# mattm458/tacotron2

Measured on AMD Instinct MI355X. Metric: mel-frames/sec (node), LJSpeech-shaped teacher-forced train step, b=32/GPU, fp32, higher is better.
Workload: dtype f32

## Files before the change

include/tacotron2_amd.h:

```cpp
#ifndef TACOTRON2_AMD_H
#define TACOTRON2_AMD_H
#include <stdint.h>
#ifdef __cplusplus
extern "C" {
#endif

#define T2_OK 0
#define T2_ERR_ARG 1
#define T2_ERR_LAUNCH 2
#define T2_ERR_RESIDENCY 3

const char* t2_last_error(void);
int t2_version(void);
int t2_sizeof(const char* struct_name);
int t2_debug_clock(int enable, uint64_t* out8);

typedef struct {
    const float* A; const float* B; float* C;
    int M, N, K;
    int64_t lda, ldb, ldc;
    int a_kmajor, b_kmajor;
    float alpha;
    const float* bias; const float* bias2;
    const float* mulmask; int64_t ldmask;
    int relu;
    int accumulate;
    int splitk;
    int batch; int64_t sA, sB, sC;
    int share_cu;
    int native_fp32;
    int a_tap_len; int64_t a_tap_stride;
    int precision;
    float* stat_out; int stat_Lp, stat_L;
} T2Gemm;
int t2_gemm(const T2Gemm* g, void* stream);

typedef struct { const float* x; int64_t ldx; const float* w; int64_t ldw; int K; } T2Seg;
typedef struct {
    int B, H;
    int nseg; T2Seg seg[3];
    const float* wpacked;
    const float* pre; int64_t ldpre;
    const float* bias1; const float* bias2;
    const float* c_prev; int64_t ldc_prev;
    const float* drop; int64_t lddrop;
    float* h_out; int64_t ldh;
    float* h_out2; int64_t ldh2;
    float* c_out; int64_t ldc_out;
    float* gates_out; int64_t ldg;
    const int32_t* len; int t;
    const float* xt;
    float* ht_out; int ht_col0;
    const float* zone_h; int64_t ldzone_h;
    const float* zone_c; int64_t ldzone_c;
    const float* h_prev; int64_t ldh_prev;
} T2LstmStep;
int t2_lstm_step_fwd(const T2LstmStep* steps, int n, void* stream);
int t2_lstm_pack_fwd(const T2Seg* segs, int nseg, int H, float* out, void* stream);
int t2_lstm_pack_bwd(const float* W, int64_t ldw, int N4, const float* W2, int64_t ldw2, int N2, int ncols, float* out,
                     void* stream);

typedef struct {
    int64_t seg_x[3]; int64_t pre, c_prev, drop, h_out, h_out2, c_out, gates_out; int dt;
    int64_t xt, ht_out;
    int64_t zone_h, zone_c, h_prev;
} T2LstmStride;
int t2_lstm_seq_fwd(const T2LstmStep* base, const T2LstmStride* inc, int n, int S, void* stream);
int t2_lstm_seq_fwd_persist(const T2LstmStep* base, const T2LstmStride* inc, int S, uint32_t* sync, void* stream);
int t2_lstm_seq_fwd_persist_n(const T2LstmStep* base, const T2LstmStride* inc, int n, int S, uint32_t* sync, void* stream);
int t2_lstm_seq_fwd_persist_pz(const T2LstmStep* base, const T2LstmStride* inc, int n, int S, uint32_t* counters, uint32_t* flag,
                               void* stream);
int t2_lstm_persist_resident(int H, int K, int B);
int t2_lstm_persist_resident_n(int H, int K, int B, int n);
typedef struct {
    void* p[64];
    int64_t row_bytes[64];
    int64_t nrows[64];
    int64_t stride_bytes[64];
    int n;
} T2ZeroRegions;
int t2_zero_regions(const T2ZeroRegions* r, void* stream);
int t2_stream_probe_chain(uint32_t* word, int n, void* stream);
int t2_stream_probe_spin(uint32_t* word, int microseconds, void* stream);
int t2_debug_persist_spin_limit(int polls);
int t2_guard_poison(const uint32_t* flag, float* x, int64_t n, void* stream);
typedef struct {
    int B, H, N4;
    const float* dg_next; int64_t lddg;
    const float* W; int64_t ldw;
    const float* dg2; int64_t lddg2; const float* W2; int64_t ldw2; int N2;
    const float* wtpacked;
    int ncols; int epi;
    const float* ext1; int64_t ldx1; const float* ext2; int64_t ldx2;
    float* dx_out; int64_t lddx;
    const float* drop; int64_t lddrop;
    const float* gates; int64_t ldgs;
    const float* c_prev; int64_t ldcp; const float* c_cur; int64_t ldcc;
    float* dc; int64_t lddc;
    float* dg_out; int64_t ldgo;
    float* dg_out2; int64_t ldgo2;
    const int32_t* len; int t;
    const float* dgt_next;
    float* dgt_out;
    int off_chain;
    const float* zone_h; int64_t ldzone_h;
    const float* zone_c; int64_t ldzone_c;
    float* dhz; int64_t lddhz;
} T2LstmBwdStep;
int t2_lstm_step_bwd(const T2LstmBwdStep* steps, int n, void* stream);
typedef struct { int64_t dg, dg2, ext1, ext2, drop, gates, c_prev, c_cur; int dt; int64_t dgt; int64_t zone_h, zone_c; } T2LstmBwdStride;
int t2_lstm_seq_bwd(const T2LstmBwdStep* base, const T2LstmBwdStride* inc, int n, int S, void* stream);

typedef struct {
    int B, L, A, Ad, Ef, Kl;
    const float* att_h; int64_t ldh;
    const float* Wq; const float* U; const float* v;
    const float* w_prev; int64_t ldw;
    const float* cum_prev; int64_t ldcum;
    const float* pmT; const float* memory; const int32_t* len;
    float* e_part; float* th_out;
    float* w_out; int64_t ldwo; float* cum_out; int64_t ldco;
    float* ctx_out; int64_t ldctx; float* ctx_out2; int64_t ldctx2;
    float* ctxt_out; int ctxt_col0;
    uint64_t* clk;
    int win_back, win_fwd;
    int32_t* win_peak;
    int forward;
} T2AttnStep;
int t2_attn_fold_location(const float* Wd, const float* Wc, float* U, int Ad, int F, int Kl, void* stream);
int t2_attn_step_fwd(const T2AttnStep* s, void* stream);

typedef struct {
    int B, L, T, A, Ad, Ef, Kl;
    const float* W_ih_ctx; int64_t ld_wih;
    const float* W_hh; const float* Wq; const float* U; const float* v;
    const float* wpacked;
    const float* pre; const float* pmT; const float* memory; const int32_t* len;
    const float* att_drop;
    float* xdec; float* att_c; float* gates; float* align; float* cum; float* th;
    float* xproj_ctx; int64_t ld_xproj;
    float* e_part;
    int t_begin, t_end;
    float* xdec_t;
    uint64_t* clk;
    int forward;
} T2AttnSeq;
int t2_attn_seq_fwd(const T2AttnSeq* a, void* stream);

typedef struct {
    int B, L, T, A, Ad, Ef, Kl;
    const float* W_ih_ctx; int64_t ld_wih;
    const float* W_hh; const float* Wq; const float* U; const float* v;
    const float* wtp_ctx;
    const float* wtp_h;
    const float* wtp_q;
    const float* memory; const float* xdec; const float* att_c; const float* gates; const float* align;
    const float* cum; const float* th; const float* att_drop;
    const float* dh_ext; int64_t ld_dh;
    const float* dctx_ext1; int64_t ld_dc1;
    const float* dctx_ext2; int64_t ld_dc2;
    float* dgates; float* dctx_tot; float* dq; float* dpmT; float* dv_part; float* dU_part;
    float* dc; float* G; float* de; float* din_part;
    float* dh_rec;
    int t_hi, t_lo;
    float* dgates_t;
    uint64_t* clk;
    float* ws_bd;
    const float* dalign;
} T2AttnSeqBwd;
int t2_attn_seq_bwd(const T2AttnSeqBwd* a, void* stream);

int t2_attn_seq_bwd_stash(const T2AttnSeqBwd* a, float* de_stash, int64_t ld_stash, void* stream);
int t2_attn_seq_bwd_forward(const T2AttnSeqBwd* a, float* de_stash, int64_t ld_stash, float* dprior, void* stream);
int t2_attn_acc_bwd(const T2AttnSeqBwd* a, const float* de_stash, int64_t ld_stash, int t_begin, int t_end, void* stream);
typedef struct { const float* zone_h; const float* zone_c; int64_t stride; float* dhz; } T2AttnZone;
int t2_attn_seq_fwd_zone(const T2AttnSeq* a, const T2AttnZone* z, void* stream);
int t2_attn_seq_bwd_zone(const T2AttnSeqBwd* a, float* de_stash, int64_t ld_stash, float* dprior, const T2AttnZone* z, void* stream);

int t2_embedding_fwd(const int64_t* idx, const float* table, float* out, int B, int L, int E, int pad, void* stream);
int t2_embedding_bwd(const int64_t* idx, const float* dout, float* dtable, int B, int L, int E, int Lp, int pad, void* stream);
int t2_pack_conv_weight(const float* w, float* wp, int Co, int Ci, int K, int flip, void* stream);
int t2_unpack_conv_wgrad(const float* gp, float* g, int Co, int Ci, int K, void* stream);

typedef struct {
    int B, L, C;
    const float* x; int Lp_x;
    const float* gamma; const float* beta;
    float* running_mean; float* running_var;
    int training; float momentum, eps;
    double* sums;
    float* mean; float* invstd;
    int act;
    const float* drop;
    const float* res; int Lp_res, pad_res;
    const int32_t* len; float fill;
    float* y; int Lp_y, pad_y;
    const float* dy; int Lp_dy, pad_dy;
    float* dx; int Lp_dx, pad_dx;
    float* dgamma; float* dbeta;
    int phase; const float* shift; float grad_share;
    int sums_prezeroed;
    const float* tile_stats; int tile_M;
} T2Bn;
int t2_bn_fwd(const T2Bn* s, void* stream);
int t2_bn_bwd(const T2Bn* s, void* stream);

int t2_colsum(const float* x, int64_t ld, int64_t R, int C, float* out, void* stream);
int t2_mel_to_tm(const float* mel, float* out, int B, int T, int M, void* stream);
int t2_swap01(const float* in, float* out, int D0, int D1, int C, int accumulate, void* stream);
int t2_finalize_fwd(const float* proj, int64_t ld_proj, const int32_t* len, float* mels, float* gates, float* post_in, int B,
                    int T, int M, void* stream);
int t2_finalize_bwd(const float* dpost_in, float* dproj, int B, int T, int M, void* stream);
int t2_outgrad_pack(const float* d_mels, const float* d_post, const float* d_gates, const int32_t* len, float* d_post_out,
                    float* dproj, int B, int T, int M, void* stream);
int t2_loss_fwd_bwd(const float* mels, const float* post, const float* gates, const float* mel_tgt, const float* gate_tgt,
                    const int32_t* len, int B, int T, int M, double* loss3 , float* d_post, float* dproj,
                    float grad_scale, void* stream);
int t2_loss_terms(const float* mels, const float* post, const float* gates, const float* mel_tgt, const float* gate_tgt,
                  const int32_t* len, int B, int T, int M, double* loss3, float* d_mels, float* d_post, float* d_gates,
                  float grad_scale, void* stream);
int t2_guided_attn(const float* align, const int32_t* chars_len, const int32_t* mel_len, int B, int T, int L, float sigma,
                   float alpha, double* loss, float* dalign, float grad_scale, void* stream);
int t2_mel_to_tm_r(const float* mel, float* out, int B, int T, int M, int r, void* stream);
int t2_finalize_fwd_r(const float* proj, int64_t ld_proj, const int32_t* len, float* mels, float* gates, float* post_in, int B,
                      int T, int M, int r, void* stream);
int t2_finalize_bwd_r(const float* dpost_in, float* dproj, int B, int T, int M, int r, void* stream);
int t2_outgrad_pack_r(const float* d_mels, const float* d_post, const float* d_gates, const int32_t* len, float* d_post_out,
                      float* dproj, int B, int T, int M, int r, void* stream);
int t2_loss_fwd_bwd_r(const float* mels, const float* post, const float* gates, const float* mel_tgt, const float* gate_tgt,
                      const int32_t* len, int B, int T, int M, int r, double* loss3, float* d_post, float* dproj,
                      float grad_scale, void* stream);
typedef struct { int mel_loss; int masked; float stop_weight; } T2LossOpts;
int t2_loss_fwd_bwd_opt(const float* mels, const float* post, const float* gates, const float* mel_tgt, const float* gate_tgt,
                        const int32_t* len, int B, int T, int M, int r, double* loss3, float* d_post, float* dproj,
                        float grad_scale, const T2LossOpts* opts, void* stream);
int t2_loss_terms_opt(const float* mels, const float* post, const float* gates, const float* mel_tgt, const float* gate_tgt,
                      const int32_t* len, int B, int T, int M, double* loss3, float* d_mels, float* d_post, float* d_gates,
                      float grad_scale, const T2LossOpts* opts, void* stream);
int t2_relu_mask_bwd(const float* g, const float* y, const float* mask, float* out, int64_t n, void* stream);
int t2_condition_fwd(const float* enc, const float* spk_table, const int32_t* spk, const float* desc, float* memory, int B,
                     int L, int E, int Ef, void* stream);
int t2_condition_bwd(const float* dmem, const float* memory, const int32_t* spk, float* denc, float* dspk_table, float* ddesc,
                     int B, int L, int E, int Ef, void* stream);
int t2_tanh_bias(float* x, const float* bias, int64_t rows, int C, void* stream);
int t2_leaky_relu(const float* x, float* y, int64_t n, float scale, float slope, void* stream);
int t2_axpy(const float* x, float* y, int64_t n, float alpha, void* stream);
int t2_tanh_bwd(const float* g, const float* y, float* out, int64_t n, void* stream);

int t2_linear_rows(const float* x, int64_t ldx, const float* w, int64_t ldw, const float* bias, const float* mask,
                   int64_t ldmask, int relu, float* out, int64_t ldo, int B, int N, int K, void* stream);
typedef struct {
    int B, L, A, D, Ef, Ad, P, M, Kl, Tcap;
    const float* W_comb; const float* b_comb; const float* row_comb;
    const float* W_pre2;
    const float* W_comb_t; const float* W_pre2_t; float* p1_t;
    const float* wp_att; const float* b_att_ih; const float* b_att_hh;
    const float* wp_dec; const float* b_dec_ih; const float* b_dec_hh;
    const float* Wq; const float* U; const float* v;
    const float* pmT; const float* memory; const int32_t* len;
    const float* prenet_mask;
    float* xs; float* att_h; float* att_c; float* dec_c; float* cum; float* xproj; float* p1; float* e_part;
    float* proj; int64_t ld_proj; float* align;
    int32_t* done; int32_t* state;
    const float* dec_pre;
    int win_back, win_fwd;
    int32_t* win_peak;
    int forward;
    float zone_p;
    const float* zone_att; const float* zone_dec;
    float stop_logit;
} T2Infer;
int t2_decoder_infer(const T2Infer* a, int t0, int t1, void* stream);
typedef struct { const float* proj[64]; int Bg[64]; int ngroups; int64_t ld_proj; int M, nframes; } T2StopScan;
int t2_stop_scan(const T2StopScan* s, int64_t* lengths, int32_t* out2, void* stream);
int t2_stop_scan_r(const T2StopScan* s, int r, int max_len, int64_t* lengths, int32_t* out2, void* stream);
int t2_stop_scan_thr(const T2StopScan* s, int r, int max_len, float stop_logit, int64_t* lengths, int32_t* out2, void* stream);

#define T2_ALIGN_MAX_L 4096
typedef struct {
    const float* align; int64_t ld_b, ld_s;
    int B, S, L, r, mode;
    const int32_t* chars_len;
    const int32_t* frames_len;
    int32_t* dur; int64_t ld_dur;
    float* stats;
    uint8_t* back;
} T2AlignDur;
int t2_align_durations(const T2AlignDur* a, void* stream);

#define T2_DTW_MAX_T 4096
#define T2_DTW_MAX_K 32
#define T2_CEPS_MAX_M 1024
typedef struct {
    const float* mel; int64_t ld_b, ld_t;
    int B, T, M, K;
    const int32_t* len;
    const float* basis;
    float* out; int64_t ld_ob, ld_ot;
} T2MelCeps;
int t2_mel_cepstra(const T2MelCeps* a, void* stream);
typedef struct {
    const float* a; int64_t ld_ab, ld_at;
    const float* b; int64_t ld_bb, ld_bt;
    int B, Ta, Tb, K;
    const int32_t* len_a; const int32_t* len_b;
    float scale;
    double* cost;
    int32_t* path_len;
    uint8_t* back;
    int32_t* path;
} T2Dtw;
int t2_dtw(const T2Dtw* a, void* stream);

#define T2_YIN_MAX_SPAN 4096
#define T2_PROSODY_NSTAT 8
#define T2_PROSODY_MAX_T 4096
typedef struct {
    const float* wav; int64_t ld_wav;
    const int64_t* n;
    int B; int64_t n_max;
    int sr, hop, W, tau_min, tau_max;
    float thr, vthr, power_floor;
    float* f0; float* aper; float* power;
    float* cmnd;
} T2Yin;
int t2_yin(const T2Yin* a, void* stream);
typedef struct {
    const float* f0; const float* aper; const float* power;
    const int64_t* n;
    int B, T, hop, S;
    float* out;
} T2ProsodyStats;
int t2_prosody_stats(const T2ProsodyStats* a, void* stream);

int t2_logmel_frames(int64_t n_samples, int hop);
int t2_logmel_fwd(const float* wav, int64_t n, const float* basis, const float* fb, float* padded, float* spec, float* mag,
                  float* out, int n_fft, int hop, int n_mels, void* stream);

int t2_logmel_batch_workspace(int B, int64_t n_max, int n_fft, int hop, int n_mels, int64_t* out5);
int t2_logmel_batch_fwd(const float* wavs, int64_t ld_wav, const int64_t* n_dev, int B, int64_t n_max, const float* basis,
                        const float* fb, float* padded, float* spec, float* mag, float* tmp, float* mel, int64_t T_out,
                        float* gate, int32_t* mel_len, int n_fft, int hop, int n_mels, void* stream);

int t2_philox_mask(float* out, int64_t n, float p, uint64_t seed, uint64_t stream_id, void* stream);
int t2_philox_bernoulli(float* out, int64_t n, float p, uint64_t seed, uint64_t stream_id, void* stream);
int t2_sumsq(const float* g, int64_t n, double* out, void* stream);
int t2_adam_step(float* p, const float* g, float* m, float* v, int64_t n, const double* sumsq, float max_norm, float lr,
                 float beta1, float beta2, float eps, float weight_decay, int step, float grad_scale, void* stream);

#ifdef __cplusplus
}
#endif
#endif
```

tacotron2_amd/csrc/t2_common.hpp:

```cpp
#pragma once
#include <hip/hip_runtime.h>
#include <mutex>
#include <unordered_map>
#include <stdint.h>
#include <stdio.h>
#include <string.h>
#include <stdlib.h>

#include "../../include/tacotron2_amd.h"

typedef float f32x4 __attribute__((ext_vector_type(4)));
typedef float f32x2 __attribute__((ext_vector_type(2)));
typedef float f32x16 __attribute__((ext_vector_type(16)));

#define T2_WAVE 64

#define T2_CHECK_LAUNCH()                                                     \
    do {                                                                      \
        hipError_t e__ = hipGetLastError();                                   \
        if (e__ != hipSuccess) {                                              \
            t2_set_error(hipGetErrorString(e__), __FILE__, __LINE__);         \
            return T2_ERR_LAUNCH;                                             \
        }                                                                     \
    } while (0)

#define T2_REQUIRE(cond, msg)                                                 \
    do {                                                                      \
        if (!(cond)) {                                                        \
            t2_set_error(msg, __FILE__, __LINE__);                            \
            return T2_ERR_ARG;                                                \
        }                                                                     \
    } while (0)

#define T2_TRY(expr)                                                          \
    do {                                                                      \
        int rc__ = (expr);                                                    \
        if (rc__ != 0) return rc__;                                           \
    } while (0)

void t2_set_error(const char* msg, const char* file, int line);

int t2_lstm_step_fwd_launch(const T2LstmStep* steps, int n, hipStream_t st);
int t2_lstm_step_bwd_launch(const T2LstmBwdStep* steps, int n, hipStream_t st, unsigned long long* clk = nullptr);
void t2_lstm_fwd_advance(T2LstmStep& c, const T2LstmStride& inc);
void t2_lstm_bwd_advance(T2LstmBwdStep& c, const T2LstmBwdStride& inc);

#define T2_CHAIN_PRIO() __builtin_amdgcn_s_setprio(3)

#ifdef T2_STAMPS
#define T2_RING_BEGIN(clk, cond, kind)                                                                              \
    unsigned long long* ring__ = nullptr;                                                                           \
    if ((clk) && (cond)) {                                                                                          \
        const unsigned long long seq__ = atomicAdd(&(clk)[32], 1ull);                                               \
        ring__ = (clk) + 40 + 8 * (seq__ % 11);                                                                     \
        ring__[0] = (kind); ring__[4] = 0; ring__[5] = 0; ring__[6] = 0;                                            \
        ring__[1] = __builtin_amdgcn_s_memrealtime(); ring__[3] = __builtin_amdgcn_s_memtime();                     \
    }
#define T2_RING(i) do { if (ring__) ring__[i] = __builtin_amdgcn_s_memtime(); } while (0)
#define T2_RING_END() do { if (ring__) { ring__[7] = __builtin_amdgcn_s_memtime(); ring__[2] = __builtin_amdgcn_s_memrealtime(); } } while (0)
#else
#define T2_RING_BEGIN(clk, cond, kind) do { } while (0)
#define T2_RING(i) do { } while (0)
#define T2_RING_END() do { } while (0)
#endif

#ifdef T2_AB_KNOBS
#define T2_KNOB(env, dflt) (getenv(env) ? atoi(getenv(env)) : (dflt))
#else
#define T2_KNOB(env, dflt) (dflt)
#endif

static inline int t2_cdiv(long a, long b) { return (int)((a + b - 1) / b); }
static inline bool t2_aligned16(const void* p) { return (((uintptr_t)p) & 15) == 0; }

__device__ __forceinline__ float t2_sigmoid(float x) { return __builtin_amdgcn_rcpf(1.0f + __expf(-x)); }
__device__ __forceinline__ float t2_tanh(float x) { return 1.0f - 2.0f * __builtin_amdgcn_rcpf(__expf(2.0f * x) + 1.0f); }

template <int CTRL, int ROW_MASK>
__device__ __forceinline__ float t2_dpp(float ident, float v) {
    return __builtin_bit_cast(float, __builtin_amdgcn_update_dpp(__builtin_bit_cast(int, ident), __builtin_bit_cast(int, v), CTRL,
                                                                 ROW_MASK, 0xf, false));
}
__device__ __forceinline__ float t2_wave_sum(float v) {
    v += t2_dpp<0xB1, 0xf>(0.f, v);
    v += t2_dpp<0x4E, 0xf>(0.f, v);
    v += t2_dpp<0x124, 0xf>(0.f, v);
    v += t2_dpp<0x128, 0xf>(0.f, v);
    v += t2_dpp<0x142, 0xa>(0.f, v);
    v += t2_dpp<0x143, 0xc>(0.f, v);
    return __builtin_bit_cast(float, __builtin_amdgcn_readlane(__builtin_bit_cast(int, v), 63));
}
__device__ __forceinline__ float t2_wave_max(float v) {
    const float ni = -__builtin_inff();
    v = fmaxf(v, t2_dpp<0xB1, 0xf>(ni, v));
    v = fmaxf(v, t2_dpp<0x4E, 0xf>(ni, v));
    v = fmaxf(v, t2_dpp<0x124, 0xf>(ni, v));
    v = fmaxf(v, t2_dpp<0x128, 0xf>(ni, v));
    v = fmaxf(v, t2_dpp<0x142, 0xa>(ni, v));
    v = fmaxf(v, t2_dpp<0x143, 0xc>(ni, v));
    return __builtin_bit_cast(float, __builtin_amdgcn_readlane(__builtin_bit_cast(int, v), 63));
}
__device__ __forceinline__ float t2_quad_sum(float v) {
    v += t2_dpp<0xB1, 0xf>(0.f, v);
    v += t2_dpp<0x4E, 0xf>(0.f, v);
    return v;
}
__device__ __forceinline__ float t2_oct_sum(float v) {
    v = t2_quad_sum(v);
    v += t2_dpp<0x141, 0xf>(0.f, v);
    return v;
}
__device__ __forceinline__ float t2_row_sum(float v) {
    v = t2_quad_sum(v);
    v += t2_dpp<0x124, 0xf>(0.f, v);
    v += t2_dpp<0x128, 0xf>(0.f, v);
    return v;
}
__device__ __forceinline__ float t2_half_sum_hi(float v) {
    v = t2_row_sum(v);
    v += t2_dpp<0x142, 0xa>(0.f, v);
    return v;
}
__device__ __forceinline__ double t2_wave_sum_d(double v) {
#pragma unroll
    for (int o = 32; o > 0; o >>= 1) v += __shfl_xor(v, o, 64);
    return v;
}

__device__ __forceinline__ float t2_block_sum(float v, float* red) {
    const int lane = threadIdx.x & 63, w = threadIdx.x >> 6, nw = (blockDim.x + 63) >> 6;
    v = t2_wave_sum(v);
    __syncthreads();
    if (lane == 0) red[w] = v;
    __syncthreads();
    float s = 0.f;
    for (int i = 0; i < nw; ++i) s += red[i];
    return s;
}
__device__ __forceinline__ float t2_block_max(float v, float* red) {
    const int lane = threadIdx.x & 63, w = threadIdx.x >> 6, nw = (blockDim.x + 63) >> 6;
    v = t2_wave_max(v);
    __syncthreads();
    if (lane == 0) red[w] = v;
    __syncthreads();
    float s = red[0];
    for (int i = 1; i < nw; ++i) s = fmaxf(s, red[i]);
    return s;
}

template <typename K>
inline bool t2_allow_lds(K kernel, size_t bytes) {
    if (bytes <= 64 * 1024) return true;
    if (bytes > 160 * 1024) return false;
    static std::unordered_map<const void*, size_t> granted;
    static std::mutex mu;
    const void* f = reinterpret_cast<const void*>(kernel);
    std::lock_guard<std::mutex> lock(mu);
    size_t& g = granted[f];
    if (bytes > g) {
        if (hipFuncSetAttribute(f, hipFuncAttributeMaxDynamicSharedMemorySize, (int)bytes) != hipSuccess) return false;
        g = bytes;
    }
    return true;
}

__device__ __forceinline__ void t2_philox4(uint32_t c0, uint32_t c1, uint32_t c2, uint32_t c3, uint32_t k0,
                                           uint32_t k1, uint32_t out[4]) {
#pragma unroll
    for (int r = 0; r < 10; ++r) {
        const uint64_t p0 = (uint64_t)0xD2511F53u * c0;
        const uint64_t p1 = (uint64_t)0xCD9E8D57u * c2;
        const uint32_t n0 = (uint32_t)(p1 >> 32) ^ c1 ^ k0;
        const uint32_t n1 = (uint32_t)p1;
        const uint32_t n2 = (uint32_t)(p0 >> 32) ^ c3 ^ k1;
        const uint32_t n3 = (uint32_t)p0;
        c0 = n0; c1 = n1; c2 = n2; c3 = n3;
        k0 += 0x9E3779B9u; k1 += 0xBB67AE85u;
    }
    out[0] = c0; out[1] = c1; out[2] = c2; out[3] = c3;
}
```

tacotron2_amd/csrc/t2_elementwise.hip:

```cpp
#include "t2_common.hpp"
#include <cmath>

namespace {

__global__ void embedding_fwd_kernel(const int64_t* idx, const float* table, float* out, int B, int L, int E, int pad) {
    const int Lp = L + 2 * pad;
    const long n = (long)B * Lp * E;
    for (long i = (long)blockIdx.x * blockDim.x + threadIdx.x; i < n; i += (long)gridDim.x * blockDim.x) {
        const int e = (int)(i % E);
        const long row = i / E;
        const int lp = (int)(row % Lp), b = (int)(row / Lp);
        const int l = lp - pad;
        float v = 0.f;
        if (l >= 0 && l < L) v = table[idx[(long)b * L + l] * E + e];
        out[i] = v;
    }
}

__global__ void embedding_bwd_kernel(const int64_t* idx, const float* dout, float* dtable, int B, int L, int E, int Lp,
                                     int pad) {
    const long n = (long)B * L * E;
    for (long i = (long)blockIdx.x * blockDim.x + threadIdx.x; i < n; i += (long)gridDim.x * blockDim.x) {
        const int e = (int)(i % E);
        const long row = i / E;
        const int l = (int)(row % L), b = (int)(row / L);
        const int64_t id = idx[row];
        if (id != 0) atomicAdd(&dtable[id * E + e], dout[((long)b * Lp + pad + l) * E + e]);
    }
}

__global__ void pack_conv_w_kernel(const float* w, float* wp, int Co, int Ci, int K, int flip) {
    const long n = (long)Co * Ci * K;
    for (long i = (long)blockIdx.x * blockDim.x + threadIdx.x; i < n; i += (long)gridDim.x * blockDim.x) {
        const int k = (int)(i % K);
        const int ci = (int)((i / K) % Ci);
        const int co = (int)(i / ((long)K * Ci));
        if (!flip) wp[(long)co * K * Ci + (long)k * Ci + ci] = w[i];
        else wp[(long)ci * K * Co + (long)(K - 1 - k) * Co + co] = w[i];
    }
}

__global__ void unpack_conv_wgrad_kernel(const float* gp, float* g, int Co, int Ci, int K) {
    const long n = (long)Co * Ci * K;
    for (long i = (long)blockIdx.x * blockDim.x + threadIdx.x; i < n; i += (long)gridDim.x * blockDim.x) {
        const int k = (int)(i % K);
        const int ci = (int)((i / K) % Ci);
        const int co = (int)(i / ((long)K * Ci));
        g[i] += gp[(long)co * K * Ci + (long)k * Ci + ci];
    }
}

struct BnK {
    int B, L, C;
    const float* x; int Lp_x;
    const float* gamma; const float* beta;
    float* rmean; float* rvar;
    int training; float momentum, eps;
    double* sums;
    const float* shift;
    float* mean; float* invstd;
    int act;
    const float* drop;
    const float* res; int Lp_res, pad_res;
    const int32_t* len; float fill;
    float* y; int Lp_y, pad_y;
    const float* dy; int Lp_dy, pad_dy;
    float* dx; int Lp_dx, pad_dx;
    float* dgamma; float* dbeta;
    double grad_share;
};

__global__ __launch_bounds__(256) void bn_stats_kernel(BnK p, int rows_per_block) {
    __shared__ float s1[4][64], s2[4][64];
    const int cl = threadIdx.x & 63, rl = threadIdx.x >> 6;
    const int c = blockIdx.x * 64 + cl;
    const long R = (long)p.B * p.L;
    const long r0 = (long)blockIdx.y * rows_per_block;
    long r1 = r0 + rows_per_block; if (r1 > R) r1 = R;
    float a = 0.f, q = 0.f;
    if (blockIdx.x == 0 && blockIdx.y == 0 && threadIdx.x == 0) atomicAdd(&p.sums[2 * p.C], (double)R);
    if (c < p.C) {
        const float sh = p.shift ? p.shift[c] : p.x[c];
        for (long r = r0 + rl; r < r1; r += 4) {
            const int b = (int)(r / p.L), l = (int)(r % p.L);
            const float v = p.x[((long)b * p.Lp_x + l) * p.C + c] - sh;
            a += v; q = fmaf(v, v, q);
        }
    }
    s1[rl][cl] = a; s2[rl][cl] = q;
    __syncthreads();
    if (rl == 0 && c < p.C) {
        const double sa = (double)s1[0][cl] + s1[1][cl] + s1[2][cl] + s1[3][cl];
        const double sq = (double)s2[0][cl] + s2[1][cl] + s2[2][cl] + s2[3][cl];
        atomicAdd(&p.sums[c], sa);
        atomicAdd(&p.sums[p.C + c], sq);
    }
}

__global__ __launch_bounds__(1024) void bn_merge_tiles_kernel(BnK p, const float* ts, int tile_M) {
    __shared__ double sn[16][64], sm[16][64], sq[16][64];
    const int cl = threadIdx.x & 63, tl = threadIdx.x >> 6;
    const int c = blockIdx.x * 64 + cl;
    const int ntile = (tile_M + 127) / 128;
    const int Lp = p.Lp_x, L = p.L;
    auto upto = [&](int x) { const int r = x % Lp; return (x / Lp) * L + (r < L ? r : L); };
    auto merge = [](double& n, double& mean, double& M2, double nt, double mt, double m2t) {
        if (nt <= 0) return;
        const double tot = n + nt, delta = mt - mean;
        mean += delta * nt / tot;
        M2 += m2t + delta * delta * n * nt / tot;
        n = tot;
    };
    double n = 0, mean = 0, M2 = 0;
    if (c < p.C) {
        for (int t0 = tl; t0 < ntile; t0 += 64) {
            float sh[4], s1[4], s2[4];
#pragma unroll
            for (int u = 0; u < 4; ++u) {
                const int t = t0 + 16 * u;
                const float* o = ts + (long)(t < ntile ? t : 0) * 3 * p.C + c;
                sh[u] = o[0]; s1[u] = o[p.C]; s2[u] = o[2 * (long)p.C];
            }
#pragma unroll
            for (int u = 0; u < 4; ++u) {
                const int t = t0 + 16 * u;
                if (t >= ntile) continue;
                const int r0 = t * 128, r1 = r0 + 128 < tile_M ? r0 + 128 : tile_M;
                const double nt = (double)(upto(r1) - upto(r0));
                if (nt <= 0) continue;
                merge(n, mean, M2, nt, (double)sh[u] + (double)s1[u] / nt, (double)s2[u] - (double)s1[u] * s1[u] / nt);
            }
        }
    }
    sn[tl][cl] = n; sm[tl][cl] = mean; sq[tl][cl] = M2;
    __syncthreads();
    for (int s_ = 8; s_ >= 1; s_ >>= 1) {
        if (tl < s_) {
            double a = sn[tl][cl], b = sm[tl][cl], d = sq[tl][cl];
            merge(a, b, d, sn[tl + s_][cl], sm[tl + s_][cl], sq[tl + s_][cl]);
            sn[tl][cl] = a; sm[tl][cl] = b; sq[tl][cl] = d;
        }
        __syncthreads();
    }
    if (tl == 0 && c < p.C) {
        n = sn[0][cl]; mean = sm[0][cl]; M2 = sq[0][cl];
        const double s = (double)(p.shift ? p.shift[c] : p.x[c]);
        const double dm = mean - s;
        p.sums[c] = n * dm;
        p.sums[p.C + c] = (M2 > 0 ? M2 : 0) + n * dm * dm;
        if (c == 0) p.sums[2 * p.C] = n;
    }
}

__global__ void bn_finalize_kernel(BnK p) {
    const int c = blockIdx.x * blockDim.x + threadIdx.x;
    if (c >= p.C) return;
    if (p.training) {
        const double n = p.sums[2 * p.C];
        const double md = p.sums[c] / n;
        double var = p.sums[p.C + c] / n - md * md;
        if (var < 0) var = 0;
        const double m = md + (double)(p.shift ? p.shift[c] : p.x[c]);
        p.mean[c] = (float)m;
        p.invstd[c] = (float)(1.0 / sqrt(var + (double)p.eps));
        if (p.rmean) {
            const double unb = n > 1 ? var * n / (n - 1) : var;
            p.rmean[c] = (1.f - p.momentum) * p.rmean[c] + p.momentum * (float)m;
            p.rvar[c] = (1.f - p.momentum) * p.rvar[c] + p.momentum * (float)unb;
        }
    } else {
        p.mean[c] = p.rmean[c];
        p.invstd[c] = 1.f / sqrtf(p.rvar[c] + p.eps);
    }
}

__global__ void bn_apply_kernel(BnK p) {
    const long n = (long)p.B * p.Lp_y * p.C;
    for (long i = (long)blockIdx.x * blockDim.x + threadIdx.x; i < n; i += (long)gridDim.x * blockDim.x) {
        const int c = (int)(i % p.C);
        const long row = i / p.C;
        const int lp = (int)(row % p.Lp_y), b = (int)(row / p.Lp_y);
        const int l = lp - p.pad_y;
        float v = 0.f;
        if (l >= 0 && l < p.L) {
            const float xv = p.x[((long)b * p.Lp_x + l) * p.C + c];
            v = (xv - p.mean[c]) * p.invstd[c] * p.gamma[c] + p.beta[c];
            if (p.act == 1) v = fmaxf(v, 0.f);
            else if (p.act == 2) v = t2_tanh(v);
            if (p.drop) v *= p.drop[((long)b * p.L + l) * p.C + c];
            if (p.res) v += p.res[((long)b * p.Lp_res + p.pad_res + l) * p.C + c];
            if (p.len && l >= p.len[b]) v = p.fill;
        }
        p.y[i] = v;
    }
}

__device__ __forceinline__ float bn_dz(const BnK& p, int b, int l, int c, float& xhat) {
    const float xv = p.x[((long)b * p.Lp_x + l) * p.C + c];
    xhat = (xv - p.mean[c]) * p.invstd[c];
    float g = p.dy[((long)b * p.Lp_dy + p.pad_dy + l) * p.C + c];
    if (p.drop) g *= p.drop[((long)b * p.L + l) * p.C + c];
    const float pre = xhat * p.gamma[c] + p.beta[c];
    if (p.act == 1) g = pre > 0.f ? g : 0.f;
    else if (p.act == 2) { const float t = t2_tanh(pre); g *= (1.f - t * t); }
    return g;
}

__global__ __launch_bounds__(256) void bn_bwd_reduce_kernel(BnK p, int rows_per_block) {
    __shared__ float s1[4][64], s2[4][64];
    const int cl = threadIdx.x & 63, rl = threadIdx.x >> 6;
    const int c = blockIdx.x * 64 + cl;
    const long R = (long)p.B * p.L;
    const long r0 = (long)blockIdx.y * rows_per_block;
    long r1 = r0 + rows_per_block; if (r1 > R) r1 = R;
    float a = 0.f, q = 0.f;
    if (blockIdx.x == 0 && blockIdx.y == 0 && threadIdx.x == 0) atomicAdd(&p.sums[2 * p.C], (double)R);
    if (c < p.C) {
        for (long r = r0 + rl; r < r1; r += 4) {
            const int b = (int)(r / p.L), l = (int)(r % p.L);
            float xh;
            const float dz = bn_dz(p, b, l, c, xh);
            a += dz; q = fmaf(dz, xh, q);
        }
    }
    s1[rl][cl] = a; s2[rl][cl] = q;
    __syncthreads();
    if (rl == 0 && c < p.C) {
        atomicAdd(&p.sums[c], (double)s1[0][cl] + s1[1][cl] + s1[2][cl] + s1[3][cl]);
        atomicAdd(&p.sums[p.C + c], (double)s2[0][cl] + s2[1][cl] + s2[2][cl] + s2[3][cl]);
    }
}

__global__ void bn_bwd_apply_kernel(BnK p) {
    const long n = (long)p.B * p.Lp_dx * p.C;
    const float invn = (float)(1.0 / p.sums[2 * p.C]);
    for (long i = (long)blockIdx.x * blockDim.x + threadIdx.x; i < n; i += (long)gridDim.x * blockDim.x) {
        const int c = (int)(i % p.C);
        const long row = i / p.C;
        const int lp = (int)(row % p.Lp_dx), b = (int)(row / p.Lp_dx);
        const int l = lp - p.pad_dx;
        float v = 0.f;
        if (l >= 0 && l < p.L) {
            float xh;
            const float dz = bn_dz(p, b, l, c, xh);
            const float gi = p.gamma[c] * p.invstd[c];
            if (p.training) v = gi * (dz - (float)p.sums[c] * invn - xh * (float)p.sums[p.C + c] * invn);
            else v = gi * dz;
        }
        p.dx[i] = v;
        if (lp == 0 && b == 0) {
            p.dbeta[c] += (float)(p.sums[c] * p.grad_share);
            p.dgamma[c] += (float)(p.sums[p.C + c] * p.grad_share);
        }
    }
}

void to_bnk(const T2Bn* s, BnK& k) {
    k.B = s->B; k.L = s->L; k.C = s->C; k.x = s->x; k.Lp_x = s->Lp_x; k.gamma = s->gamma; k.beta = s->beta;
    k.rmean = s->running_mean; k.rvar = s->running_var; k.training = s->training; k.momentum = s->momentum; k.eps = s->eps;
    k.sums = s->sums; k.mean = s->mean; k.invstd = s->invstd; k.act = s->act; k.drop = s->drop;
    k.res = s->res; k.Lp_res = s->Lp_res; k.pad_res = s->pad_res; k.len = s->len; k.fill = s->fill;
    k.y = s->y; k.Lp_y = s->Lp_y; k.pad_y = s->pad_y; k.dy = s->dy; k.Lp_dy = s->Lp_dy; k.pad_dy = s->pad_dy;
    k.dx = s->dx; k.Lp_dx = s->Lp_dx; k.pad_dx = s->pad_dx; k.dgamma = s->dgamma; k.dbeta = s->dbeta;
    k.shift = s->shift; k.grad_share = s->grad_share > 0.f ? (double)s->grad_share : 1.0;
}

inline int ew_grid(long n) { long g = (n + 255) / 256; return (int)(g > 4096 ? 4096 : (g < 1 ? 1 : g)); }

__global__ __launch_bounds__(256) void colsum_kernel(const float* x, long ld, long R, int C, float* out, int rows_per_block) {
    __shared__ float s1[4][64];
    const int cl = threadIdx.x & 63, rl = threadIdx.x >> 6;
    const int c = blockIdx.x * 64 + cl;
    const long r0 = (long)blockIdx.y * rows_per_block;
    long r1 = r0 + rows_per_block; if (r1 > R) r1 = R;
    float a = 0.f;
    if (c < C) for (long r = r0 + rl; r < r1; r += 4) a += x[r * ld + c];
    s1[rl][cl] = a;
    __syncthreads();
    if (rl == 0 && c < C) atomicAdd(&out[c], s1[0][cl] + s1[1][cl] + s1[2][cl] + s1[3][cl]);
}

__global__ __launch_bounds__(256) void colsum4_kernel(const float* x, long ld, long R, int C, float* out, int rows_per_block) {
    __shared__ f32x4 s1[4][64];
    const int cl = threadIdx.x & 63, rl = threadIdx.x >> 6;
    const int c = blockIdx.x * 256 + cl * 4;
    const int cc = c < C ? c : 0;
    const long r0 = (long)blockIdx.y * rows_per_block;
    long r1 = r0 + rows_per_block; if (r1 > R) r1 = R;
    f32x4 a = {0.f, 0.f, 0.f, 0.f};
    long r = r0 + rl;
    for (; r + 28 < r1; r += 32) {
        f32x4 v[8];
#pragma unroll
        for (int i = 0; i < 8; ++i) v[i] = *reinterpret_cast<const f32x4*>(x + (r + 4 * i) * ld + cc);
#pragma unroll
        for (int i = 0; i < 8; ++i) a += v[i];
    }
    for (; r < r1; r += 4) a += *reinterpret_cast<const f32x4*>(x + r * ld + cc);
    s1[rl][cl] = a;
    __syncthreads();
    if (rl == 0 && c < C) {
        const f32x4 t = s1[0][cl] + s1[1][cl] + s1[2][cl] + s1[3][cl];
        atomicAdd(&out[c], t[0]); atomicAdd(&out[c + 1], t[1]); atomicAdd(&out[c + 2], t[2]); atomicAdd(&out[c + 3], t[3]);
    }
}


template <bool GROUPED>
__global__ void mel_to_tm_kernel(const float* mel, float* out, int B, int T, int M, int r_, int S_) {
    const int r = GROUPED ? r_ : 1, S = GROUPED ? S_ : T;
    const long n = (long)(S + 1) * B * M;
    for (long i = (long)blockIdx.x * blockDim.x + threadIdx.x; i < n; i += (long)gridDim.x * blockDim.x) {
        const int m = (int)(i % M);
        const long row = i / M;
        const int b = (int)(row % B), s = (int)(row / B);
        const long t = (long)r * s - 1;
        out[i] = (s == 0 || (GROUPED && t >= T)) ? 0.f : mel[((long)b * T + t) * M + m];
    }
}

__global__ void swap01_kernel(const float* in, float* out, int D0, int D1, int C, int accumulate) {
    const long n = (long)D0 * D1 * C;
    for (long i = (long)blockIdx.x * blockDim.x + threadIdx.x; i < n; i += (long)gridDim.x * blockDim.x) {
        const int c = (int)(i % C);
        const long row = i / C;
        const int d1 = (int)(row % D1), d0 = (int)(row / D1);
        const long o = ((long)d1 * D0 + d0) * C + c;
        if (accumulate) out[o] += in[i]; else out[o] = in[i];
    }
}

template <bool GROUPED>
__global__ void finalize_fwd_kernel(const float* proj, long ldp, const int32_t* len, float* mels, float* gates, float* post_in,
                                    int B, int T, int M, int r_) {
    const int r = GROUPED ? r_ : 1;
    const int Tp = T + 4, M1 = M + 1;
    const long n = (long)B * Tp * M1;
    for (long i = (long)blockIdx.x * blockDim.x + threadIdx.x; i < n; i += (long)gridDim.x * blockDim.x) {
        const int m = (int)(i % M1);
        const long row = i / M1;
        const int tp = (int)(row % Tp), b = (int)(row / Tp);
        const int t = tp - 2;
        const bool in = t >= 0 && t < T;
        const int s = in ? t / r : 0, j = in ? t - s * r : 0;
        const float v = in ? proj[((long)s * B + b) * ldp + (m < M ? j * M + m : r * M)] : 0.f;
        if (m < M) {
            if (post_in) post_in[((long)b * Tp + tp) * M + m] = v;
            if (in) mels[((long)b * T + t) * M + m] = (t >= len[b]) ? 0.f : v;
        } else if (in) {
            gates[(long)b * T + t] = (t >= len[b]) ? -1000.f : v;
        }
    }
}

__device__ __forceinline__ float loss_stop_w() { return 1.f; }
__device__ __forceinline__ float loss_stop_w(float w) { return w; }
template <bool GROUPED, int MEL = 0, bool MASKED = false, bool WEIGHTED = false, typename... W>
__global__ __launch_bounds__(256) void loss_kernel(const float* mels, const float* post, const float* gates, const float* mel_tgt,
                                                   const float* gate_tgt, const int32_t* len, int B, int T, int M, int r_, int S_,
                                                   double* loss3, float* d_post, float* dproj, float gscale, float* d_mels,
                                                   float* d_gates, W... stop_weight) {
    static_assert(sizeof...(W) == (WEIGHTED ? 1 : 0), "the weight argument comes with WEIGHTED only");
    __shared__ double red[3][4];
    __shared__ unsigned long long nf_s;
    const float stop_w = loss_stop_w(stop_weight...);
    const int r = GROUPED ? r_ : 1, S = GROUPED ? S_ : T;
    const long nm = (long)B * T * M, ng = (long)B * T;
    const long nv = (long)B * S * r * M, ns = (long)B * S;
    const long ldq = (long)r * M + 1;
    float sm = 1.f / (float)nm, sg = 1.f / (float)ng;
    double dm = (double)nm, dg = (double)ng;
    if (MASKED) {
        if (threadIdx.x == 0) nf_s = 0ull;
        __syncthreads();
        unsigned long long c = 0ull;
        for (int b = threadIdx.x; b < B; b += blockDim.x) c += (unsigned long long)min(max(len[b], 0), T);
        if (c) atomicAdd(&nf_s, c);
        __syncthreads();
        const double nf = (double)nf_s;
        dg = nf; dm = nf * (double)M;
        sg = nf > 0.0 ? (float)(1.0 / dg) : 0.f;
        sm = nf > 0.0 ? (float)(1.0 / dm) : 0.f;
    }
    double a_g = 0, a_m = 0, a_p = 0;
    for (long i = (long)blockIdx.x * blockDim.x + threadIdx.x; i < nv + ns; i += (long)gridDim.x * blockDim.x) {
        if (i < nv) {
            const int m = (int)(i % M);
            const long row = i / M;
            const int tv = (int)(row % ((long)S * r)), b = (int)(row / ((long)S * r));
            const int s = tv / r, j = tv - s * r;
            float g = 0.f;
            if (tv < T) {
                const long k = ((long)b * T + tv) * M + m;
                const bool masked = tv >= len[b];
                float g1 = 0.f, g2 = 0.f;
                if (!MASKED || !masked) {
                    const float tg = mel_tgt[k];
                    const float e1 = mels[k] - tg, e2 = post[k] - tg;
                    if (MEL == 0) {
                        a_m += (double)e1 * e1; a_p += (double)e2 * e2;
                        g1 = masked ? 0.f : 2.f * e1 * sm * gscale;
                        g2 = masked ? 0.f : 2.f * e2 * sm * gscale;
                    } else {
                        const float s1 = (float)(e1 > 0.f) - (float)(e1 < 0.f), s2 = (float)(e2 > 0.f) - (float)(e2 < 0.f);
                        a_m += (double)fabsf(e1) + (MEL == 2 ? (double)e1 * e1 : 0.0);
                        a_p += (double)fabsf(e2) + (MEL == 2 ? (double)e2 * e2 : 0.0);
                        g1 = masked ? 0.f : (MEL == 2 ? 2.f * e1 + s1 : s1) * sm * gscale;
                        g2 = masked ? 0.f : (MEL == 2 ? 2.f * e2 + s2 : s2) * sm * gscale;
                    }
                }
                if (d_post) d_post[k] = g2;
                if (d_mels) d_mels[k] = g1;
                g = g1 + g2;
            }
            if (dproj) dproj[((long)s * B + b) * ldq + (long)j * M + m] = g;
        } else {
            const long q = i - nv;
            const int s = (int)(q % S), b = (int)(q / S);
            float gsum = 0.f;
            for (int j = 0; j < r; ++j) {
                const int t = s * r + j;
                if (t >= T) break;
                float g = 0.f;
                if (!MASKED || t < len[b]) {
                    const float x = gates[(long)b * T + t], y = gate_tgt[(long)b * T + t];
                    if (!WEIGHTED) {
                        a_g += (double)(fmaxf(x, 0.f) - x * y + log1pf(expf(-fabsf(x))));
                        g = t >= len[b] ? 0.f : (t2_sigmoid(x) - y) * sg * gscale;
                    } else {
                        const float l1p = log1pf(expf(-fabsf(x)));
                        a_g += (double)(y * (fmaxf(-x, 0.f) + l1p) + stop_w * (1.f - y) * (fmaxf(x, 0.f) + l1p));
                        g = t >= len[b] ? 0.f : (t2_sigmoid(x) * (y + stop_w * (1.f - y)) - y) * sg * gscale;
                    }
                }
                if (d_gates) d_gates[(long)b * T + t] = g;
                gsum = GROUPED ? gsum + g : g;
            }
            if (dproj) dproj[((long)s * B + b) * ldq + (long)r * M] = gsum;
        }
    }
    const int lane = threadIdx.x & 63, w = threadIdx.x >> 6;
    a_g = t2_wave_sum_d(a_g); a_m = t2_wave_sum_d(a_m); a_p = t2_wave_sum_d(a_p);
    if (lane == 0) { red[0][w] = a_g; red[1][w] = a_m; red[2][w] = a_p; }
    __syncthreads();
    if (threadIdx.x < 3) {
        const double s = red[threadIdx.x][0] + red[threadIdx.x][1] + red[threadIdx.x][2] + red[threadIdx.x][3];
        if (!MASKED) atomicAdd(&loss3[threadIdx.x], s / (threadIdx.x == 0 ? (double)ng : (double)nm));
        else if (dg > 0.0) atomicAdd(&loss3[threadIdx.x], s / (threadIdx.x == 0 ? dg : dm));
    }
}
__global__ __launch_bounds__(256) void guided_attn_kernel(const float* align, const int32_t* chars_len, const int32_t* mel_len,
                                                          int B, int T, int L, double inv2s2, float alpha, double* loss,
                                                          float* dalign, float gscale) {
    __shared__ double red[4];
    double acc = 0;
    const int lane = threadIdx.x & 63, w = __builtin_amdgcn_readfirstlane(threadIdx.x >> 6);
    for (long row = (long)blockIdx.x * 4 + w; row < (long)B * T; row += (long)gridDim.x * 4) {
        const int b = (int)(row / T), t = (int)(row - (long)b * T);
        const int Nb = min(max(chars_len[b], 0), L), Tb = min(max(mel_len[b], 0), T);
        const bool live = t < Tb && Nb > 0;
        const double invNT = live ? 1.0 / ((double)Nb * (double)Tb) : 0.0;
        const double coef = (double)alpha / (double)B * invNT;
        const float cg = (float)(coef * (double)gscale);
        float rowsum = 0.f;
        for (int l = lane; l < L; l += 64) {
            float g = 0.f;
            if (live && l < Nb) {
                const double x = (double)((long)l * Tb - (long)t * Nb) * invNT;
                g = -expm1f(-(float)(x * x * inv2s2));
                rowsum = fmaf(g, align[row * L + l], rowsum);
            }
            if (dalign) dalign[row * L + l] = cg * g;
        }
        acc += coef * (double)rowsum;
    }
    acc = t2_wave_sum_d(acc);
    if (lane == 0) red[w] = acc;
    __syncthreads();
    if (threadIdx.x == 0) atomicAdd(loss, red[0] + red[1] + red[2] + red[3]);
}

template <bool GROUPED>
__global__ void outgrad_pack_kernel(const float* d_mels, const float* d_post, const float* d_gates, const int32_t* len,
                                    float* d_post_out, float* dproj, int B, int T, int M, int r_, int S_) {
    const int r = GROUPED ? r_ : 1, S = GROUPED ? S_ : T;
    const long nv = (long)B * S * r * M, ns = (long)B * S;
    const long ldq = (long)r * M + 1;
    for (long i = (long)blockIdx.x * blockDim.x + threadIdx.x; i < nv + ns; i += (long)gridDim.x * blockDim.x) {
        if (i < nv) {
            const int m = (int)(i % M);
            const long row = i / M;
            const int tv = (int)(row % ((long)S * r)), b = (int)(row / ((long)S * r));
            const int s = tv / r, j = tv - s * r;
            float g = 0.f;
            if (tv < T) {
                const long k = ((long)b * T + tv) * M + m;
                const bool masked = tv >= len[b];
                const float g1 = (masked || !d_mels) ? 0.f : d_mels[k];
                const float g2 = (masked || !d_post) ? 0.f : d_post[k];
                d_post_out[k] = g2;
                g = g1 + g2;
            }
            dproj[((long)s * B + b) * ldq + (long)j * M + m] = g;
        } else {
            const long q = i - nv;
            const int s = (int)(q % S), b = (int)(q / S);
            float gsum = 0.f;
            if (d_gates)
                for (int j = 0; j < r; ++j) {
                    const int t = s * r + j;
                    if (t >= T || t >= len[b]) break;
                    gsum = GROUPED ? gsum + d_gates[(long)b * T + t] : d_gates[(long)b * T + t];
                }
            dproj[((long)s * B + b) * ldq + (long)r * M] = gsum;
        }
    }
}

template <bool GROUPED>
__global__ void finalize_bwd_kernel(const float* dpost_in, float* dproj, int B, int T, int M, int r_) {
    const int r = GROUPED ? r_ : 1;
    const int Tp = T + 4;
    const long n = (long)B * T * M;
    const long ldq = (long)r * M + 1;
    for (long i = (long)blockIdx.x * blockDim.x + threadIdx.x; i < n; i += (long)gridDim.x * blockDim.x) {
        const int m = (int)(i % M);
        const long row = i / M;
        const int t = (int)(row % T), b = (int)(row / T);
        const int s = t / r, j = t - s * r;
        dproj[((long)s * B + b) * ldq + (long)j * M + m] += dpost_in[((long)b * Tp + t) * M + m];
    }
}

__global__ void relu_mask_bwd_kernel(const float* g, const float* y, const float* mask, float* out, long n) {
    for (long i = (long)blockIdx.x * blockDim.x + threadIdx.x; i < n; i += (long)gridDim.x * blockDim.x)
        out[i] = y[i] > 0.f ? g[i] * (mask ? mask[i] : 1.f) : 0.f;
}

__global__ void condition_fwd_kernel(const float* enc, const float* spk_table, const int32_t* spk, const float* desc,
                                     float* memory, int B, int L, int E, int Ef) {
    const long n = (long)B * L * Ef;
    for (long i = (long)blockIdx.x * blockDim.x + threadIdx.x; i < n; i += (long)gridDim.x * blockDim.x) {
        const int e = (int)(i % Ef);
        const long row = i / Ef;
        const int b = (int)(row / L);
        float v;
        if (e < E) {
            v = enc[row * E + e];
            if (spk_table) v = t2_tanh(v + spk_table[(long)spk[b] * E + e]);
        } else {
            v = desc[(long)b * (Ef - E) + (e - E)];
        }
        memory[i] = v;
    }
}

__global__ void condition_bwd_kernel(const float* dmem, const float* memory, const int32_t* spk, int has_spk, float* denc,
                                     float* dspk_table, float* ddesc, int B, int L, int E, int Ef) {
    const int b = blockIdx.x, l0 = blockIdx.y * 16;
    for (int e = threadIdx.x; e < Ef; e += blockDim.x) {
        float g[16], m[16];
#pragma unroll
        for (int r = 0; r < 16; ++r) {
            const int l = l0 + r < L ? l0 + r : L - 1;
            const long i = ((long)b * L + l) * Ef + e;
            g[r] = dmem[i];
            m[r] = (e < E && has_spk) ? memory[i] : 0.f;
        }
        float acc = 0.f;
#pragma unroll
        for (int r = 0; r < 16; ++r) {
            if (l0 + r >= L) continue;
            float v = g[r];
            if (e < E) {
                if (has_spk) v *= (1.f - m[r] * m[r]);
                denc[((long)b * L + l0 + r) * E + e] = v;
            }
            acc += v;
        }
        if (e < E) { if (has_spk) atomicAdd(&dspk_table[(long)spk[b] * E + e], acc); }
        else if (ddesc) atomicAdd(&ddesc[(long)b * (Ef - E) + (e - E)], acc);
    }
}

__global__ void tanh_bias_kernel(float* x, const float* bias, long rows, int C) {
    const long n = rows * C;
    for (long i = (long)blockIdx.x * blockDim.x + threadIdx.x; i < n; i += (long)gridDim.x * blockDim.x)
        x[i] = t2_tanh(x[i] + (bias ? bias[i % C] : 0.f));
}
__global__ void tanh_bwd_kernel(const float* g, const float* y, float* out, long n) {
    for (long i = (long)blockIdx.x * blockDim.x + threadIdx.x; i < n; i += (long)gridDim.x * blockDim.x)
        out[i] = g[i] * (1.f - y[i] * y[i]);
}

__global__ void philox_mask_kernel(float* out, long n, float p, uint64_t seed, uint64_t stream_id) {
    const float keep_scale = 1.f / (1.f - p);
    const long n4 = (n + 3) / 4;
    for (long i = (long)blockIdx.x * blockDim.x + threadIdx.x; i < n4; i += (long)gridDim.x * blockDim.x) {
        uint32_t r[4];
        t2_philox4((uint32_t)i, (uint32_t)(i >> 32), (uint32_t)stream_id, (uint32_t)(stream_id >> 32), (uint32_t)seed,
                   (uint32_t)(seed >> 32), r);
#pragma unroll
        for (int j = 0; j < 4; ++j) {
            const long e = 4 * i + j;
            if (e < n) {
                const float u = (float)(r[j] >> 8) * (1.0f / 16777216.0f);
                out[e] = u < p ? 0.f : keep_scale;
            }
        }
    }
}

__global__ void philox_bernoulli_kernel(float* out, long n, float p, uint64_t seed, uint64_t stream_id) {
    const long n4 = (n + 3) / 4;
    for (long i = (long)blockIdx.x * blockDim.x + threadIdx.x; i < n4; i += (long)gridDim.x * blockDim.x) {
        uint32_t r[4];
        t2_philox4((uint32_t)i, (uint32_t)(i >> 32), (uint32_t)stream_id, (uint32_t)(stream_id >> 32), (uint32_t)seed,
                   (uint32_t)(seed >> 32), r);
#pragma unroll
        for (int j = 0; j < 4; ++j) {
            const long e = 4 * i + j;
            if (e < n) out[e] = (float)(r[j] >> 8) * (1.0f / 16777216.0f) < p ? 1.f : 0.f;
        }
    }
}

__global__ __launch_bounds__(256) void sumsq_kernel(const float* g, long n, double* out) {
    __shared__ double red[4];
    double a = 0;
    for (long i = (long)blockIdx.x * blockDim.x + threadIdx.x; i < n; i += (long)gridDim.x * blockDim.x) {
        const double v = g[i];
        a += v * v;
    }
    a = t2_wave_sum_d(a);
    if ((threadIdx.x & 63) == 0) red[threadIdx.x >> 6] = a;
    __syncthreads();
    if (threadIdx.x == 0) atomicAdd(out, red[0] + red[1] + red[2] + red[3]);
}

__global__ void adam_kernel(float* p, const float* g, float* m, float* v, long n, const double* sumsq, float max_norm,
                            float lr, float b1, float b2, float eps, float wd, float bc1, float bc2, float gscale) {
    float clip = 1.f;
    if (sumsq && !isfinite(*sumsq)) return;
    if (sumsq && max_norm > 0.f) {
        const float tot = (float)sqrt(*sumsq) * gscale;
        const float c = max_norm / (tot + 1e-6f);
        clip = c < 1.f ? c : 1.f;
    }
    clip *= gscale;
    for (long i = (long)blockIdx.x * blockDim.x + threadIdx.x; i < n; i += (long)gridDim.x * blockDim.x) {
        const float pv = p[i];
        const float gr = g[i] * clip + wd * pv;
        const float mv = b1 * m[i] + (1.f - b1) * gr;
        const float vv = b2 * v[i] + (1.f - b2) * gr * gr;
        m[i] = mv; v[i] = vv;
        p[i] = pv - lr * (mv / bc1) / (sqrtf(vv / bc2) + eps);
    }
}

__global__ void guard_poison_kernel(const uint32_t* flag, float* x, long n) {
    if (__hip_atomic_load(flag, __ATOMIC_RELAXED, __HIP_MEMORY_SCOPE_AGENT) == 0u) return;
    for (long i = (long)blockIdx.x * blockDim.x + threadIdx.x; i < n; i += (long)gridDim.x * blockDim.x) x[i] = __builtin_nanf("");
}

struct ZeroK { T2ZeroRegions r; };
__global__ __launch_bounds__(256) void zero_regions_kernel(ZeroK k) {
    const int y = blockIdx.y;
    char* base = (char*)k.r.p[y];
    const long rb = k.r.row_bytes[y], nr = k.r.nrows[y], sb = k.r.stride_bytes[y];
    const long tid = (long)blockIdx.x * blockDim.x + threadIdx.x, nth = (long)gridDim.x * blockDim.x;
    if (nr == 1 || sb == rb) {
        const long n = rb * nr;
        if ((((uintptr_t)base) & 15) == 0 && (n & 15) == 0) {
            f32x4* q = (f32x4*)base;
            const f32x4 z = {0.f, 0.f, 0.f, 0.f};
            for (long i = tid; i < (n >> 4); i += nth) q[i] = z;
        } else {
            uint32_t* q = (uint32_t*)base;
            for (long i = tid; i < (n >> 2); i += nth) q[i] = 0u;
        }
    } else {
        const long rw = rb >> 2;
        for (long i = tid; i < rw * nr; i += nth) {
            const long row = i / rw, c = i - row * rw;
            ((uint32_t*)(base + row * sb))[c] = 0u;
        }
    }
}

__global__ void probe_tick_kernel(uint32_t* word) { word[0] += 1u; }
__global__ void probe_spin_kernel(uint32_t* word, unsigned long long ticks) {
    const unsigned long long t0 = __builtin_amdgcn_s_memrealtime();
    unsigned polls = 0;
    while (__builtin_amdgcn_s_memrealtime() - t0 < ticks && polls < (1u << 24)) { __builtin_amdgcn_s_sleep(16); ++polls; }
    word[0] = polls;
}

}

#define ST ((hipStream_t)stream)

extern "C" int t2_zero_regions(const T2ZeroRegions* r, void* stream) {
    (void)hipGetLastError();
    T2_REQUIRE(r && r->n >= 0 && r->n <= 64, "t2_zero_regions: 0..64 regions");
    if (r->n == 0) return T2_OK;
    long most = 0;
    for (int i = 0; i < r->n; ++i) {
        T2_REQUIRE(r->p[i] && r->row_bytes[i] > 0 && r->nrows[i] > 0 && (r->row_bytes[i] & 3) == 0 && ((uintptr_t)r->p[i] & 3) == 0 &&
                   (r->nrows[i] == 1 || ((r->stride_bytes[i] & 3) == 0 && r->stride_bytes[i] >= r->row_bytes[i])),
                   "t2_zero_regions: regions are 4-byte aligned runs of whole words (rows: stride >= row, a multiple of 4)");
        const long n = r->row_bytes[i] * r->nrows[i];
        if (n > most) most = n;
    }
    long gx = (most + 16 * 256 * 8 - 1) / (16 * 256 * 8);
    gx = gx < 1 ? 1 : (gx > 1024 ? 1024 : gx);
    ZeroK k; k.r = *r;
    hipLaunchKernelGGL(zero_regions_kernel, dim3((unsigned)gx, r->n), dim3(256), 0, ST, k);
    T2_CHECK_LAUNCH(); return T2_OK;
}
extern "C" int t2_stream_probe_chain(uint32_t* word, int n, void* stream) {
    (void)hipGetLastError();
    T2_REQUIRE(word && n >= 0 && n <= 100000, "t2_stream_probe_chain: bad arguments");
    for (int i = 0; i < n; ++i) hipLaunchKernelGGL(probe_tick_kernel, dim3(1), dim3(1), 0, ST, word);
    T2_CHECK_LAUNCH(); return T2_OK;
}
extern "C" int t2_stream_probe_spin(uint32_t* word, int microseconds, void* stream) {
    (void)hipGetLastError();
    T2_REQUIRE(word && microseconds >= 0 && microseconds <= 50000, "t2_stream_probe_spin: 0..50000 us");
    hipLaunchKernelGGL(probe_spin_kernel, dim3(1), dim3(64), 0, ST, word, (unsigned long long)microseconds * 100ull);
    T2_CHECK_LAUNCH(); return T2_OK;
}

extern "C" int t2_guard_poison(const uint32_t* flag, float* x, int64_t n, void* stream) {
    (void)hipGetLastError();
    T2_REQUIRE(flag && x && n >= 0, "t2_guard_poison: bad arguments");
    if (n == 0) return T2_OK;
    hipLaunchKernelGGL(guard_poison_kernel, dim3(ew_grid(n) > 1024 ? 1024 : ew_grid(n)), dim3(256), 0, ST, flag, x, (long)n);
    T2_CHECK_LAUNCH(); return T2_OK;
}

extern "C" int t2_embedding_fwd(const int64_t* idx, const float* table, float* out, int B, int L, int E, int pad, void* stream) {
    (void)hipGetLastError();
    T2_REQUIRE(idx && table && out, "t2_embedding_fwd: null");
    hipLaunchKernelGGL(embedding_fwd_kernel, dim3(ew_grid((long)B * (L + 2 * pad) * E)), dim3(256), 0, ST, idx, table, out, B, L, E, pad);
    T2_CHECK_LAUNCH(); return T2_OK;
}
extern "C" int t2_embedding_bwd(const int64_t* idx, const float* dout, float* dtable, int B, int L, int E, int Lp, int pad, void* stream) {
    (void)hipGetLastError();
    T2_REQUIRE(idx && dout && dtable, "t2_embedding_bwd: null");
    hipLaunchKernelGGL(embedding_bwd_kernel, dim3(ew_grid((long)B * L * E)), dim3(256), 0, ST, idx, dout, dtable, B, L, E, Lp, pad);
    T2_CHECK_LAUNCH(); return T2_OK;
}
extern "C" int t2_pack_conv_weight(const float* w, float* wp, int Co, int Ci, int K, int flip, void* stream) {
    (void)hipGetLastError();
    T2_REQUIRE(w && wp, "t2_pack_conv_weight: null");
    hipLaunchKernelGGL(pack_conv_w_kernel, dim3(ew_grid((long)Co * Ci * K)), dim3(256), 0, ST, w, wp, Co, Ci, K, flip);
    T2_CHECK_LAUNCH(); return T2_OK;
}
extern "C" int t2_unpack_conv_wgrad(const float* gp, float* g, int Co, int Ci, int K, void* stream) {
    (void)hipGetLastError();
    T2_REQUIRE(gp && g, "t2_unpack_conv_wgrad: null");
    hipLaunchKernelGGL(unpack_conv_wgrad_kernel, dim3(ew_grid((long)Co * Ci * K)), dim3(256), 0, ST, gp, g, Co, Ci, K);
    T2_CHECK_LAUNCH(); return T2_OK;
}

extern "C" int t2_bn_fwd(const T2Bn* s, void* stream) {
    (void)hipGetLastError();
    T2_REQUIRE(s && s->x && s->gamma && s->beta && s->mean && s->invstd && s->y, "t2_bn_fwd: null operand");
    T2_REQUIRE(s->training ? (s->sums != nullptr) : (s->running_mean && s->running_var), "t2_bn_fwd: stats operands");
    T2_REQUIRE(s->phase >= 0 && s->phase <= 2 && (s->phase == 0 || (s->training && s->shift)),
               "t2_bn_fwd: phases 1/2 (sync-BN) need training statistics and a rank-independent shift");
    BnK k; to_bnk(s, k);
    if (s->training && s->phase != 2) {
        if (s->tile_stats) {
            T2_REQUIRE(s->tile_M > 0 && (long)s->tile_M <= (long)s->B * s->Lp_x, "t2_bn_fwd: tile_M is the producing GEMM's row count");
            hipLaunchKernelGGL(bn_merge_tiles_kernel, dim3(t2_cdiv(s->C, 64)), dim3(1024), 0, ST, k, s->tile_stats, s->tile_M);
        } else {
            if (!s->sums_prezeroed) (void)hipMemsetAsync(s->sums, 0, sizeof(double) * (2 * s->C + 2), ST);
            const long R = (long)s->B * s->L;
            const int rpb = 128;
            hipLaunchKernelGGL(bn_stats_kernel, dim3(t2_cdiv(s->C, 64), t2_cdiv(R, rpb)), dim3(256), 0, ST, k, rpb);
        }
    }
    if (s->phase != 1) {
        hipLaunchKernelGGL(bn_finalize_kernel, dim3(t2_cdiv(s->C, 256)), dim3(256), 0, ST, k);
        hipLaunchKernelGGL(bn_apply_kernel, dim3(ew_grid((long)s->B * s->Lp_y * s->C)), dim3(256), 0, ST, k);
    }
    T2_CHECK_LAUNCH(); return T2_OK;
}

extern "C" int t2_bn_bwd(const T2Bn* s, void* stream) {
    (void)hipGetLastError();
    T2_REQUIRE(s && s->x && s->gamma && s->beta && s->mean && s->invstd && s->dy && s->dx && s->sums && s->dgamma && s->dbeta,
               "t2_bn_bwd: null operand");
    T2_REQUIRE(s->phase >= 0 && s->phase <= 2, "t2_bn_bwd: bad phase");
    BnK k; to_bnk(s, k);
    if (s->phase != 2) {
        if (!s->sums_prezeroed) (void)hipMemsetAsync(s->sums, 0, sizeof(double) * (2 * s->C + 2), ST);
        const long R = (long)s->B * s->L;
        const int rpb = 128;
        hipLaunchKernelGGL(bn_bwd_reduce_kernel, dim3(t2_cdiv(s->C, 64), t2_cdiv(R, rpb)), dim3(256), 0, ST, k, rpb);
    }
    if (s->phase != 1) hipLaunchKernelGGL(bn_bwd_apply_kernel, dim3(ew_grid((long)s->B * s->Lp_dx * s->C)), dim3(256), 0, ST, k);
    T2_CHECK_LAUNCH(); return T2_OK;
}

extern "C" int t2_colsum(const float* x, int64_t ld, int64_t R, int C, float* out, void* stream) {
    (void)hipGetLastError();
    T2_REQUIRE(x && out && R > 0 && C > 0, "t2_colsum: bad arguments");
    if (C % 4 == 0 && ld % 4 == 0 && t2_aligned16(x) && C >= 256) {
        const int cb = t2_cdiv(C, 256);
        long rpb = t2_cdiv(R, t2_cdiv(1024, cb)); rpb = (rpb + 31) / 32 * 32; if (rpb < 32) rpb = 32;
        hipLaunchKernelGGL(colsum4_kernel, dim3(cb, t2_cdiv(R, rpb)), dim3(256), 0, ST, x, (long)ld, (long)R, C, out, (int)rpb);
    } else {
        const int rpb = 256;
        hipLaunchKernelGGL(colsum_kernel, dim3(t2_cdiv(C, 64), t2_cdiv(R, rpb)), dim3(256), 0, ST, x, (long)ld, (long)R, C, out, rpb);
    }
    T2_CHECK_LAUNCH(); return T2_OK;
}
extern "C" int t2_mel_to_tm(const float* mel, float* out, int B, int T, int M, void* stream) {
    (void)hipGetLastError();
    T2_REQUIRE(mel && out, "t2_mel_to_tm: null");
    hipLaunchKernelGGL(mel_to_tm_kernel<false>, dim3(ew_grid((long)(T + 1) * B * M)), dim3(256), 0, ST, mel, out, B, T, M, 1, T);
    T2_CHECK_LAUNCH(); return T2_OK;
}
extern "C" int t2_swap01(const float* in, float* out, int D0, int D1, int C, int accumulate, void* stream) {
    (void)hipGetLastError();
    T2_REQUIRE(in && out, "t2_swap01: null");
    hipLaunchKernelGGL(swap01_kernel, dim3(ew_grid((long)D0 * D1 * C)), dim3(256), 0, ST, in, out, D0, D1, C, accumulate);
    T2_CHECK_LAUNCH(); return T2_OK;
}
extern "C" int t2_finalize_fwd(const float* proj, int64_t ld_proj, const int32_t* len, float* mels, float* gates, float* post_in,
                               int B, int T, int M, void* stream) {
    (void)hipGetLastError();
    T2_REQUIRE(proj && len && mels && gates, "t2_finalize_fwd: null");
    hipLaunchKernelGGL(finalize_fwd_kernel<false>, dim3(ew_grid((long)B * (T + 4) * (M + 1))), dim3(256), 0, ST, proj, (long)ld_proj, len,
                       mels, gates, post_in, B, T, M, 1);
    T2_CHECK_LAUNCH(); return T2_OK;
}
extern "C" int t2_loss_fwd_bwd(const float* mels, const float* post, const float* gates, const float* mel_tgt,
                               const float* gate_tgt, const int32_t* len, int B, int T, int M, double* loss3, float* d_post,
                               float* dproj, float grad_scale, void* stream) {
    (void)hipGetLastError();
    T2_REQUIRE(mels && post && gates && mel_tgt && gate_tgt && len && loss3, "t2_loss_fwd_bwd: null");
    (void)hipMemsetAsync(loss3, 0, 3 * sizeof(double), ST);
    hipLaunchKernelGGL(loss_kernel<false>, dim3(ew_grid((long)B * T * (M + 1))), dim3(256), 0, ST, mels, post, gates, mel_tgt, gate_tgt,
                       len, B, T, M, 1, T, loss3, d_post, dproj, grad_scale, (float*)nullptr, (float*)nullptr);
    T2_CHECK_LAUNCH(); return T2_OK;
}
extern "C" int t2_loss_terms(const float* mels, const float* post, const float* gates, const float* mel_tgt, const float* gate_tgt,
                             const int32_t* len, int B, int T, int M, double* loss3, float* d_mels, float* d_post, float* d_gates,
                             float grad_scale, void* stream) {
    (void)hipGetLastError();
    T2_REQUIRE(mels && post && gates && mel_tgt && gate_tgt && len && loss3, "t2_loss_terms: null");
    (void)hipMemsetAsync(loss3, 0, 3 * sizeof(double), ST);
    hipLaunchKernelGGL(loss_kernel<false>, dim3(ew_grid((long)B * T * (M + 1))), dim3(256), 0, ST, mels, post, gates, mel_tgt, gate_tgt,
                       len, B, T, M, 1, T, loss3, d_post, (float*)nullptr, grad_scale, d_mels, d_gates);
    T2_CHECK_LAUNCH(); return T2_OK;
}
extern "C" int t2_guided_attn(const float* align, const int32_t* chars_len, const int32_t* mel_len, int B, int T, int L, float sigma,
                              float alpha, double* loss, float* dalign, float grad_scale, void* stream) {
    (void)hipGetLastError();
    T2_REQUIRE(align && chars_len && mel_len && loss, "t2_guided_attn: null");
    T2_REQUIRE(B >= 1 && T >= 1 && L >= 1, "t2_guided_attn: need B, T, L >= 1");
    T2_REQUIRE(sigma > 0.f && alpha >= 0.f, "t2_guided_attn: need sigma > 0 and alpha >= 0");
    (void)hipMemsetAsync(loss, 0, sizeof(double), ST);
    const long wgs = ((long)B * T + 3) / 4;
    hipLaunchKernelGGL(guided_attn_kernel, dim3((unsigned)(wgs > 4096 ? 4096 : wgs)), dim3(256), 0, ST, align, chars_len, mel_len,
                       B, T, L, 1.0 / (2.0 * (double)sigma * (double)sigma), alpha, loss, dalign, grad_scale);
    T2_CHECK_LAUNCH(); return T2_OK;
}
extern "C" int t2_outgrad_pack(const float* d_mels, const float* d_post, const float* d_gates, const int32_t* len,
                               float* d_post_out, float* dproj, int B, int T, int M, void* stream) {
    (void)hipGetLastError();
    T2_REQUIRE(len && d_post_out && dproj, "t2_outgrad_pack: null");
    hipLaunchKernelGGL(outgrad_pack_kernel<false>, dim3(ew_grid((long)B * T * (M + 1))), dim3(256), 0, ST, d_mels, d_post, d_gates, len,
                       d_post_out, dproj, B, T, M, 1, T);
    T2_CHECK_LAUNCH(); return T2_OK;
}
extern "C" int t2_finalize_bwd(const float* dpost_in, float* dproj, int B, int T, int M, void* stream) {
    (void)hipGetLastError();
    T2_REQUIRE(dpost_in && dproj, "t2_finalize_bwd: null");
    hipLaunchKernelGGL(finalize_bwd_kernel<false>, dim3(ew_grid((long)B * T * M)), dim3(256), 0, ST, dpost_in, dproj, B, T, M, 1);
    T2_CHECK_LAUNCH(); return T2_OK;
}
#define T2_REQUIRE_GROUPED(name) \
    T2_REQUIRE(B >= 1 && T >= 1 && M >= 1 && r >= 1 && (long)((T + r - 1) / r) * r < (1L << 31), name ": need B, T, M >= 1 and r >= 1")
extern "C" int t2_mel_to_tm_r(const float* mel, float* out, int B, int T, int M, int r, void* stream) {
    (void)hipGetLastError();
    T2_REQUIRE(mel && out, "t2_mel_to_tm_r: null");
    T2_REQUIRE_GROUPED("t2_mel_to_tm_r");
    if (r == 1) return t2_mel_to_tm(mel, out, B, T, M, stream);
    const int S = (T + r - 1) / r;
    hipLaunchKernelGGL(mel_to_tm_kernel<true>, dim3(ew_grid((long)(S + 1) * B * M)), dim3(256), 0, ST, mel, out, B, T, M, r, S);
    T2_CHECK_LAUNCH(); return T2_OK;
}
extern "C" int t2_finalize_fwd_r(const float* proj, int64_t ld_proj, const int32_t* len, float* mels, float* gates, float* post_in,
                                 int B, int T, int M, int r, void* stream) {
    (void)hipGetLastError();
    T2_REQUIRE(proj && len && mels && gates, "t2_finalize_fwd_r: null");
    T2_REQUIRE_GROUPED("t2_finalize_fwd_r");
    T2_REQUIRE(ld_proj >= (int64_t)r * M + 1, "t2_finalize_fwd_r: ld_proj < r * M + 1");
    if (r == 1) return t2_finalize_fwd(proj, ld_proj, len, mels, gates, post_in, B, T, M, stream);
    hipLaunchKernelGGL(finalize_fwd_kernel<true>, dim3(ew_grid((long)B * (T + 4) * (M + 1))), dim3(256), 0, ST, proj, (long)ld_proj, len, mels,
                       gates, post_in, B, T, M, r);
    T2_CHECK_LAUNCH(); return T2_OK;
}
extern "C" int t2_loss_fwd_bwd_r(const float* mels, const float* post, const float* gates, const float* mel_tgt,
                                 const float* gate_tgt, const int32_t* len, int B, int T, int M, int r, double* loss3, float* d_post,
                                 float* dproj, float grad_scale, void* stream) {
    (void)hipGetLastError();
    T2_REQUIRE(mels && post && gates && mel_tgt && gate_tgt && len && loss3 && d_post && dproj, "t2_loss_fwd_bwd_r: null");
    T2_REQUIRE_GROUPED("t2_loss_fwd_bwd_r");
    if (r == 1) return t2_loss_fwd_bwd(mels, post, gates, mel_tgt, gate_tgt, len, B, T, M, loss3, d_post, dproj, grad_scale, stream);
    const int S = (T + r - 1) / r;
    (void)hipMemsetAsync(loss3, 0, 3 * sizeof(double), ST);
    hipLaunchKernelGGL(loss_kernel<true>, dim3(ew_grid((long)B * S * ((long)r * M + 1))), dim3(256), 0, ST, mels, post, gates, mel_tgt,
                       gate_tgt, len, B, T, M, r, S, loss3, d_post, dproj, grad_scale, (float*)nullptr, (float*)nullptr);
    T2_CHECK_LAUNCH(); return T2_OK;
}
static int loss_opts_check(const T2LossOpts* o, const char* what) {
    T2_REQUIRE(o != nullptr, what);
    T2_REQUIRE(o->mel_loss >= 0 && o->mel_loss <= 2, what);
    T2_REQUIRE(std::isfinite(o->stop_weight) && o->stop_weight > 0.f, what);
    return T2_OK;
}
template <bool GROUPED>
static void loss_opt_launch(const T2LossOpts* o, unsigned grid, hipStream_t st, const float* mels, const float* post, const float* gates,
                            const float* mel_tgt, const float* gate_tgt, const int32_t* len, int B, int T, int M, int r, int S,
                            double* loss3, float* d_post, float* dproj, float gs, float* d_mels, float* d_gates) {
    const int key = o->mel_loss * 4 + (o->masked ? 2 : 0) + (o->stop_weight != 1.f ? 1 : 0);
#define T2_LOSS_CASE(MEL, MASKED)                               \
    case (MEL) * 4 + (MASKED) * 2:                                                                                                   \
        hipLaunchKernelGGL((loss_kernel<GROUPED, MEL, (MASKED) != 0, false>), dim3(grid), dim3(256), 0, st, mels, post, gates, mel_tgt, \
                           gate_tgt, len, B, T, M, r, S, loss3, d_post, dproj, gs, d_mels, d_gates);                                  \
        break;                                                                                                                       \
    case (MEL) * 4 + (MASKED) * 2 + 1:                                                                                               \
        hipLaunchKernelGGL((loss_kernel<GROUPED, MEL, (MASKED) != 0, true, float>), dim3(grid), dim3(256), 0, st, mels, post, gates,  \
                           mel_tgt, gate_tgt, len, B, T, M, r, S, loss3, d_post, dproj, gs, d_mels, d_gates, o->stop_weight);         \
        break;
    switch (key) {
        T2_LOSS_CASE(0, 0) T2_LOSS_CASE(0, 1) T2_LOSS_CASE(1, 0) T2_LOSS_CASE(1, 1) T2_LOSS_CASE(2, 0) T2_LOSS_CASE(2, 1)
    }
#undef T2_LOSS_CASE
}
static bool loss_opts_default(const T2LossOpts* o) { return o->mel_loss == 0 && !o->masked && o->stop_weight == 1.f; }
extern "C" int t2_loss_fwd_bwd_opt(const float* mels, const float* post, const float* gates, const float* mel_tgt,
                                   const float* gate_tgt, const int32_t* len, int B, int T, int M, int r, double* loss3, float* d_post,
                                   float* dproj, float grad_scale, const T2LossOpts* opts, void* stream) {
    (void)hipGetLastError();
    T2_REQUIRE(mels && post && gates && mel_tgt && gate_tgt && len && loss3 && d_post && dproj, "t2_loss_fwd_bwd_opt: null");
    T2_REQUIRE_GROUPED("t2_loss_fwd_bwd_opt");
    T2_TRY(loss_opts_check(opts, "t2_loss_fwd_bwd_opt: need options with mel_loss in {0, 1, 2} and a finite stop_weight > 0"));
    if (loss_opts_default(opts))
        return t2_loss_fwd_bwd_r(mels, post, gates, mel_tgt, gate_tgt, len, B, T, M, r, loss3, d_post, dproj, grad_scale, stream);
    const int S = (T + r - 1) / r;
    (void)hipMemsetAsync(loss3, 0, 3 * sizeof(double), ST);
    const unsigned grid = ew_grid((long)B * S * ((long)r * M + 1));
    if (r == 1) loss_opt_launch<false>(opts, grid, ST, mels, post, gates, mel_tgt, gate_tgt, len, B, T, M, 1, T, loss3, d_post, dproj,
                                       grad_scale, nullptr, nullptr);
    else loss_opt_launch<true>(opts, grid, ST, mels, post, gates, mel_tgt, gate_tgt, len, B, T, M, r, S, loss3, d_post, dproj, grad_scale,
                               nullptr, nullptr);
    T2_CHECK_LAUNCH(); return T2_OK;
}
extern "C" int t2_loss_terms_opt(const float* mels, const float* post, const float* gates, const float* mel_tgt, const float* gate_tgt,
                                 const int32_t* len, int B, int T, int M, double* loss3, float* d_mels, float* d_post, float* d_gates,
                                 float grad_scale, const T2LossOpts* opts, void* stream) {
    (void)hipGetLastError();
    T2_REQUIRE(mels && post && gates && mel_tgt && gate_tgt && len && loss3, "t2_loss_terms_opt: null");
    T2_REQUIRE(B >= 1 && T >= 1 && M >= 1, "t2_loss_terms_opt: need B, T, M >= 1");
    T2_TRY(loss_opts_check(opts, "t2_loss_terms_opt: need options with mel_loss in {0, 1, 2} and a finite stop_weight > 0"));
    if (loss_opts_default(opts))
        return t2_loss_terms(mels, post, gates, mel_tgt, gate_tgt, len, B, T, M, loss3, d_mels, d_post, d_gates, grad_scale, stream);
    (void)hipMemsetAsync(loss3, 0, 3 * sizeof(double), ST);
    loss_opt_launch<false>(opts, ew_grid((long)B * T * (M + 1)), ST, mels, post, gates, mel_tgt, gate_tgt, len, B, T, M, 1, T, loss3, d_post,
                           nullptr, grad_scale, d_mels, d_gates);
    T2_CHECK_LAUNCH(); return T2_OK;
}
extern "C" int t2_outgrad_pack_r(const float* d_mels, const float* d_post, const float* d_gates, const int32_t* len,
                                 float* d_post_out, float* dproj, int B, int T, int M, int r, void* stream) {
    (void)hipGetLastError();
    T2_REQUIRE(len && d_post_out && dproj, "t2_outgrad_pack_r: null");
    T2_REQUIRE_GROUPED("t2_outgrad_pack_r");
    if (r == 1) return t2_outgrad_pack(d_mels, d_post, d_gates, len, d_post_out, dproj, B, T, M, stream);
    const int S = (T + r - 1) / r;
    hipLaunchKernelGGL(outgrad_pack_kernel<true>, dim3(ew_grid((long)B * S * ((long)r * M + 1))), dim3(256), 0, ST, d_mels, d_post, d_gates,
                       len, d_post_out, dproj, B, T, M, r, S);
    T2_CHECK_LAUNCH(); return T2_OK;
}
extern "C" int t2_finalize_bwd_r(const float* dpost_in, float* dproj, int B, int T, int M, int r, void* stream) {
    (void)hipGetLastError();
    T2_REQUIRE(dpost_in && dproj, "t2_finalize_bwd_r: null");
    T2_REQUIRE_GROUPED("t2_finalize_bwd_r");
    if (r == 1) return t2_finalize_bwd(dpost_in, dproj, B, T, M, stream);
    hipLaunchKernelGGL(finalize_bwd_kernel<true>, dim3(ew_grid((long)B * T * M)), dim3(256), 0, ST, dpost_in, dproj, B, T, M, r);
    T2_CHECK_LAUNCH(); return T2_OK;
}
extern "C" int t2_relu_mask_bwd(const float* g, const float* y, const float* mask, float* out, int64_t n, void* stream) {
    (void)hipGetLastError();
    T2_REQUIRE(g && y && out, "t2_relu_mask_bwd: null");
    hipLaunchKernelGGL(relu_mask_bwd_kernel, dim3(ew_grid(n)), dim3(256), 0, ST, g, y, mask, out, (long)n);
    T2_CHECK_LAUNCH(); return T2_OK;
}
extern "C" int t2_condition_fwd(const float* enc, const float* spk_table, const int32_t* spk, const float* desc, float* memory,
                                int B, int L, int E, int Ef, void* stream) {
    (void)hipGetLastError();
    T2_REQUIRE(enc && memory && (Ef == E || desc), "t2_condition_fwd: bad arguments");
    hipLaunchKernelGGL(condition_fwd_kernel, dim3(ew_grid((long)B * L * Ef)), dim3(256), 0, ST, enc, spk_table, spk, desc, memory, B,
                       L, E, Ef);
    T2_CHECK_LAUNCH(); return T2_OK;
}
extern "C" int t2_condition_bwd(const float* dmem, const float* memory, const int32_t* spk, float* denc, float* dspk_table,
                                float* ddesc, int B, int L, int E, int Ef, void* stream) {
    (void)hipGetLastError();
    T2_REQUIRE(dmem && memory && denc, "t2_condition_bwd: null");
    hipLaunchKernelGGL(condition_bwd_kernel, dim3(B, t2_cdiv(L, 16)), dim3(256), 0, ST, dmem, memory, spk, dspk_table != nullptr, denc,
                       dspk_table, ddesc, B, L, E, Ef);
    T2_CHECK_LAUNCH(); return T2_OK;
}
__global__ void leaky_relu_kernel(const float* x, float* y, long n, float scale, float slope) {
    for (long i = (long)blockIdx.x * blockDim.x + threadIdx.x; i < n; i += (long)gridDim.x * blockDim.x) {
        const float v = scale * x[i];
        y[i] = v > 0.f ? v : slope * v;
    }
}
__global__ void axpy_kernel(const float* x, float* y, long n, float alpha) {
    for (long i = (long)blockIdx.x * blockDim.x + threadIdx.x; i < n; i += (long)gridDim.x * blockDim.x) y[i] = fmaf(alpha, x[i], y[i]);
}
extern "C" int t2_leaky_relu(const float* x, float* y, int64_t n, float scale, float slope, void* stream) {
    (void)hipGetLastError();
    T2_REQUIRE(x && y && n >= 0, "t2_leaky_relu: bad arguments");
    if (n == 0) return T2_OK;
    hipLaunchKernelGGL(leaky_relu_kernel, dim3(ew_grid(n)), dim3(256), 0, ST, x, y, (long)n, scale, slope);
    T2_CHECK_LAUNCH(); return T2_OK;
}
extern "C" int t2_axpy(const float* x, float* y, int64_t n, float alpha, void* stream) {
    (void)hipGetLastError();
    T2_REQUIRE(x && y && n >= 0, "t2_axpy: bad arguments");
    if (n == 0) return T2_OK;
    hipLaunchKernelGGL(axpy_kernel, dim3(ew_grid(n)), dim3(256), 0, ST, x, y, (long)n, alpha);
    T2_CHECK_LAUNCH(); return T2_OK;
}
extern "C" int t2_tanh_bias(float* x, const float* bias, int64_t rows, int C, void* stream) {
    (void)hipGetLastError();
    T2_REQUIRE(x, "t2_tanh_bias: null");
    hipLaunchKernelGGL(tanh_bias_kernel, dim3(ew_grid(rows * C)), dim3(256), 0, ST, x, bias, (long)rows, C);
    T2_CHECK_LAUNCH(); return T2_OK;
}
extern "C" int t2_tanh_bwd(const float* g, const float* y, float* out, int64_t n, void* stream) {
    (void)hipGetLastError();
    T2_REQUIRE(g && y && out, "t2_tanh_bwd: null");
    hipLaunchKernelGGL(tanh_bwd_kernel, dim3(ew_grid(n)), dim3(256), 0, ST, g, y, out, (long)n);
    T2_CHECK_LAUNCH(); return T2_OK;
}
extern "C" int t2_philox_mask(float* out, int64_t n, float p, uint64_t seed, uint64_t stream_id, void* stream) {
    (void)hipGetLastError();
    T2_REQUIRE(out && n >= 0 && p >= 0.f && p < 1.f, "t2_philox_mask: bad arguments");
    if (n == 0) return T2_OK;
    hipLaunchKernelGGL(philox_mask_kernel, dim3(ew_grid((n + 3) / 4)), dim3(256), 0, ST, out, (long)n, p, seed, stream_id);
    T2_CHECK_LAUNCH(); return T2_OK;
}
extern "C" int t2_philox_bernoulli(float* out, int64_t n, float p, uint64_t seed, uint64_t stream_id, void* stream) {
    (void)hipGetLastError();
    T2_REQUIRE(out && n >= 0 && p >= 0.f && p <= 1.f, "t2_philox_bernoulli: bad arguments");
    if (n == 0) return T2_OK;
    hipLaunchKernelGGL(philox_bernoulli_kernel, dim3(ew_grid((n + 3) / 4)), dim3(256), 0, ST, out, (long)n, p, seed, stream_id);
    T2_CHECK_LAUNCH(); return T2_OK;
}
extern "C" int t2_sumsq(const float* g, int64_t n, double* out, void* stream) {
    (void)hipGetLastError();
    T2_REQUIRE(g && out, "t2_sumsq: null");
    (void)hipMemsetAsync(out, 0, sizeof(double), ST);
    hipLaunchKernelGGL(sumsq_kernel, dim3(ew_grid(n) > 1024 ? 1024 : ew_grid(n)), dim3(256), 0, ST, g, (long)n, out);
    T2_CHECK_LAUNCH(); return T2_OK;
}
extern "C" int t2_adam_step(float* p, const float* g, float* m, float* v, int64_t n, const double* sumsq, float max_norm, float lr,
                            float beta1, float beta2, float eps, float weight_decay, int step, float grad_scale, void* stream) {
    (void)hipGetLastError();
    T2_REQUIRE(p && g && m && v && step >= 1, "t2_adam_step: bad arguments");
    const float bc1 = 1.f - powf(beta1, (float)step), bc2 = 1.f - powf(beta2, (float)step);
    hipLaunchKernelGGL(adam_kernel, dim3(ew_grid(n)), dim3(256), 0, ST, p, g, m, v, (long)n, sumsq, max_norm, lr, beta1, beta2, eps,
                       weight_decay, bc1, bc2, grad_scale);
    T2_CHECK_LAUNCH(); return T2_OK;
}
```

tacotron2_amd/csrc/t2_error.cpp:

```cpp
#include <stdio.h>
#include "../../include/tacotron2_amd.h"
static thread_local char g_err[512] = "";
void t2_set_error(const char* msg, const char* file, int line) {
    snprintf(g_err, sizeof(g_err), "%s (%s:%d)", msg ? msg : "?", file ? file : "?", line);
}
extern "C" const char* t2_last_error(void) { return g_err; }
extern "C" int t2_version(void) { return 100; }

#include <string.h>
extern "C" int t2_sizeof(const char* name) {
#define T2_SZ(T) if (strcmp(name, #T) == 0) return (int)sizeof(T)
    T2_SZ(T2Gemm); T2_SZ(T2Seg); T2_SZ(T2LstmStep); T2_SZ(T2LstmStride); T2_SZ(T2LstmBwdStep); T2_SZ(T2LstmBwdStride);
    T2_SZ(T2AttnStep); T2_SZ(T2AttnSeq); T2_SZ(T2AttnSeqBwd); T2_SZ(T2Bn); T2_SZ(T2Infer); T2_SZ(T2StopScan); T2_SZ(T2ZeroRegions);
    T2_SZ(T2AlignDur); T2_SZ(T2AttnZone); T2_SZ(T2LossOpts); T2_SZ(T2MelCeps); T2_SZ(T2Dtw);
    T2_SZ(T2Yin); T2_SZ(T2ProsodyStats);
#undef T2_SZ
    return -1;
}
```

tacotron2_amd/engine.py:

```python
from __future__ import annotations

import contextlib
import ctypes
import math
import numbers
import threading as _threading
from typing import Dict, NamedTuple, Optional

import torch

from . import _lib
from . import guard as _guard
from ._lib import call, make
from .params import ParamStore, reduction_factor

KL, KPAD = 31, 15


def _stream():
    return torch.cuda.current_stream().cuda_stream


_TLS = _threading.local()

# ... 42 lines not shown
        raise ValueError(f"yin: need 0 < fmin < fmax, got fmin = {fmin!r}, fmax = {fmax!r}")
    return int(sr // fmax), int(sr // fmin)


def _check_lengths(fn: str, n, B: int, dev):
    if not torch.is_tensor(n) or n.device != dev:
        raise ValueError(f"{fn}: n must be a tensor on the device of the signals, {dev}")
    if n.dim() != 1 or n.shape[0] != B or n.is_floating_point() or n.dtype == torch.bool:
        raise ValueError(f"{fn}: n must be {B} integers")
    return n.to(torch.int64).contiguous()


def yin(wav, n, sr=22050, hop=256, W=1024, fmin=60.0, fmax=500.0, thr=0.1, vthr=0.3, power_floor=1e-10, n_max=None,
        return_cmnd=False):
    if not torch.is_tensor(wav) or wav.dim() != 2 or wav.dtype != torch.float32:
        raise ValueError("yin: wav must be a float32 (B, samples) tensor")
    if wav.device.type != "cuda":
        raise ValueError(f"yin: wav must be on the GPU, got {wav.device}")
    B, ld = wav.shape
    if B < 1 or B > 65535:
        raise ValueError(f"yin: batch of {B}, outside 1 .. 65535")
    if ld > 1 and wav.stride(1) != 1:
        raise ValueError("yin: the last dimension of wav must be contiguous")
    n_max = ld if n_max is None else int(n_max)
    ld_wav = wav.stride(0) if B > 1 else max(ld, 1)
    if not 0 <= n_max <= ld or (B > 1 and ld_wav < n_max):
        raise ValueError(f"yin: n_max = {n_max} outside 0 .. {ld}, the row length of wav (row stride {ld_wav})")
    n64 = _check_lengths("yin", n, B, wav.device)
    for name, val in (("hop", hop), ("W", W)):
        if isinstance(val, bool) or not isinstance(val, int):
            raise ValueError(f"yin: {name} must be an integer, got {val!r}")
    tau_min, tau_max = yin_lags(sr, fmin, fmax)
    if hop < 1 or W < 16:
        raise ValueError(f"yin: need hop >= 1 and W >= 16, got hop = {hop}, W = {W}")
    if tau_min < 2 or tau_max <= tau_min + 1:
        raise ValueError(f"yin: lags {tau_min} .. {tau_max} of {fmin} .. {fmax} Hz at {sr} Hz: need tau_min >= 2 and "
                         "tau_max > tau_min + 1")
    if W + tau_max > YIN_MAX_SPAN:
        raise ValueError(f"yin: W + tau_max = {W + tau_max} samples per frame, above the limit of {YIN_MAX_SPAN} (T2_YIN_MAX_SPAN)")
    for name, val in (("thr", thr), ("vthr", vthr), ("power_floor", power_floor)):
        if not isinstance(val, numbers.Real) or not math.isfinite(val):
            raise ValueError(f"yin: {name} must be a finite number, got {val!r}")
    T = 1 + n_max // hop
    with torch.cuda.device(wav.device):
        f0, aper, power = (torch.empty(B, T, dtype=torch.float32, device=wav.device) for _ in range(3))
        cmnd = torch.empty(B, T, tau_max + 1, dtype=torch.float32, device=wav.device) if return_cmnd else None
        a = make("T2Yin", wav=wav, ld_wav=ld_wav, n=n64, B=B, n_max=n_max, sr=sr, hop=hop, W=W, tau_min=tau_min, tau_max=tau_max,
                 thr=float(thr), vthr=float(vthr), power_floor=float(power_floor), f0=f0, aper=aper, power=power, cmnd=cmnd)
        call("t2_yin", a, _stream())
    return (f0, aper, power, cmnd) if return_cmnd else (f0, aper, power)


def prosody_stats(f0, aper, power, n, hop=256, span=1024 + 367):
    for name, x in (("f0", f0), ("aper", aper), ("power", power)):
        if not torch.is_tensor(x) or x.dim() != 2 or x.dtype != torch.float32:
            raise ValueError(f"prosody_stats: {name} must be a float32 (B, T) tensor")
        if x.device.type != "cuda" or x.device != f0.device:
            raise ValueError(f"prosody_stats: {name} must be on the GPU, all three on one device")
        if x.shape != f0.shape or not x.is_contiguous():
            raise ValueError(f"prosody_stats: {name} must be contiguous and of the shape of f0 {tuple(f0.shape)}")
    B, T = f0.shape
    if B < 1 or B > 65535:
        raise ValueError(f"prosody_stats: batch of {B}, outside 1 .. 65535")
    if T < 1 or T > PROSODY_MAX_T:
        raise ValueError(f"prosody_stats: {T} frames, outside 1 .. {PROSODY_MAX_T} (T2_PROSODY_MAX_T)")
    for name, val in (("hop", hop), ("span", span)):
        if isinstance(val, bool) or not isinstance(val, int) or val < 1:
            raise ValueError(f"prosody_stats: {name} must be an integer >= 1, got {val!r}")
    n64 = _check_lengths("prosody_stats", n, B, f0.device)
    with torch.cuda.device(f0.device):
        out = torch.empty(B, PROSODY_NSTAT, dtype=torch.float32, device=f0.device)
        a = make("T2ProsodyStats", f0=f0, aper=aper, power=power, n=n64, B=B, T=T, hop=hop, S=span, out=out)
        call("t2_prosody_stats", a, _stream())
    return out


def fill_splits(M: int, N: int, K: int) -> bool:
    return ((M + 127) // 128) * ((N + 127) // 128) < 256 and K >= 1024


def chunk_splits(frames: int, B: int, D: int) -> int:
    tiles = ((frames * B + 127) // 128) * ((4 * D + 127) // 128)
    return max(1, min(4, 256 // max(tiles, 1)))


def check_attention_window(window):
    if window is None:
        return None
    try:
        back, fwd = window
    except (TypeError, ValueError):
        raise ValueError(f"attention_window must be (back, fwd), got {window!r}") from None
    for v in (back, fwd):
        if isinstance(v, bool) or not isinstance(v, numbers.Integral) or v < 0:
            raise ValueError(f"attention_window must be two integers >= 0, got {window!r}")
    return int(back), int(fwd)


def check_forward_attention(forward, window=None):
    if not isinstance(forward, bool):
        raise ValueError(f"forward_attention must be True or False, got {forward!r}")
    if forward and window is not None:
        raise ValueError("forward_attention does not compose with attention_window: use one of the two")
    return forward


def check_rate(p, name: str, closed: bool = False) -> float:
    if isinstance(p, bool) or not isinstance(p, (int, float)) or not (0.0 <= float(p) < 1.0 or (closed and float(p) == 1.0)):
        raise ValueError(f"{name} must be a number in [0, 1{']' if closed else ')'}, got {p!r}")
    return float(p)


def zone_stride(z, n: int) -> int:
    return 0 if z is None or z.shape[0] == 1 else n


def check_guided_attention(guided):
    if guided is None:
        return None
    try:
        sigma, alpha = guided
    except (TypeError, ValueError):
        raise ValueError(f"guided_attention must be (sigma, alpha), got {guided!r}") from None
    for v in (sigma, alpha):
        if isinstance(v, bool) or not isinstance(v, numbers.Real) or v != v or abs(v) == float("inf"):
            raise ValueError(f"guided_attention must be two finite numbers (sigma, alpha), got {guided!r}")
    if sigma <= 0 or alpha < 0:
        raise ValueError(f"guided_attention needs sigma > 0 and alpha >= 0, got {guided!r}")
    return float(sigma), float(alpha)


MEL_LOSSES = ("l2", "l1", "l1+l2")
LOSS_DEFAULTS = ("l2", False, 1.0)


def check_loss_options(loss):
    if loss is None:
        return LOSS_DEFAULTS
    if isinstance(loss, dict):
        unknown = sorted(set(loss) - {"mel", "masked", "stop_weight"})
        if unknown:
            raise ValueError(f"loss options: unknown key {unknown[0]!r} (known: mel, masked, stop_weight)")
        mel, masked, w = (loss.get(k, dflt) for k, dflt in zip(("mel", "masked", "stop_weight"), LOSS_DEFAULTS))
    else:
        try:
            mel, masked, w = loss
        except (TypeError, ValueError):
            raise ValueError(f"loss options must be a dict or (mel, masked, stop_weight), got {loss!r}") from None
    if not isinstance(mel, str) or mel not in MEL_LOSSES:
        raise ValueError(f"loss options: mel must be one of {', '.join(MEL_LOSSES)}, got {mel!r}")
    if not isinstance(masked, bool):
        raise ValueError(f"loss options: masked must be True or False, got {masked!r}")
    if isinstance(w, bool) or not isinstance(w, numbers.Real) or w != w or abs(w) == float("inf") or w <= 0:
        raise ValueError(f"loss options: stop_weight must be a finite number > 0, got {w!r}")
    if not 0.0 < float(ctypes.c_float(float(w)).value) < float("inf"):
        raise ValueError(f"loss options: stop_weight must be a finite float32 > 0, got {w!r}")
    return mel, masked, float(w)


def loss_opts_struct(loss):
    mel, masked, w = loss
    return make("T2LossOpts", mel_loss=MEL_LOSSES.index(mel), masked=int(masked), stop_weight=w)


def check_stop_threshold(tau) -> float:
    if isinstance(tau, bool) or not isinstance(tau, numbers.Real) or not 0.0 < float(tau) < 1.0:
        raise ValueError(f"stop_threshold must be a number with 0 < threshold < 1, got {tau!r}")
    return float(tau)


def stop_logit(tau: float) -> float:
    v = float(ctypes.c_float(math.log(tau / (1.0 - tau))).value)
    if v != v or abs(v) == float("inf"):
        raise ValueError(f"stop_threshold {tau!r} has no finite float32 logit")
    return v


def _ptr(t: torch.Tensor, elem_off: int = 0) -> int:
    return t.data_ptr() + 4 * elem_off


def _pending() -> Dict[int, list]:
    d = getattr(_TLS, "pending", None)
    if d is None:
        d = _TLS.pending = {}
    return d


def zero_later(t: torch.Tensor) -> torch.Tensor:
    if t.numel() == 0:
        return t
    es = t.element_size()
    if t.is_contiguous():
        reg = (t.data_ptr(), t.numel() * es, 1, t.numel() * es)
    else:
        assert t.dim() == 2 and t.stride(1) == 1, "zero_later: contiguous tensors or rows with unit inner stride"
        reg = (t.data_ptr(), t.shape[1] * es, t.shape[0], t.stride(0) * es)
    assert reg[0] % 4 == 0 and reg[1] % 4 == 0 and reg[3] % 4 == 0, "zero_later: regions are runs of whole 4-byte words"
    st = torch.cuda.current_stream(t.device)
    _pending().setdefault(st.cuda_stream, []).append((reg, t))
    return t


def flush_zeros() -> None:
    mine = _pending()
    if not mine:
        return
    pending = list(mine.items())
    mine.clear()
    for stream, regs in pending:
        for i0 in range(0, len(regs), 64):
            part = regs[i0:i0 + 64]
            z = _lib.S["T2ZeroRegions"]()
            for i, ((ptr, rb, nr, sb), _) in enumerate(part):
                z.p[i] = ptr; z.row_bytes[i] = rb; z.nrows[i] = nr; z.stride_bytes[i] = sb
            z.n = len(part)
            call("t2_zero_regions", z, stream)


_lib.PRE_CALL.append(flush_zeros)


def splitk_for(M: int, N: int, K: int) -> int:
    tiles = ((M + 127) // 128) * ((N + 127) // 128)
    kt = (K + 31) // 32
    best, best_cost = 1, None
    for sk in range(1, max(1, min(kt // 4, 64)) + 1):
        w = tiles * sk
        cost = ((w + 255) // 256) / sk * (1.15 if w < 384 else 1.0) * (1.0 + 0.01 * sk)
        if best_cost is None or cost < best_cost - 1e-12:
            best, best_cost = sk, cost
    return best


def _chunk_sizes(T: int, CH: int, ramp_at_end: bool = True):
    if not ramp_at_end or CH < 16 or T <= CH:
        return [min(CH, T - c0) for c0 in range(0, T, CH)]
    tail = [CH // 2, CH // 4, CH // 8, CH - CH // 2 - CH // 4 - CH // 8]
    body = T - CH
    sizes = [min(CH, body - c0) for c0 in range(0, body, CH)]
    return sizes + tail


def chunk_ranges(T: int, CH: int, ramp: bool = True, descending: bool = False):
    edges = [0]
    for n in _chunk_sizes(T, CH, ramp_at_end=ramp):
        edges.append(edges[-1] + n)
    asc = list(zip(edges[:-1], edges[1:]))
    return [(c1, c0) for c0, c1 in reversed(asc)] if descending else asc


def forward_schedule(T: int, CH: int, B: int, D: int, ramp: bool = True, splitk_small: bool = True, controls: bool = False):
    out = []
    for c0, c1 in chunk_ranges(T, CH, ramp):
        sk = chunk_splits(c1 - c0, B, D) if splitk_small else 1
        out.append((c0, c1, sk, sk > 1 and not controls))
    return out


class SideOp(NamedTuple):
    kind: str
    share: bool
    hi: int = 0
    lo: int = 0
    k: int = -1


class BackwardSchedule(NamedTuple):
    chunks: tuple
    tail: tuple


def backward_schedule(T: int, CH: int, WG: int, n_deferred: int, stash: bool, ramp: bool = True) -> BackwardSchedule:
    ranges = chunk_ranges(T, CH, ramp, descending=True)
    n, left = len(ranges), n_deferred
    dec_hi = att_hi = T

    def att(kind, k, hi=None):
        return SideOp(kind, kind == "att_wgrads", ranges[k][0] if hi is None else hi, ranges[k][1], k)
    chunks = []
    for ci, (hi, lo) in enumerate(ranges):
        ops = []
        if (ci + 1) % WG == 0:
            ops.append(SideOp("dec_wgrads", True, dec_hi, lo)); dec_hi = lo
        if left and ci >= 4:
            ops.append(SideOp("deferred", True)); left -= 1
        k = ci - 2
        if k >= 0:
            if stash:
                ops.append(att("att_acc", k))
            if (k + 1) % WG == 0:
                ops.append(att("att_wgrads", k, hi=att_hi)); att_hi = ranges[k][1]
        chunks.append((hi, lo, tuple(ops)))
    tail = [att("att_acc", n - 2)] if stash and n >= 2 else []
    tail += [SideOp("deferred", False)] * left
    if dec_hi > 0:
        tail.append(SideOp("dec_wgrads", True, dec_hi, 0))
    if stash:
        tail.append(att("att_acc", n - 1))
    tail += [SideOp("acc_done", False), att("att_wgrads", n - 1, hi=att_hi)]
    return BackwardSchedule(tuple(chunks), tuple(tail))


class Engine:

    def __init__(self, ps: ParamStore):
        self.ps = ps
        self.d = ps.dims
        self.r = reduction_factor(ps.dims)
        self.dev = ps.device
        self.zoneout = check_rate(ps.dims.get("zoneout", 0.0), "zoneout", closed=True)
        self.cell_dropout = check_rate(ps.dims.get("cell_dropout", 0.1), "cell_dropout")
        self._ws: Dict[str, torch.Tensor] = {}
        self._ceps_bases: Dict[tuple, torch.Tensor] = {}
        self._cleared: Dict[tuple, tuple] = {}
        self._bn_clean: set = set()
        self._persist_next = 0
        self._side = None
        self.chunk = 64
        self.chunk_bwd = 64
        self.dec_chain = "persistent"
        self._persist_sync = None
        self._persist_ok = {}
        self.wgrad_group = 4
        self.ramp_chunks = True
        self.share_cu = 1
        self.splitk_small_chunks = True
        self.enc_chain = "persistent"
        self.enc_persist_max_rows = 32
        self.bn_epilogue_stats = False
        self.bptt_off_chain = True
        self.sync_bn_group = None
        self.guided_loss = None
        self.grad_tail_hook = None
        self.generation = 0
        self.profile = False
        self.marks = []; self.spans = []
        self.guard_bytes = _guard.DEFAULT_BYTES
        self._guards: Dict[str, tuple] = {}
        self._guard_short: Dict[str, int] = {}

    def persist_resident(self, D: int, B: int, n: int = 1) -> bool:
        key = (D, min(B, 32) <= 16, n)
        if key not in self._persist_ok:
            rc = _lib.call_value("t2_lstm_persist_resident_n", D, D, min(B, 32), n)
            if rc not in (0, 3):
                raise _lib.T2Error(f"t2_lstm_persist_resident failed (rc={rc}): {_lib.lib().t2_last_error().decode()}")
            self._persist_ok[key] = rc == 0
        return self._persist_ok[key]

    def persist_sync(self):
        if self._persist_sync is None:
            self._persist_sync = torch.zeros(self.PERSIST_RING0 + 256 * self.PERSIST_RING, dtype=torch.int32, device=self.dev)
        return self._persist_sync

    def check_persistent_kernels(self):
        if self._persist_sync is not None and int(self._persist_sync[256].item()) != 0:
            self._persist_sync[256:272].zero_()
            raise _lib.T2Error("t2_lstm_seq_fwd_persist: an inter-workgroup wait timed out (outputs of that forward are invalid)")
        if self.guard_bytes > 0 or self.ps.guard_bytes > 0:
            hits = self.guard_check()
            if hits:
                raise _lib.T2Error("guard bands overwritten: " + _guard.describe(hits))

    def guard_check(self) -> list:
        if self.dev.type == "cuda":
            torch.cuda.synchronize(self.dev)
        hits = []
        for name, (backing, g, n, short) in self._guards.items():
            hits += _guard.scan(name, backing, g, n, short)
        return hits + self.ps.guard_check()

    def side_stream(self):
        if self._side is None:
            self._side = torch.cuda.Stream(device=self.dev)
        return self._side

    def stream_concurrency_check(self, n: int = 200, spin_us: int = 3000) -> dict:
        import os
        main, side = torch.cuda.current_stream(), self.side_stream()
        w = torch.zeros(8, dtype=torch.int32, device=self.dev)

        def pattern(spin):
            e0, e1 = torch.cuda.Event(enable_timing=True), torch.cuda.Event(enable_timing=True)
            e0.record(main)
            if spin:
                self._wait(side, e0)
                call("t2_stream_probe_spin", _ptr(w, 4), spin, side.cuda_stream)
            call("t2_stream_probe_chain", w, n, main.cuda_stream)
            e1.record(main)
            torch.cuda.synchronize(self.dev)
            return e0.elapsed_time(e1) * 1e3

        pattern(10)
        alone_us = pattern(0)
        beside_us = pattern(spin_us)
        ok = beside_us < alone_us + 0.5 * spin_us
        return dict(ok=bool(ok), launches=n, chain_alone_us=round(alone_us, 1), chain_beside_spin_us=round(beside_us, 1),
                    spin_us=spin_us, us_per_dependent_launch=round(alone_us / n, 2),
                    GPU_MAX_HW_QUEUES=os.environ.get("GPU_MAX_HW_QUEUES"))

    def ensure_concurrent_streams(self, max_tries: int = 8) -> dict:
        qc = self.stream_concurrency_check()
        tries = 1
        while not qc["ok"] and tries < max_tries:
            self._spare_streams = getattr(self, "_spare_streams", []) + [self._side]
            self._side = torch.cuda.Stream(device=self.dev)
            qc = self.stream_concurrency_check()
            tries += 1
        qc["tries"] = tries
        return qc

    def mark(self, name: str):
        if self.profile:
            ev = torch.cuda.Event(enable_timing=True)
            ev.record(torch.cuda.current_stream())
            self.marks.append((name, ev))

    def segment_times_ms(self):
        out: Dict[str, float] = {}
        for (n0, e0), (n1, e1) in zip(self.marks[:-1], self.marks[1:]):
            out[n1] = out.get(n1, 0.0) + e0.elapsed_time(e1)
        for name, e0, e1 in self.spans:
            out[name] = out.get(name, 0.0) + e0.elapsed_time(e1)
        return out

    def span_begin(self):
        if not self.profile:
            return None
        ev = torch.cuda.Event(enable_timing=True)
        ev.record(torch.cuda.current_stream())
        return ev

    def span_end(self, name: str, e0):
        if e0 is not None:
            ev = torch.cuda.Event(enable_timing=True)
            ev.record(torch.cuda.current_stream())
            self.spans.append((name, e0, ev))

    def make_masks(self, B: int, L: int, T: int, training: bool, seed: int, step: int) -> dict:
        d = self.d
        p = float(d["dropout"])
        E, Pd, A, D, M, Pn = d["encoded_dim"], d["prenet_dim"], d["att_rnn_dim"], d["rnn_hidden_dim"], d["num_mels"], d["postnet_dim"]
        st = _stream()
        sid = [step * 64]
        Tf, T = T, (T + self.r - 1) // self.r

        def gen(name, n, rate):
            m = self.buf("mask." + name, n)
            call("t2_philox_mask", m, n, rate, seed, sid[0], st)
            sid[0] += 1
            return m

        masks = {}
        if p > 0.0:
            masks["prenet_drop"] = [gen(f"pre{i}", (T + 1) * B * Pd, p).view(T + 1, B, Pd) for i in range(2)]
        if training:
            if p > 0.0:
                masks["enc_drop"] = [gen(f"enc{i}", B * L * E, p).view(B, L, E) for i in range(3)]
                chans = [Pn, Pn, Pn, Pn, M]
                masks["post_drop"] = [gen(f"post{i}", B * Tf * c, p).view(B, Tf, c) for i, c in enumerate(chans)]
            if self.cell_dropout > 0.0:
                masks["att_drop"] = gen("att", T * B * A, self.cell_dropout).view(T, B, A)
                masks["dec_drop"] = gen("dec", T * B * D, self.cell_dropout).view(T, B, D)
        if self.zoneout > 0.0 and training:
            for i, (key, H) in enumerate((("att_zone_h", A), ("att_zone_c", A), ("dec_zone_h", D), ("dec_zone_c", D))):
                masks[key] = self.buf("mask." + key, T, B, H)
                call("t2_philox_bernoulli", masks[key], T * B * H, self.zoneout, seed, step * 64 + 48 + i, st)
        elif self.zoneout > 0.0:
            for cell, H in (("att", A), ("dec", D)):
                block = self.buf(f"mask.{cell}_zone_p", 1, B, H).fill_(self.zoneout)
                masks[cell + "_zone_h"] = masks[cell + "_zone_c"] = block
        return masks

    def buf(self, name: str, *shape, dtype=torch.float32, zero: bool = False) -> torch.Tensor:
        n = 1
        for s in shape:
            n *= s
        t = self._ws.get(name)
        if self.guard_bytes > 0:
            if t is None or t.numel() != n or t.dtype != dtype:
                assert all(nm != name for nm, _ in self._cleared.values()), \
                    f"workspace {name}: prezero() and the buf(zero=True) that follows it ask for different sizes"
                t = self._ws[name] = self._guarded(name, n, dtype)
        elif t is None or t.numel() < n or t.dtype != dtype:
            t = torch.empty(max(n, 1), dtype=dtype, device=self.dev)
            self._ws[name] = t
        v = t[:n].view(*shape)
        return self.need_zero(v) if zero else v

    def clear_ahead(self, v: torch.Tensor, name: str = "") -> torch.Tensor:
        assert v.is_contiguous()
        self._cleared[(v.data_ptr(), v.numel() * v.element_size())] = (name, zero_later(v))
        return v

    def need_zero(self, v: torch.Tensor) -> torch.Tensor:
        if not (v.is_contiguous() and self._cleared.pop((v.data_ptr(), v.numel() * v.element_size()), None)):
            zero_later(v)
        return v

    def prezero(self, name: str, *shape, dtype=torch.float32) -> torch.Tensor:
        return self.clear_ahead(self.buf(name, *shape, dtype=dtype), name)

    def gemm_fill(self, A, B, C, M, N, K, lda, ldb, ldc, a_k=1, b_k=1, bias=None):
        if fill_splits(M, N, K) and torch.is_tensor(C):
            self.need_zero(C.view(-1)[:M * ldc])
            gemm(A, B, C, M, N, K, lda, ldb, ldc, a_k=a_k, b_k=b_k, bias=bias, accumulate=2, splitk=2)
        else:
            gemm(A, B, C, M, N, K, lda, ldb, ldc, a_k=a_k, b_k=b_k, bias=bias)

    def fill_ahead(self, C, M, N, K, ldc) -> None:
        if fill_splits(M, N, K):
            self.clear_ahead(C.view(-1)[:M * ldc])

    @staticmethod
    def _record(stream):
        flush_zeros()
        return stream.record_event()

    @staticmethod
    def _wait(stream, other):
        flush_zeros()
        (stream.wait_event if isinstance(other, torch.cuda.Event) else stream.wait_stream)(other)

    def _guarded(self, name: str, n: int, dtype) -> torch.Tensor:
        short = self._guard_short.get(name, 0)
        backing, v, g = _guard.alloc(n, dtype, self.dev, self.guard_bytes, short)
        self._guards[name] = (backing, g, n, short)
        return v

    def out(self, name: str, *shape, zero: bool = False) -> torch.Tensor:
        if self.guard_bytes <= 0:
            return (torch.zeros if zero else torch.empty)(*shape, dtype=torch.float32, device=self.dev)
        n = 1
        for s in shape:
            n *= s
        v = self._guarded("out." + name, n, torch.float32)
        return (v.zero_() if zero else v).view(*shape)

    def workspace_report(self, top: int = 8) -> dict:
        sizes = sorted(((t.numel() * t.element_size(), n) for n, t in self._ws.items()), reverse=True)
        return dict(total_bytes=sum(b for b, _ in sizes), buffers=len(sizes), largest={n: b for b, n in sizes[:top]})

    BN_SLOTS = {"enc.conv0": 0, "enc.conv1": 1, "enc.conv2": 2, "post.conv0": 3, "post.conv1": 4, "post.conv2": 5, "post.conv3": 6,
                "post.conv4": 7}

    def bn_sums(self, tag: str, backward: bool) -> torch.Tensor:
        C = max(self.d["encoded_dim"], self.d["postnet_dim"], self.d["num_mels"])
        arena = self.buf("bn.sums", 16, 2 * C + 2, dtype=torch.float64)
        if tag not in self.BN_SLOTS:
            return zero_later(self.buf(f"{tag}.sums", 2 * C + 2, dtype=torch.float64))
        slot = self.BN_SLOTS[tag] + (8 if backward else 0)
        if slot in self._bn_clean:
            self._bn_clean.discard(slot)
        else:
            zero_later(arena[slot])
        return arena[slot]

    def begin_phase(self, backward: bool):
        self._cleared.clear()
        C = max(self.d["encoded_dim"], self.d["postnet_dim"], self.d["num_mels"])
        arena = self.buf("bn.sums", 16, 2 * C + 2, dtype=torch.float64)
        zero_later(arena[8:] if backward else arena[:8])
        self._bn_clean = (self._bn_clean - set(range(0, 16))) | set(range(8, 16) if backward else range(0, 8))
        if not backward:
            if self._persist_sync is not None:
                zero_later(self._persist_sync[self.PERSIST_RING0:])
            self._persist_next = 0

    PERSIST_RING0 = 320
    PERSIST_RING = 96

    def persist_flag(self) -> int:
        return self.persist_sync().data_ptr() + 4 * 256

    def persist_counters(self, nblocks: int) -> int:
        ring = self.persist_sync()
        if self._persist_next + nblocks > self.PERSIST_RING:
            zero_later(ring[self.PERSIST_RING0:])
            self._persist_next = 0
        a = ring.data_ptr() + 4 * (self.PERSIST_RING0 + 256 * self._persist_next)
        self._persist_next += nblocks
        return a

    def pack_fwd(self, name, segs, H):
        arr = (_lib.S["T2Seg"] * len(segs))()
        ktot = 0
        for i, (w, ld, K) in enumerate(segs):
            arr[i].w = w if isinstance(w, int) else w.data_ptr()
            arr[i].ldw = ld; arr[i].K = K
            ktot += K
        ntpad = (ktot // 16 + 15) // 16 * 16
        out = self.buf("pack." + name, H // 4 * ntpad * 256)
        call("t2_lstm_pack_fwd", arr, len(segs), H, out, _stream())
        return out

    def pack_bwd(self, name, W, ldw, N4, ncols, W2=None, ldw2=0, N2=0):
        tiles = (ncols + 15) // 16
        nchpad = ((N4 + N2) // 16 + 31) // 32 * 32
        out = self.buf("pack." + name, tiles * nchpad * 256)
        call("t2_lstm_pack_bwd", W, ldw, N4, W2, ldw2, N2, ncols, out, _stream())
        return out

    def conv_bn_fwd(self, tag, x_pad, w, bias, bn_prefix, B, L, Ci, Co, act, drop, training, ctx,
                    y=None, Lp_y=None, pad_y=2, res=None, Lp_res=0, pad_res=0, length=None, fill=0.0):
        P, Bf = self.ps.P, self.ps.Bf
        Lp = L + 4
        wp = self.buf(f"{tag}.wp", Co, 5 * Ci)
        call("t2_pack_conv_weight", w, wp, Co, Ci, 5, 0, _stream())
        raw = self.buf(f"{tag}.raw", B * Lp, Co)
        Mg = B * Lp - 4
        tstats = None
        if training and self.bn_epilogue_stats and not fill_splits(Mg, Co, 5 * Ci) and not GEMM_NATIVE_FP32[0]:
            tstats = self.buf(f"{tag}.tstats", (Mg + 127) // 128, 3, Co)
            gemm(x_pad, wp, raw, Mg, Co, 5 * Ci, Ci, 5 * Ci, Co, bias=bias, stat_out=tstats, stat_Lp=Lp, stat_L=L)
        else:
            self.gemm_fill(x_pad, wp, raw, Mg, Co, 5 * Ci, Ci, 5 * Ci, Co, bias=bias)
        mean = self.buf(f"{tag}.mean", Co)
        invstd = self.buf(f"{tag}.invstd", Co)
        sums = self.bn_sums(tag, backward=False)
        if y is None:
            y = self.buf(f"{tag}.y", B, Lp, Co)
            Lp_y = Lp
        sync = training and self.sync_bn_group is not None
        bn = make("T2Bn", B=B, L=L, C=Co, x=raw, Lp_x=Lp, gamma=P[bn_prefix + ".weight"], beta=P[bn_prefix + ".bias"],
                  running_mean=Bf[bn_prefix + ".running_mean"], running_var=Bf[bn_prefix + ".running_var"],
                  training=1 if training else 0, momentum=0.1, eps=1e-5, sums=sums, mean=mean, invstd=invstd, act=act,
                  drop=drop, res=res, Lp_res=Lp_res, pad_res=pad_res, len=length, fill=fill, y=y, Lp_y=Lp_y, pad_y=pad_y,
                  sums_prezeroed=1, tile_stats=tstats, tile_M=Mg if tstats is not None else 0)
        if sync:
            shift = self.buf(f"{tag}.shift", Co)
            shift.copy_(Bf[bn_prefix + ".running_mean"])
            bn.shift = shift.data_ptr(); bn.phase = 1
            call("t2_bn_fwd", bn, _stream())
            import torch.distributed as dist
            dist.all_reduce(sums, group=self.sync_bn_group)
            bn.phase = 2
        call("t2_bn_fwd", bn, _stream())
        if training:
            self.ps.num_batches_tracked[bn_prefix + ".num_batches_tracked"] += 1
        ctx[tag] = dict(x_pad=x_pad, raw=raw, mean=mean, invstd=invstd, drop=drop, wp=wp)
        return y

    def encoder_fwd(self, chars_idx, chars_len32, training, masks, ctx):
        d, P = self.d, self.ps.P
        B, L = chars_idx.shape
        E, H = d["encoded_dim"], d["encoded_dim"] // 2
        Lp = L + 4
        x = self.buf("enc.x0", B, Lp, E)
        for li in range(3):
            self.fill_ahead(self.buf(f"enc.conv{li}.raw", B * Lp, E), B * Lp - 4, E, 5 * E, E)
        call("t2_embedding_fwd", chars_idx, P["encoder.embedding.weight"], x, B, L, E, 2, _stream())
        enc_drop = masks.get("enc_drop") if masks else None
        for li, i in enumerate((0, 4, 8)):
            x = self.conv_bn_fwd(f"enc.conv{li}", x, P[f"encoder.convolutions.{i}.weight"],
                                 P[f"encoder.convolutions.{i}.bias"], f"encoder.convolutions.{i + 1}", B, L, E, E, 1,
                                 enc_drop[li] if enc_drop is not None else None, training, ctx)
        pre = self.buf("enc.pre", B * Lp, 8 * H)
        w_ih = self.ps.cat_view("encoder.lstm.weight_ih_l0", 8 * H, E)
        b_ih = self.ps.cat_view("encoder.lstm.bias_ih_l0", 8 * H, 0)
        b_hh = self.ps.cat_view("encoder.lstm.bias_hh_l0", 8 * H, 0)
        gemm(_ptr(x, 2 * E), w_ih, pre, B * Lp - 4, 8 * H, E, E, E, 8 * H, bias=b_ih, bias2=b_hh)
        S = L
        hs = self.buf("enc.h", 2, S + 1, B, H)
        cs = self.buf("enc.c", 2, S + 1, B, H)
        gs = self.buf("enc.gates", 2, S, B, 4 * H)
        for z in (hs[0, 0], cs[0, 0], hs[1, S], cs[1, S]):
            zero_later(z)
        enc = self.buf("enc.out", B, L, E)
        steps = (_lib.S["T2LstmStep"] * 2)()
        incs = (_lib.S["T2LstmStride"] * 2)()
        persist = B <= self.enc_persist_max_rows and self.enc_chain == "persistent" and H % 16 == 0 and self.persist_resident(H, B, 2)
        ctx["enc_persist"] = persist
        if persist:
            Bp = (B + 15) // 16 * 16
            ht = self.buf("enc.ht", 2, S + 1, H // 16, Bp, 16, zero=(B != Bp))
            zero_later(ht[0, 0]); zero_later(ht[1, S])
        for dr in range(2):
            t0 = 0 if dr == 0 else S - 1
            sg = 1 if dr == 0 else -1
            whh = P["encoder.lstm.weight_hh_l0" + ("" if dr == 0 else "_reverse")]
            slot_in = 0 if dr == 0 else S
            slot_out = 1 if dr == 0 else S - 1
            st = steps[dr]
            st.B, st.H, st.nseg = B, H, 1
            st.wpacked = self.pack_fwd(f"enc.whh{dr}", [(whh, H, H)], H).data_ptr()
            st.seg[0].x = _ptr(hs[dr, slot_in]); st.seg[0].ldx = H
            st.seg[0].w = whh.data_ptr(); st.seg[0].ldw = H; st.seg[0].K = H
            st.pre = _ptr(pre, t0 * 8 * H + dr * 4 * H); st.ldpre = Lp * 8 * H
            st.c_prev = _ptr(cs[dr, slot_in]); st.ldc_prev = H
            st.h_out = _ptr(hs[dr, slot_out]); st.ldh = H
            st.h_out2 = _ptr(enc, t0 * E + dr * H); st.ldh2 = L * E
            st.c_out = _ptr(cs[dr, slot_out]); st.ldc_out = H
            st.gates_out = _ptr(gs[dr, t0]); st.ldg = 4 * H
            st.len = chars_len32.data_ptr(); st.t = t0
            ic = incs[dr]
            ic.seg_x[0] = sg * B * H
            ic.pre = sg * 8 * H; ic.c_prev = sg * B * H; ic.h_out = sg * B * H; ic.h_out2 = sg * E
            ic.c_out = sg * B * H; ic.gates_out = sg * B * 4 * H; ic.dt = sg
            if persist:
                st.xt = _ptr(ht[dr, slot_in]); st.ht_out = _ptr(ht[dr, slot_out]); st.ht_col0 = 0
                ic.xt = sg * H * Bp; ic.ht_out = sg * H * Bp
        self.mark("fwd.enc.convs")
        if persist:
            call("t2_lstm_seq_fwd_persist_pz", steps, incs, 2, S, self.persist_counters((B + 31) // 32), self.persist_flag(), _stream())
            call("t2_guard_poison", self._persist_sync.data_ptr() + 4 * 256, enc, B * L * E, _stream())
        else:
            call("t2_lstm_seq_fwd", steps, incs, 2, S, _stream())
        ctx["enc_stash"] = dict(x3=x, pre=pre, hs=hs, cs=cs, gs=gs, B=B, L=L)
        return enc

    def controls_terms(self, controls, B):
        d, P = self.d, self.ps.P
        C = d.get("controls_dim", 0) if d.get("controls") else 0
        assert (controls is not None) == bool(C), \
            "Controls are enabled, but no control vector was passed to the model!" if C else \
            "Controls are disabled, but a control vector was passed to the model!"
        if not C:
            return None, None, None
        M, D = self.r * d["num_mels"], d["rnn_hidden_dim"]
        ctl = controls.to(self.dev, torch.float32).contiguous()
        assert tuple(ctl.shape) == (B, C), f"controls must be (B, {C})"
        cterm = self.buf("ctl.dec", B, 4 * D)
        gemm(ctl, P["decoder.lstm.weight_ih#controls"], cterm, B, 4 * D, C, C, C, 4 * D)
        cmel1 = self.buf("ctl.mel", B, M + 1, zero=True)
        gemm(ctl, P["decoder.mel_out.weight#controls"], cmel1, B, M, C, C, C, M + 1)
        return ctl, cterm, cmel1

    def condition(self, pf, enc, speaker_id, description_embeddings):
        d, P = self.d, self.ps.P
        B, L, E = enc.shape
        Ef = E + (128 if d.get("description_embeddings") else 0)
        Ad = d["att_dim"]
        st = _stream()
        memory = self.buf(pf + "memory", B, L, Ef)
        desc = None
        if d.get("description_embeddings"):
            desc = self.buf(pf + "desc", B, 128)
            Dd = d["description_embeddings_dim"]
            gemm(description_embeddings, P["description_embeddings_linear.0.weight"], desc, B, 128, Dd, Dd, Dd, 128)
            call("t2_tanh_bias", desc, P["description_embeddings_linear.0.bias"], B, 128, st)
        spk32 = speaker_id.to(torch.int32) if d.get("speaker_tokens") else None
        call("t2_condition_fwd", enc, P["speaker_embedding.weight"] if d.get("speaker_tokens") else None, spk32, desc,
             memory, B, L, E, Ef, st)
        pmT = self.buf(pf + "pmT", B, Ad, L)
        gemm(P["att_encoder.weight"], memory, pmT, Ad, L, Ef, Ef, Ef, L, batch=B, sA=0, sB=L * Ef, sC=Ad * L)
        return memory, desc, spk32, pmT

    def postnet_fwd(self, post_in, post, mlen32, B, T, post_drop, training, ctx):
        d, P = self.d, self.ps.P
        M, Pn = d["num_mels"], d["postnet_dim"]
        chans = [M, Pn, Pn, Pn, Pn, M]
        x = post_in
        for li in range(5):
            last = li == 4
            x = self.conv_bn_fwd(f"post.conv{li}", x, P[f"postnet.postnet.{4 * li}.weight"], None,
                                 f"postnet.postnet.{4 * li + 1}", B, T, chans[li], chans[li + 1], 0 if last else 2,
                                 post_drop[li] if post_drop is not None else None, training, ctx,
                                 y=post if last else None, Lp_y=T if last else None, pad_y=0 if last else 2,
                                 res=post_in if last else None, Lp_res=T + 4, pad_res=2,
                                 length=mlen32 if last else None, fill=0.0)

    def forward_tf(self, chars_idx, chars_len, mel, mel_len, speaker_id=None, description_embeddings=None,
                   training=True, masks: Optional[dict] = None, save_for_backward=True, controls=None, forward_attention=False):
        forward_attention = check_forward_attention(forward_attention)
        d, P, ps = self.d, self.ps.P, self.ps
        masks = masks or {}
        B, L = chars_idx.shape
        Tf, M = mel.shape[1], d["num_mels"]
        r = self.r
        T, Mr = (Tf + r - 1) // r, r * M
        E, Pd, A, D, Ad = d["encoded_dim"], d["prenet_dim"], d["att_rnn_dim"], d["rnn_hidden_dim"], d["att_dim"]
        Ef = E + (128 if d.get("description_embeddings") else 0)
        F = d.get("loc_filters", 32)
        ctx: dict = dict(B=B, L=L, T=Tf, S=T, r=r, forward_attention=forward_attention)
        self.generation += 1
        ctx["generation"] = self.generation
        st = _stream()
        len32 = chars_len.to(torch.int32)
        mlen32 = mel_len.to(torch.int32)
        ctx["len32"], ctx["mlen32"], ctx["chars_idx"] = len32, mlen32, chars_idx

        self.begin_phase(backward=False)
        self.mark("start")
        main0, side0 = torch.cuda.current_stream(), self.side_stream()
        self._wait(side0, main0)
        with torch.cuda.stream(side0):
            mel_tm = self.buf("mel_tm", T + 1, B, M)
            call("t2_mel_to_tm_r", mel, mel_tm, B, Tf, M, r, _stream())
            pd = masks.get("prenet_drop")
            p1 = self.buf("p1", T + 1, B, Pd)
            p2 = self.buf("p2", T + 1, B, Pd)
            R1 = (T + 1) * B
            gemm(mel_tm, P["prenet.0.weight"], p1, R1, Pd, M, M, M, Pd, relu=1, mulmask=pd[0] if pd else None, ldmask=Pd)
            gemm(p1, P["prenet.3.weight"], p2, R1, Pd, Pd, Pd, Pd, Pd, relu=1, mulmask=pd[1] if pd else None, ldmask=Pd)
            R = T * B
            pre_att = self.buf("pre_att", T, B, 4 * A)
            sp0 = self.span_begin()
            gemm(p2, P["decoder.att_rnn.weight_ih"], pre_att, R, 4 * A, Pd, Pd, Pd + Ef, 4 * A,
                 bias=P["decoder.att_rnn.bias_ih"], bias2=P["decoder.att_rnn.bias_hh"])
            self.span_end("fwd.dec.pre_att_gemm.side_stream", sp0)
        enc = self.encoder_fwd(chars_idx, len32, training, masks, ctx)
        self.mark("fwd.enc.bilstm")

        memory, desc, spk32, pmT = self.condition("", enc, speaker_id, description_embeddings)
        ctx.update(enc=enc, memory=memory, desc=desc, spk32=spk32, desc_in=description_embeddings)

        self.mark("fwd.condition")
        self._wait(main0, side0)
        self.mark("fwd.dec.pre_att_gemm")
        U = self.buf("U", Ad, 2, KL)
        call("t2_attn_fold_location", P["decoder.attention.location_dense.weight"],
             P["decoder.attention.location_conv.weight"], U, Ad, F, KL, st)
        xdec = self.buf("xdec", T + 1, B, A + Ef)
        zero_later(xdec[0])
        att_c = self.buf("att_c", T + 1, B, A)
        zero_later(att_c[0])
        cum = self.buf("cum", T + 1, B, L)
        zero_later(cum[0])
        xproj = self.buf("xproj", T + 1, B, D + Ef)
        zero_later(xproj[0])
        Bp = (B + 15) // 16 * 16
        xdec_t = self.buf("xdec_t", T + 1, (A + Ef) // 16, Bp, 16, zero=(B != Bp))
        zero_later(xdec_t[0])
        dech_t = self.buf("dech_t", T + 1, D // 16, Bp, 16, zero=(B != Bp))
        zero_later(dech_t[0])
        gates_att = self.buf("gates_att", T, B, 4 * A) if save_for_backward else None
        th = self.buf("th", T, B, Ad, (L + 3) // 4 * 4) if save_for_backward else None
        align = self.out("align", B, T, L)
        e_part = self.buf("e_part", B, Ad // 16, L)
        wp_att = self.pack_fwd("att", [(P["decoder.att_rnn.weight_hh"], A, A),
                                       (_ptr(P["decoder.att_rnn.weight_ih"], Pd), Pd + Ef, Ef)], A)
        seq = make("T2AttnSeq", B=B, L=L, T=T, A=A, Ad=Ad, Ef=Ef, Kl=KL, wpacked=wp_att,
                   W_ih_ctx=_ptr(P["decoder.att_rnn.weight_ih"], Pd), ld_wih=Pd + Ef,
                   W_hh=P["decoder.att_rnn.weight_hh"], Wq=P["decoder.attention.query_layer.weight"], U=U,
                   v=P["decoder.attention.v.weight"], pre=pre_att, pmT=pmT, memory=memory, len=len32,
                   att_drop=masks.get("att_drop"), xdec=xdec, att_c=att_c, gates=gates_att, align=align, cum=cum, th=th,
                   xproj_ctx=_ptr(xproj, B * (D + Ef) + D), ld_xproj=D + Ef, e_part=e_part, xdec_t=xdec_t,
                   forward=int(forward_attention))
        azh, azc = masks.get("att_zone_h"), masks.get("att_zone_c")
        zatt = make("T2AttnZone", zone_h=azh, zone_c=azc, stride=zone_stride(azh if azh is not None else azc, B * A)) \
            if azh is not None or azc is not None else None
        pre_dec = self.buf("pre_dec", T, B, 4 * D)
        dec_c = self.buf("dec_c", T + 1, B, D)
        zero_later(dec_c[0])
        gates_dec = self.buf("gates_dec", T, B, 4 * D) if save_for_backward else None
        dd = masks.get("dec_drop")
        dzh, dzc = masks.get("dec_zone_h"), masks.get("dec_zone_c")
        dzs = zone_stride(dzh if dzh is not None else dzc, B * D)
        ldp = D + Ef
        wp_dec = self.pack_fwd("dec", [(P["decoder.lstm.weight_hh"], D, D)], D)

        def dec_chunk(c0, c1):
            stp = make("T2LstmStep", B=B, H=D, nseg=1, wpacked=wp_dec, pre=_ptr(pre_dec, c0 * B * 4 * D), ldpre=4 * D,
                       c_prev=_ptr(dec_c, c0 * B * D), ldc_prev=D,
                       drop=_ptr(dd, c0 * B * D) if dd is not None else None, lddrop=D,
                       h_out=_ptr(xproj, (c0 + 1) * B * ldp), ldh=ldp, c_out=_ptr(dec_c, (c0 + 1) * B * D), ldc_out=D,
                       gates_out=_ptr(gates_dec, c0 * B * 4 * D) if gates_dec is not None else None, ldg=4 * D,
                       xt=_ptr(dech_t, c0 * D * Bp), ht_out=_ptr(dech_t, (c0 + 1) * D * Bp), ht_col0=0,
                       zone_h=_ptr(dzh, c0 * dzs) if dzh is not None else None, ldzone_h=D,
                       zone_c=_ptr(dzc, c0 * dzs) if dzc is not None else None, ldzone_c=D,
                       h_prev=_ptr(xproj, c0 * B * ldp) if dzh is not None or dzc is not None else None, ldh_prev=ldp)
            stp.seg[0].x = _ptr(xproj, c0 * B * ldp); stp.seg[0].ldx = ldp
            stp.seg[0].w = P["decoder.lstm.weight_hh"].data_ptr(); stp.seg[0].ldw = D; stp.seg[0].K = D
            inc = make("T2LstmStride", pre=B * 4 * D, c_prev=B * D, drop=B * D, h_out=B * ldp, c_out=B * D,
                       gates_out=B * 4 * D, dt=0, xt=D * Bp, ht_out=D * Bp, zone_h=dzs, zone_c=dzs, h_prev=B * ldp)
            inc.seg_x[0] = B * ldp
            return stp, inc

        ctl, cterm, cmel1 = self.controls_terms(controls, B)

        def pre_dec_gemm(c0, c1, sk, cleared):
            if cterm is not None:
                pre_dec[c0:c1].copy_(cterm.unsqueeze(0).expand(c1 - c0, B, 4 * D))
            if cleared:
                self.need_zero(pre_dec[c0:c1])
            gemm(_ptr(xdec, (c0 + 1) * B * (A + Ef)), P["decoder.lstm.weight_ih"], _ptr(pre_dec, c0 * B * 4 * D), (c1 - c0) * B,
                 4 * D, A + Ef, A + Ef, A + Ef, 4 * D, bias=P["decoder.lstm.bias_ih"], bias2=P["decoder.lstm.bias_hh"],
                 accumulate=2 if sk > 1 else (1 if cterm is not None else 0), splitk=sk)

        main, side = torch.cuda.current_stream(), self.side_stream()
        sched = forward_schedule(T, self.chunk, B, D, self.ramp_chunks, self.splitk_small_chunks, cterm is not None)
        for c0, c1, sk, cleared in sched:
            if cleared:
                self.clear_ahead(pre_dec[c0:c1])
        self._wait(side, main)
        persist = B <= 64 and self.dec_chain == "persistent" and D // 4 <= 256 and self.persist_resident(D, B)
        ctx["persist"] = persist
        sync = self.persist_sync() if persist else None
        for c0, c1, sk, cleared in sched:
            seq.t_begin, seq.t_end = c0, c1
            if zatt is not None:
                call("t2_attn_seq_fwd_zone", seq, zatt, st)
            else:
                call("t2_attn_seq_fwd", seq, st)
            ev = self._record(main)
            with torch.cuda.stream(side):
                self._wait(side, ev)
                with share_cu(self.share_cu if persist else 0):
                    pre_dec_gemm(c0, c1, sk, cleared)
                stp, inc = dec_chunk(c0, c1)
                if persist:
                    call("t2_lstm_seq_fwd_persist_pz", stp, inc, 1, c1 - c0, self.persist_counters((B + 31) // 32), self.persist_flag(),
                         side.cuda_stream)
                else:
                    call("t2_lstm_seq_fwd", stp, inc, 1, c1 - c0, side.cuda_stream)
        self.mark("fwd.dec.attn_chain")
        self._wait(main, side)
        self.mark("fwd.dec.lstm_chain_tail")

        wproj = ps.cat_view("decoder.mel_out.weight", Mr + 1, D + Ef)
        bproj = ps.cat_view("decoder.mel_out.bias", Mr + 1, 0)
        proj = self.buf("proj", T, B, Mr + 1)
        if cmel1 is not None:
            proj.copy_(cmel1.unsqueeze(0).expand(T, B, Mr + 1))
        gemm(_ptr(xproj, B * ldp), wproj, proj, R, Mr + 1, ldp, ldp, ldp, Mr + 1, bias=bproj,
             accumulate=1 if cmel1 is not None else 0)
        if persist:
            call("t2_guard_poison", self._persist_sync.data_ptr() + 4 * 256, proj, R * (Mr + 1), st)
        self.mark("fwd.dec.proj_gemm")
        mels = self.out("mels", B, Tf, M)
        gates = self.out("gates", B, Tf, 1)
        post_in = self.buf("post.x0", B, Tf + 4, M)
        call("t2_finalize_fwd_r", proj, Mr + 1, mlen32, mels, gates, post_in, B, Tf, M, r, st)

        post = self.out("post", B, Tf, M)
        self.postnet_fwd(post_in, post, mlen32, B, Tf, masks.get("post_drop"), training, ctx)
        self.mark("fwd.postnet")
        ctx.update(controls=ctl, pmT=pmT, mel_tm=mel_tm, p1=p1, p2=p2, pd=pd, pre_att=pre_att, U=U, xdec=xdec, att_c=att_c, cum=cum,
                   xproj=xproj, gates_att=gates_att, th=th, align=align, pre_dec=pre_dec, dec_c=dec_c,
                   gates_dec=gates_dec, proj=proj, post_in=post_in, masks=masks, training=training)
        return (mels, post, gates, align), ctx

    def _wgrad(self, dY, ldy, X, ldx, Cgrad, ldc, Mout, Nin, R):
        gemm(dY, X, Cgrad, Mout, Nin, R, ldy, ldx, ldc, a_k=0, b_k=0, accumulate=2, splitk=splitk_for(Mout, Nin, R))

    def conv_bn_bwd(self, tag, ctx, dy, Lp_dy, pad_dy, w, gw, gbias, bn_prefix, B, L, Ci, Co, act, training, need_dx=True,
                    defer=None, wgrad_stream=None):
        P, G = self.ps.P, self.ps.G
        c = ctx[tag]
        Lp = L + 4
        st = _stream()
        draw = self.buf(f"{tag}.draw", B, Lp, Co)
        sums = self.bn_sums(tag, backward=True)
        bn = make("T2Bn", B=B, L=L, C=Co, x=c["raw"], Lp_x=Lp, gamma=P[bn_prefix + ".weight"], beta=P[bn_prefix + ".bias"],
                  training=1 if training else 0, momentum=0.1, eps=1e-5, sums=sums, sums_prezeroed=1, mean=c["mean"], invstd=c["invstd"],
                  act=act, drop=c["drop"], dy=dy, Lp_dy=Lp_dy, pad_dy=pad_dy, dx=draw, Lp_dx=Lp, pad_dx=2,
                  dgamma=G[bn_prefix + ".weight"], dbeta=G[bn_prefix + ".bias"])
        if training and self.sync_bn_group is not None:
            import torch.distributed as dist
            bn.phase = 1
            call("t2_bn_bwd", bn, st)
            dist.all_reduce(sums, group=self.sync_bn_group)
            bn.phase = 2; bn.grad_share = 1.0 / dist.get_world_size(self.sync_bn_group)
        call("t2_bn_bwd", bn, st)
        R = B * Lp - 4
        if gbias is not None:
            call("t2_colsum", draw, Co, B * Lp, Co, gbias, st)
        def wgrad():
            dwp = self.buf(f"{tag}.dwp", Co, 5 * Ci, zero=True)
            self._wgrad(_ptr(draw, 2 * Co), Co, c["x_pad"], Ci, dwp, 5 * Ci, Co, 5 * Ci, R)
            call("t2_unpack_conv_wgrad", dwp, gw, Co, Ci, 5, _stream())
        if defer is not None:
            defer.append(wgrad)
        else:
            ev = self._record(torch.cuda.current_stream())
            with torch.cuda.stream(wgrad_stream):
                self._wait(wgrad_stream, ev)
                wgrad()
        if not need_dx:
            return None
        wf = self.buf(f"{tag}.wf", Ci, 5 * Co)
        call("t2_pack_conv_weight", w, wf, Co, Ci, 5, 1, st)
        dx = self.buf(f"{tag}.dx", B * Lp, Ci)
        self.gemm_fill(draw, wf, dx, R, Ci, 5 * Co, Co, 5 * Co, Ci)
        return dx

    def backward_tf(self, ctx, d_post, dproj, d_align=None):
        d, P, G, ps = self.d, self.ps.P, self.ps.G, self.ps
        if ctx.get("generation") != self.generation:
            raise RuntimeError("backward of a stale forward: the activation stashes of this forward were overwritten by a later "
                               "grad-enabled forward of the same model (one live teacher-forced graph per model; INTEGRATION.md)")
        B, L, Tf = ctx["B"], ctx["L"], ctx["T"]
        r = ctx["r"]
        T = ctx["S"]
        if d_align is not None:
            if not isinstance(d_align, torch.Tensor) or d_align.dtype != torch.float32:
                raise ValueError("backward_tf: d_align must be a float32 tensor, got "
                                 f"{d_align.dtype if isinstance(d_align, torch.Tensor) else type(d_align).__name__}")
            if tuple(d_align.shape) != (B, T, L):
                raise ValueError(f"backward_tf: d_align has shape {tuple(d_align.shape)}, the alignments {(B, T, L)}")
            if not d_align.is_contiguous():
                raise ValueError("backward_tf: d_align must be contiguous")
            if d_align.device != ctx["align"].device:
                raise ValueError(f"backward_tf: d_align is on {d_align.device}, the engine on {ctx['align'].device}")
        M, E, Pd, A, D, Ad = d["num_mels"], d["encoded_dim"], d["prenet_dim"], d["att_rnn_dim"], d["rnn_hidden_dim"], d["att_dim"]
        Mr = r * M
        Ef = E + (128 if d.get("description_embeddings") else 0)
        F = d.get("loc_filters", 32)
        H = E // 2
        Pn = d["postnet_dim"]
        st = _stream()
        training = ctx["training"]
        masks = ctx["masks"]
        R, R1 = T * B, (T + 1) * B
        ldp, ldx = D + Ef, A + Ef
        self.begin_phase(backward=True)
        chans = [M, Pn, Pn, Pn, Pn, M]
        for li in range(5):
            self.prezero(f"post.conv{li}.dwp", chans[li + 1], 5 * chans[li])
        Lp_e = L + 4
        for li in range(3):
            self.prezero(f"enc.conv{li}.dwp", E, 5 * E)
            self.fill_ahead(self.buf(f"enc.conv{li}.dx", B * Lp_e, E), B * Lp_e - 4, E, 5 * E, E)
        self.fill_ahead(self.buf("enc.dx3", B * Lp_e, E), B * Lp_e - 4, E, 8 * H, E)

        dy, Lp_dy = d_post, Tf
        post_wgrads = []
        for li in range(4, -1, -1):
            dy = self.conv_bn_bwd(f"post.conv{li}", ctx, dy, Lp_dy, 0, P[f"postnet.postnet.{4 * li}.weight"],
                                  G[f"postnet.postnet.{4 * li}.weight"], None, f"postnet.postnet.{4 * li + 1}", B, Tf,
                                  chans[li], chans[li + 1], 0 if li == 4 else 2, training, defer=post_wgrads)
            Lp_dy = Tf + 4
        call("t2_finalize_bwd_r", dy, dproj, B, Tf, M, r, st)
        self.mark("bwd.postnet")

        xproj, xdec = ctx["xproj"], ctx["xdec"]
        wproj = ps.cat_view("decoder.mel_out.weight", Mr + 1, ldp)
        dxproj = self.buf("dxproj", T, B, ldp)
        gemm(dproj, wproj, dxproj, R, ldp, Mr + 1, Mr + 1, ldp, ldp, a_k=1, b_k=0)
        ctl = ctx.get("controls")

        def proj_wgrads():
            self._wgrad(dproj, Mr + 1, _ptr(xproj, B * ldp), ldp, ps.cat_view("decoder.mel_out.weight", Mr + 1, ldp, grad=True),
                        ldp, Mr + 1, ldp, R)
            call("t2_colsum", dproj, Mr + 1, R, Mr + 1, ps.cat_view("decoder.mel_out.bias", Mr + 1, 0, grad=True), _stream())
            if ctl is not None:
                C = ctl.shape[1]
                s_proj = self.buf("ctl.dproj_sum", B, Mr + 1, zero=True)
                call("t2_colsum", dproj, B * (Mr + 1), T, B * (Mr + 1), s_proj, _stream())
                self._wgrad(s_proj, Mr + 1, ctl, C, G["decoder.mel_out.weight#controls"], C, Mr, C, B)
        post_wgrads.append(proj_wgrads)

        dgd = self.buf("dgd", T + 1, B, 4 * D)
        zero_later(dgd[T])
        Bp = (B + 15) // 16 * 16
        dgd_t = self.buf("dgd_t", T + 1, 4 * D // 16, Bp, 16)
        zero_later(dgd_t[T])
        Zt = self.buf("Zatt_t", T + 1, 4 * A // 16, Bp, 16)
        zero_later(Zt[T])
        dc_dec = self.buf("dc_dec", B, D, zero=True)
        dd = masks.get("dec_drop")
        dzh, dzc = masks.get("dec_zone_h"), masks.get("dec_zone_c")
        azh, azc = masks.get("att_zone_h"), masks.get("att_zone_c")
        dzs = zone_stride(dzh if dzh is not None else dzc, B * D)
        dhz_dec = self.buf("dhz_dec", B, D, zero=True) if dzh is not None or dzc is not None else None
        dhz_att = self.buf("dhz_att", B, A, zero=True) if azh is not None or azc is not None else None
        wtp_dec = self.pack_bwd("dec.t", P["decoder.lstm.weight_hh"], D, 4 * D, D)
        dxdec = self.buf("dxdec", T, B, ldx)
        ldz = 4 * A + Ad
        Z = self.buf("Zatt", T + 1, B, ldz)
        zero_later(Z[T, :, :4 * A])
        dga = Z
        dctx_tot = self.buf("dctx_tot", T, B, Ef)
        dpmT = self.buf("dpmT", B, Ad, L, zero=True)
        dv_part = self.buf("dv_part", B, Ad, zero=True)
        dU_part = self.buf("dU_part", B, Ad * 2 * KL, zero=True)
        dc_att = self.buf("dc_att", B, A, zero=True)
        Gc = self.buf("Gcum", 2, B, L)
        de = self.buf("de", B, L)
        de_stash = self.buf("de_stash", T, B, L) if L <= 252 else None
        din_part = self.buf("din_part", B, Ad // 16, 2, L)
        wtp_ctx = self.pack_bwd("att.ctx.t", _ptr(P["decoder.att_rnn.weight_ih"], Pd), Pd + Ef, 4 * A, Ef)
        wtp_h = self.pack_bwd("att.h.t", P["decoder.att_rnn.weight_hh"], A, 4 * A, A)
        wtp_q = self.pack_bwd("att.q.t", P["decoder.attention.query_layer.weight"], A, Ad, A)
        dh_rec = self.buf("dh_rec", B, A)
        fwd_att = bool(ctx.get("forward_attention"))
        dprior = self.buf("dprior", 2, B, L) if fwd_att else None
        sb = make("T2AttnSeqBwd", B=B, L=L, T=T, A=A, Ad=Ad, Ef=Ef, Kl=KL, wtp_ctx=wtp_ctx, wtp_h=wtp_h, wtp_q=wtp_q,
                  dh_rec=dh_rec,
                  W_ih_ctx=_ptr(P["decoder.att_rnn.weight_ih"], Pd), ld_wih=Pd + Ef, W_hh=P["decoder.att_rnn.weight_hh"],
                  Wq=P["decoder.attention.query_layer.weight"], U=ctx["U"], v=P["decoder.attention.v.weight"],
                  memory=ctx["memory"], xdec=xdec, att_c=ctx["att_c"], gates=ctx["gates_att"], align=ctx["align"],
                  cum=ctx["cum"], th=ctx["th"], att_drop=masks.get("att_drop"),
                  dh_ext=dxdec, ld_dh=ldx, dctx_ext1=_ptr(dxdec, A), ld_dc1=ldx, dctx_ext2=_ptr(dxproj, D), ld_dc2=ldp,
                  dgates=Z, dctx_tot=dctx_tot, dq=None, dpmT=dpmT, dv_part=dv_part, dU_part=dU_part,
                  dc=dc_att, G=Gc, de=de, din_part=din_part, dgates_t=Zt, clk=getattr(self, "clk_bwd", None), dalign=d_align,
                  ws_bd=self.buf("attn.ws_bd", Ad // 16 * 16896))
        zatt = make("T2AttnZone", zone_h=azh, zone_c=azc, stride=zone_stride(azh if azh is not None else azc, B * A), dhz=dhz_att) \
            if dhz_att is not None else None
        self.mark("bwd.dec.proj")
        main, side = torch.cuda.current_stream(), self.side_stream()
        self._wait(side, main)

        def dec_bwd_chunk(hi, lo):
            s = make("T2LstmBwdStep", B=B, H=D, N4=4 * D, dg_next=_ptr(dgd, hi * B * 4 * D), lddg=4 * D,
                     W=P["decoder.lstm.weight_hh"], ldw=D, wtpacked=wtp_dec, ncols=D, epi=1,
                     ext1=_ptr(dxproj, (hi - 1) * B * ldp), ldx1=ldp,
                     drop=_ptr(dd, (hi - 1) * B * D) if dd is not None else None, lddrop=D,
                     gates=_ptr(ctx["gates_dec"], (hi - 1) * B * 4 * D), ldgs=4 * D,
                     c_prev=_ptr(ctx["dec_c"], (hi - 1) * B * D), ldcp=D, c_cur=_ptr(ctx["dec_c"], hi * B * D), ldcc=D,
                     dc=dc_dec, lddc=D, dg_out=_ptr(dgd, (hi - 1) * B * 4 * D), ldgo=4 * D,
                     dgt_next=_ptr(dgd_t, hi * Bp * 4 * D), dgt_out=_ptr(dgd_t, (hi - 1) * Bp * 4 * D),
                     off_chain=1 if self.bptt_off_chain else 0,
                     zone_h=_ptr(dzh, (hi - 1) * dzs) if dzh is not None else None, ldzone_h=D,
                     zone_c=_ptr(dzc, (hi - 1) * dzs) if dzc is not None else None, ldzone_c=D, dhz=dhz_dec, lddhz=D)
            inc = make("T2LstmBwdStride", dg=-B * 4 * D, ext1=-B * ldp, drop=-B * D, gates=-B * 4 * D, c_prev=-B * D,
                       c_cur=-B * D, dt=0, dgt=-Bp * 4 * D, zone_h=-dzs, zone_c=-dzs)
            return s, inc

        def dec_wgrads_chunk(hi, lo):
            n = (hi - lo) * B
            g0 = _ptr(dgd, lo * B * 4 * D)
            self._wgrad(g0, 4 * D, _ptr(xdec, (lo + 1) * B * ldx), ldx, G["decoder.lstm.weight_ih"], ldx, 4 * D, ldx, n)
            self._wgrad(g0, 4 * D, _ptr(xproj, lo * B * ldp), ldp, G["decoder.lstm.weight_hh"], D, 4 * D, D, n)

        gWih = G["decoder.att_rnn.weight_ih"]

        def att_wgrads(hi, lo):
            n = (hi - lo) * B
            z0 = _ptr(Z, lo * B * ldz)
            self._wgrad(z0, ldz, _ptr(ctx["p2"], lo * B * Pd), Pd, gWih, Pd + Ef, 4 * A, Pd, n)
            self._wgrad(z0, ldz, _ptr(xdec, lo * B * ldx + A), ldx, _ptr(gWih, Pd), Pd + Ef, 4 * A, Ef, n)
            self._wgrad(z0, ldz, _ptr(xdec, lo * B * ldx), ldx, G["decoder.att_rnn.weight_hh"], A, 4 * A, A, n)
            self._wgrad(_ptr(Z, (lo + 1) * B * ldz + 4 * A), ldz, _ptr(xdec, (lo + 1) * B * ldx), ldx,
                        G["decoder.attention.query_layer.weight"], A, Ad, A, n)
        sched = backward_schedule(T, self.chunk_bwd, max(1, int(self.wgrad_group)), len(post_wgrads), de_stash is not None,
                                  self.ramp_chunks)
        done = []

        def att_acc(hi, lo):
            call("t2_attn_acc_bwd", sb, de_stash, B * L, lo, hi, side.cuda_stream)
        run = dict(dec_wgrads=dec_wgrads_chunk, att_acc=att_acc, att_wgrads=att_wgrads, deferred=lambda hi, lo: post_wgrads.pop(0)())

        def side_op(op):
            if op.k >= 0:
                self._wait(side, done[op.k])
            run[op.kind](op.hi, op.lo)
        for hi, lo, ops in sched.chunks:
            with torch.cuda.stream(side), share_cu(self.share_cu):
                s, inc = dec_bwd_chunk(hi, lo)
                call("t2_lstm_seq_bwd", s, inc, 1, hi - lo, side.cuda_stream)
                gemm(_ptr(dgd, lo * B * 4 * D), P["decoder.lstm.weight_ih"], _ptr(dxdec, lo * B * ldx), (hi - lo) * B, ldx, 4 * D,
                     4 * D, ldx, ldx, a_k=1, b_k=0)
                ev = self._record(side)
                for op in ops:
                    side_op(op)
            self._wait(main, ev)
            sb.t_hi, sb.t_lo = hi, lo
            if zatt is not None:
                call("t2_attn_seq_bwd_zone", sb, de_stash, B * L, dprior, zatt, st)
            elif fwd_att:
                call("t2_attn_seq_bwd_forward", sb, de_stash, B * L, dprior, st)
            else:
                call("t2_attn_seq_bwd_stash", sb, de_stash, B * L, st)
            done.append(self._record(main))
        with torch.cuda.stream(side):
            for op in sched.tail:
                if op.kind == "acc_done":
                    acc_done = self._record(side)
                    continue
                with share_cu(self.share_cu) if op.share else contextlib.nullcontext():
                    side_op(op)
            db = self.buf("db_dec", 4 * D, zero=True)
            call("t2_colsum", dgd, 4 * D, R, 4 * D, db, side.cuda_stream)
            for nm in ("decoder.lstm.bias_ih", "decoder.lstm.bias_hh"):
                call("t2_colsum", db, 4 * D, 1, 4 * D, G[nm], side.cuda_stream)
            if ctl is not None:
                s_dgd = self.buf("ctl.dgd_sum", B, 4 * D, zero=True)
                call("t2_colsum", dgd, B * 4 * D, T, B * 4 * D, s_dgd, side.cuda_stream)
                self._wgrad(s_dgd, 4 * D, ctl, ctl.shape[1], G["decoder.lstm.weight_ih#controls"], ctl.shape[1], 4 * D,
                            ctl.shape[1], B)
        self.mark("bwd.dec.chains")

        dmem = self.buf("dmem", B, L, Ef)
        gemm(ctx["align"], dctx_tot, dmem, L, Ef, T, L, B * Ef, Ef, a_k=0, b_k=0, batch=B, sA=T * L, sB=Ef, sC=L * Ef)
        Watt = P["att_encoder.weight"]
        self._wait(main, acc_done)
        gemm(dpmT, Watt, dmem, L, Ef, Ad, L, Ef, Ef, a_k=0, b_k=0, accumulate=1, batch=B, sA=Ad * L, sB=0, sC=L * Ef)

        self._wait(side, main)
        with torch.cuda.stream(side):
            sst = side.cuda_stream
            db = self.buf("db_att", 4 * A, zero=True)
            call("t2_colsum", dga, ldz, R, 4 * A, db, sst)
            for nm in ("decoder.att_rnn.bias_ih", "decoder.att_rnn.bias_hh"):
                call("t2_colsum", db, 4 * A, 1, 4 * A, G[nm], sst)
            call("t2_colsum", dv_part, Ad, B, Ad, G["decoder.attention.v.weight"], sst)
            dU = self.buf("dU", Ad, 2 * KL, zero=True)
            call("t2_colsum", dU_part, Ad * 2 * KL, B, Ad * 2 * KL, dU, sst)
            Wd, Wc = P["decoder.attention.location_dense.weight"], P["decoder.attention.location_conv.weight"]
            gemm(dU, Wc, G["decoder.attention.location_dense.weight"], Ad, F, 2 * KL, 2 * KL, 2 * KL, F, accumulate=1)
            gemm(Wd, dU, G["decoder.attention.location_conv.weight"], F, 2 * KL, Ad, F, 2 * KL, 2 * KL, a_k=0, b_k=0,
                 accumulate=1)
            gemm(dpmT, ctx["memory"], G["att_encoder.weight"], Ad, Ef, L, L, Ef, Ef, a_k=1, b_k=0, accumulate=2, batch=B,
                 sA=Ad * L, sB=L * Ef, sC=0)
            dp2 = self.buf("dp2", T + 1, B, Pd)
            zero_later(dp2[T])
            gemm(dga, P["decoder.att_rnn.weight_ih"], dp2, R, Pd, 4 * A, ldz, Pd + Ef, Pd, a_k=1, b_k=0)
            pd = ctx["pd"]
            g2 = self.buf("g2", T + 1, B, Pd)
            call("t2_relu_mask_bwd", dp2, ctx["p2"], pd[1] if pd else None, g2, R1 * Pd, sst)
            self._wgrad(g2, Pd, ctx["p1"], Pd, G["prenet.3.weight"], Pd, Pd, Pd, R1)
            dp1 = self.buf("dp1", T + 1, B, Pd)
            gemm(g2, P["prenet.3.weight"], dp1, R1, Pd, Pd, Pd, Pd, Pd, a_k=1, b_k=0)
            g1 = self.buf("g1", T + 1, B, Pd)
            call("t2_relu_mask_bwd", dp1, ctx["p1"], pd[0] if pd else None, g1, R1 * Pd, sst)
            self._wgrad(g1, Pd, ctx["mel_tm"], M, G["prenet.0.weight"], M, Pd, M, R1)
            if self.grad_tail_hook is not None:
                self.grad_tail_hook()
        self.mark("bwd.dec.attn_gemms")

        denc = self.buf("denc", B, L, E)
        ddesc = self.buf("ddesc", B, 128, zero=True) if d.get("description_embeddings") else None
        call("t2_condition_bwd", dmem, ctx["memory"], ctx["spk32"], denc,
             G["speaker_embedding.weight"] if d.get("speaker_tokens") else None, ddesc, B, L, E, Ef, st)
        if ddesc is not None:
            Dd = d["description_embeddings_dim"]
            dlin = self.buf("dlin", B, 128)
            call("t2_tanh_bwd", ddesc, ctx["desc"], dlin, B * 128, st)
            self._wgrad(dlin, 128, ctx["desc_in"], Dd, G["description_embeddings_linear.0.weight"], Dd, 128, Dd, B)
            call("t2_colsum", dlin, 128, B, 128, G["description_embeddings_linear.0.bias"], st)

        e = ctx["enc_stash"]
        S, Lp = L, L + 4
        hs, cs, gs = e["hs"], e["cs"], e["gs"]
        dgt = self.buf("enc.dgt", 2, S + 1, B, 4 * H)
        zero_later(dgt[0, S]); zero_later(dgt[1, 0])
        dpre = self.buf("enc.dpre", B * Lp, 8 * H, zero=True)
        dc_enc = self.buf("enc.dc", 2, B, H, zero=True)
        steps = (_lib.S["T2LstmBwdStep"] * 2)()
        incs = (_lib.S["T2LstmBwdStride"] * 2)()
        len32 = ctx["len32"]
        for dr in range(2):
            sg = -1 if dr == 0 else 1
            t0 = S - 1 if dr == 0 else 0
            whh = P["encoder.lstm.weight_hh_l0" + ("" if dr == 0 else "_reverse")]
            sp = steps[dr]
            sp.B, sp.H, sp.N4, sp.ncols, sp.epi = B, H, 4 * H, H, 1
            sp.W = whh.data_ptr(); sp.ldw = H
            sp.wtpacked = self.pack_bwd(f"enc.whh{dr}.t", whh, H, 4 * H, H).data_ptr()
            sp.ext1 = _ptr(denc, t0 * E + dr * H); sp.ldx1 = L * E
            sp.gates = _ptr(gs[dr, t0]); sp.ldgs = 4 * H
            sp.c_prev = _ptr(cs[dr, t0 if dr == 0 else t0 + 1]); sp.ldcp = H
            sp.c_cur = _ptr(cs[dr, t0 + 1 if dr == 0 else t0]); sp.ldcc = H
            sp.dc = _ptr(dc_enc[dr]); sp.lddc = H
            sp.dg_next = _ptr(dgt[dr, S if dr == 0 else 0]); sp.lddg = 4 * H
            sp.dg_out = _ptr(dgt[dr, t0 if dr == 0 else t0 + 1]); sp.ldgo = 4 * H
            sp.dg_out2 = _ptr(dpre, t0 * 8 * H + dr * 4 * H); sp.ldgo2 = Lp * 8 * H
            sp.len = len32.data_ptr(); sp.t = t0
            ic = incs[dr]
            ic.dg = sg * B * 4 * H; ic.dg2 = sg * 8 * H; ic.ext1 = sg * E; ic.gates = sg * B * 4 * H
            ic.c_prev = sg * B * H; ic.c_cur = sg * B * H; ic.dt = sg
        call("t2_lstm_seq_bwd", steps, incs, 2, S, st)
        Rr = B * Lp - 4
        x3 = e["x3"]

        def bilstm_wgrads():
            for dr in range(2):
                nm = "encoder.lstm.weight_hh_l0" + ("" if dr == 0 else "_reverse")
                hprev = hs[0, 0] if dr == 0 else hs[1, 1]
                self._wgrad(_ptr(dgt[dr, 0 if dr == 0 else 1]), 4 * H, hprev, H, G[nm], H, 4 * H, H, S * B)
            self._wgrad(dpre, 8 * H, _ptr(x3, 2 * E), E, ps.cat_view("encoder.lstm.weight_ih_l0", 8 * H, E, grad=True), E, 8 * H, E, Rr)
            call("t2_colsum", dpre, 8 * H, B * Lp, 8 * H, ps.cat_view("encoder.lstm.bias_ih_l0", 8 * H, 0, grad=True), _stream())
            call("t2_colsum", dpre, 8 * H, B * Lp, 8 * H, ps.cat_view("encoder.lstm.bias_hh_l0", 8 * H, 0, grad=True), _stream())
        ev = self._record(main)
        with torch.cuda.stream(side):
            self._wait(side, ev)
            bilstm_wgrads()
        dx = self.buf("enc.dx3", B * Lp, E)
        self.gemm_fill(dpre, ps.cat_view("encoder.lstm.weight_ih_l0", 8 * H, E), dx, Rr, E, 8 * H, 8 * H, E, E, a_k=1, b_k=0)

        self.mark("bwd.bilstm")
        for li, i in reversed(list(enumerate((0, 4, 8)))):
            dx = self.conv_bn_bwd(f"enc.conv{li}", ctx, dx, Lp, 0, P[f"encoder.convolutions.{i}.weight"],
                                  G[f"encoder.convolutions.{i}.weight"], G[f"encoder.convolutions.{i}.bias"],
# ... 342 lines not shown
```

tacotron2_amd/trainer.py:

```python
from __future__ import annotations

from typing import Optional, Sequence

import torch
import torch.distributed as dist

from .engine import Engine, check_forward_attention, check_guided_attention, check_loss_options, zero_later
from .params import ParamStore


class Trainer:
    def __init__(self, ps: ParamStore, lr: float, weight_decay: float, scheduler_milestones: Sequence[int] = (),
                 max_norm: float = 1.0, seed: int = 1234, sync_bn: bool = False, overlap_allreduce: bool = False,
                 force_collectives: bool = False, shape_timeout_s: float = 300.0, guided_attention=None,
                 forward_attention: bool = False, loss_options=None):
        self.ps = ps
        self.engine = Engine(ps)
        self.guided_attention = check_guided_attention(guided_attention)
        self.forward_attention = check_forward_attention(forward_attention)
        self.loss_options = check_loss_options(loss_options)
        self.last_guided_loss = None
        self.base_lr, self.weight_decay, self.max_norm = lr, weight_decay, max_norm
        self.milestones = sorted(int(m) for m in scheduler_milestones)
        self.global_step = 0
        self.seed = seed
        self.world = dist.get_world_size() if dist.is_available() and dist.is_initialized() else 1
        self.rank = dist.get_rank() if self.world > 1 else 0
        self.dp = self.world > 1 or (bool(force_collectives) and dist.is_available() and dist.is_initialized())
        self.frozen: set = set()
        self.sync_bn = bool(sync_bn) and self.dp
        if self.sync_bn:
            self.engine.sync_bn_group = dist.group.WORLD
        self.overlap_allreduce = bool(overlap_allreduce) and self.dp and not self.sync_bn
        self._tail_start = ps.offsets["prenet.0.weight"]
        self._tail_work = None
        if self.overlap_allreduce:
            self.engine.grad_tail_hook = self._start_tail_allreduce
        self._shape_group = None
        self.queue_check = None
        if self.dp:
            import datetime
            try:
                self._shape_group = dist.new_group(backend="gloo", timeout=datetime.timedelta(seconds=shape_timeout_s))
            except Exception as e:
                import warnings
                warnings.warn(f"Trainer: no gloo group for the shape negotiation ({e}); the padded shape of every step is agreed on "
                              "the main thread over the default process group (one host synchronisation per step)")
            if ps.device.type == "cuda":
                self.queue_check = self.engine.ensure_concurrent_streams()
                if not self.queue_check["ok"]:
                    import warnings
                    warnings.warn("Trainer: the engine's main and side streams do NOT run concurrently in this process "
                                  f"({self.queue_check}): every new side stream landed on the main stream's hardware queue.  Set GPU_MAX_HW_QUEUES=16 (or more) in the "
                                  "environment BEFORE the first GPU call of the process (import tacotron2_amd first); every "
                                  "training step will otherwise be ~35 % slower.")

    def _start_tail_allreduce(self):
        self._tail_work = dist.all_reduce(self.ps.grad[self._tail_start:], async_op=True)

    def trainable_ranges(self):
        ps = self.ps
        if not self.frozen:
            return [(0, ps.numel)]
        names = list(ps.offsets)
        ranges = []
        for i, name in enumerate(names):
            if name in self.frozen:
                continue
            a = ps.offsets[name]
            b = ps.offsets[names[i + 1]] if i + 1 < len(names) else ps.numel
            if ranges and ranges[-1][1] == a:
                ranges[-1] = (ranges[-1][0], b)
            else:
                ranges.append((a, b))
        return ranges

    def lr_at(self, step: int) -> float:
        return self.base_lr * (0.1 ** sum(1 for m in self.milestones if step >= m))

    def negotiate_shape(self, L: int, T: int):
        if not self.dp:
            return int(L), int(T)
        if self._shape_group is not None:
            lt = torch.tensor([int(L), int(T)], dtype=torch.int64)
            dist.all_reduce(lt, op=dist.ReduceOp.MAX, group=self._shape_group)
        else:
            lt = torch.tensor([int(L), int(T)], dtype=torch.int64, device=self.ps.device)
            dist.all_reduce(lt, op=dist.ReduceOp.MAX)
            lt = lt.cpu()
        return int(lt[0]), int(lt[1])

    @staticmethod
    def pad_to(batch: dict, Lg: int, Tg: int) -> dict:
        out = dict(batch)
        L = batch["chars_idx"].shape[1]
        T = batch["mel_spectrogram"].shape[1]
        if L < Lg:
            out["chars_idx"] = torch.nn.functional.pad(batch["chars_idx"], (0, Lg - L))
        if T < Tg:
            out["mel_spectrogram"] = torch.nn.functional.pad(batch["mel_spectrogram"], (0, 0, 0, Tg - T))
            out["gate"] = torch.nn.functional.pad(batch["gate"], (0, 0, 0, Tg - T))
        return out

    def global_pad(self, batch: dict) -> dict:
        if not self.dp:
            return batch
        Lg, Tg = self.negotiate_shape(batch["chars_idx"].shape[1], batch["mel_spectrogram"].shape[1])
        return self.pad_to(batch, Lg, Tg)

    @property
    def loader_negotiation(self) -> bool:
        return self.dp and self._shape_group is not None

    def negotiate_collated(self, collated):
        if not self.dp:
            return collated
        if hasattr(collated, "set_global_shape"):
            collated.set_global_shape(*self.negotiate_shape(collated.L, collated.T))
            return collated
        data, meta, extra = collated
        if self._shape_group is None:
            raise RuntimeError("Trainer.negotiate_collated needs the host-side (gloo) group: without it the shape is agreed on the "
                               "main thread (train_step(padded=False)); see Trainer.loader_negotiation")
        Lg, Tg = self.negotiate_shape(data["chars_idx"].shape[1], data["mel_spectrogram"].shape[1])
        return self.pad_to(data, Lg, Tg), meta, extra

    def train_step(self, batch: dict, masks: Optional[dict] = None, padded: bool = False):
        eng, ps = self.engine, self.ps
        if not padded:
            batch = self.global_pad(batch)
        ci, mel = batch["chars_idx"], batch["mel_spectrogram"]
        B, L = ci.shape
        T = mel.shape[1]
        eng.marks = []; eng.spans = []
        if masks is None:
            masks = eng.make_masks(B, L, T, True, self.seed + 7919 * self.rank, self.global_step)
        eng.mark("masks")
        outs, ctx = eng.forward_tf(ci, batch["chars_idx_len"], mel, batch["mel_spectrogram_len"],
                                   speaker_id=batch.get("speaker_id"),
                                   description_embeddings=batch.get("description_embeddings"), training=True, masks=masks,
                                   controls=batch.get("controls"), forward_attention=self.forward_attention)
        zero_later(ps.grad)
        loss3 = eng.loss_and_grads(outs, ctx, mel, batch["gate"], guided=self.guided_attention, loss=self.loss_options)
        self.last_guided_loss = eng.guided_loss
        if self.dp:
            if self._tail_work is not None:
                dist.all_reduce(ps.grad[:self._tail_start])
                self._tail_work.wait()
                self._tail_work = None
            else:
                dist.all_reduce(ps.grad)
            eng.mark("allreduce")
        for name in self.frozen:
            zero_later(ps.G[name])
        self.global_step += 1
        eng.adam_step(self.global_step, self.lr_at(self.global_step - 1), self.weight_decay, self.max_norm,
                      grad_scale=1.0 / self.world, ranges=self.trainable_ranges() if self.frozen else None)
        eng.mark("optimizer")
        return loss3, outs
```

Baseline: 296,100.

## Generate conv dropout masks inside BN kernels and batch mask and weight-pack launches

Conv-layer dropout masks are no longer written to memory. The BN forward and backward kernels now regenerate them on the fly from Philox using the seed, stream and rate, through new vectorised apply, reduce and backward kernels. The remaining masks are produced by one multi-region Philox launch on the side stream, and all conv weight packing (forward and flipped) is batched into a single multi-entry launch up front. This removes mask memory traffic and many small kernel launches, in exchange for recomputing Philox twice per element in backward and adding a C%4 constraint.

```diff
diff --git a/include/tacotron2_amd.h b/include/tacotron2_amd.h
--- a/include/tacotron2_amd.h
+++ b/include/tacotron2_amd.h
@@ -181,6 +181,13 @@
 int t2_embedding_bwd(const int64_t* idx, const float* dout, float* dtable, int B, int L, int E, int Lp, int pad, void* stream);
 int t2_pack_conv_weight(const float* w, float* wp, int Co, int Ci, int K, int flip, void* stream);
 int t2_unpack_conv_wgrad(const float* gp, float* g, int Co, int Ci, int K, void* stream);
+typedef struct {
+    const float* w[16];
+    float* wp[16];
+    int Co[16], Ci[16], K[16], flip[16];
+    int count;
+} T2ConvPacks;
+int t2_pack_conv_weights(const T2ConvPacks* p, void* stream);
 
 typedef struct {
     int B, L, C;
@@ -201,6 +208,8 @@
     int phase; const float* shift; float grad_share;
     int sums_prezeroed;
     const float* tile_stats; int tile_M;
+    uint64_t drop_seed, drop_stream;
+    float drop_rate;
 } T2Bn;
 int t2_bn_fwd(const T2Bn* s, void* stream);
 int t2_bn_bwd(const T2Bn* s, void* stream);
@@ -344,6 +353,16 @@
 
 int t2_philox_mask(float* out, int64_t n, float p, uint64_t seed, uint64_t stream_id, void* stream);
 int t2_philox_bernoulli(float* out, int64_t n, float p, uint64_t seed, uint64_t stream_id, void* stream);
+typedef struct {
+    float* out[8];
+    int64_t n[8];
+    float rate[8];
+    uint64_t stream_id[8];
+    int kind[8];
+    uint64_t seed;
+    int count;
+} T2PhiloxMasks;
+int t2_philox_masks(const T2PhiloxMasks* m, void* stream);
 int t2_sumsq(const float* g, int64_t n, double* out, void* stream);
 int t2_adam_step(float* p, const float* g, float* m, float* v, int64_t n, const double* sumsq, float max_norm, float lr,
                  float beta1, float beta2, float eps, float weight_decay, int step, float grad_scale, void* stream);
diff --git a/tacotron2_amd/csrc/t2_common.hpp b/tacotron2_amd/csrc/t2_common.hpp
--- a/tacotron2_amd/csrc/t2_common.hpp
+++ b/tacotron2_amd/csrc/t2_common.hpp
@@ -179,3 +179,13 @@
     }
     out[0] = c0; out[1] = c1; out[2] = c2; out[3] = c3;
 }
+
+__device__ __forceinline__ float t2_keep_scale(float p) { return 1.f / (1.f - p); }
+__device__ __forceinline__ float t2_mask_value(uint32_t word, float p, float keep_scale, bool bernoulli = false) {
+    const float u = (float)(word >> 8) * (1.0f / 16777216.0f);
+    return bernoulli ? (u < p ? 1.f : 0.f) : (u < p ? 0.f : keep_scale);
+}
+__device__ __forceinline__ void t2_mask_words(long quad, uint64_t seed, uint64_t stream_id, uint32_t r[4]) {
+    t2_philox4((uint32_t)quad, (uint32_t)(quad >> 32), (uint32_t)stream_id, (uint32_t)(stream_id >> 32), (uint32_t)seed,
+               (uint32_t)(seed >> 32), r);
+}
diff --git a/tacotron2_amd/csrc/t2_elementwise.hip b/tacotron2_amd/csrc/t2_elementwise.hip
--- a/tacotron2_amd/csrc/t2_elementwise.hip
+++ b/tacotron2_amd/csrc/t2_elementwise.hip
@@ -68,6 +68,7 @@
     float* dx; int Lp_dx, pad_dx;
     float* dgamma; float* dbeta;
     double grad_share;
+    uint64_t drop_seed, drop_stream; float drop_rate;
 };
 
 __global__ __launch_bounds__(256) void bn_stats_kernel(BnK p, int rows_per_block) {
@@ -255,6 +256,151 @@
     }
 }
 
+template <bool VEC> __device__ __forceinline__ void bn_ld4(const float* q, float v[4]) {
+    if (VEC) { const f32x4 t = *(const f32x4*)q; v[0] = t.x; v[1] = t.y; v[2] = t.z; v[3] = t.w; }
+    else { v[0] = q[0]; v[1] = q[1]; v[2] = q[2]; v[3] = q[3]; }
+}
+template <bool VEC> __device__ __forceinline__ void bn_st4(float* q, const float v[4]) {
+    if (VEC) { f32x4 t; t.x = v[0]; t.y = v[1]; t.z = v[2]; t.w = v[3]; *(f32x4*)q = t; }
+    else { q[0] = v[0]; q[1] = v[1]; q[2] = v[2]; q[3] = v[3]; }
+}
+__device__ __forceinline__ float bn_mul_rn(float a, float b) {
+#pragma clang fp contract(off)
+    return a * b;
+}
+__device__ __forceinline__ float bn_add_rn(float a, float b) {
+#pragma clang fp contract(off)
+    return a + b;
+}
+__device__ __forceinline__ void bn_scale4(const BnK& p, int b, int l, int c, float s[4]) {
+    const long e = ((long)b * p.L + l) * p.C + c;
+    uint32_t r[4];
+    t2_mask_words(e >> 2, p.drop_seed, p.drop_stream, r);
+    const float keep_scale = t2_keep_scale(p.drop_rate);
+#pragma unroll
+    for (int j = 0; j < 4; ++j) s[j] = t2_mask_value(r[j], p.drop_rate, keep_scale);
+}
+
+template <bool VEC> __global__ __launch_bounds__(256) void bn_apply4_kernel(BnK p) {
+    const int C4 = p.C >> 2;
+    const long n = (long)p.B * p.Lp_y * C4;
+    for (long i = (long)blockIdx.x * blockDim.x + threadIdx.x; i < n; i += (long)gridDim.x * blockDim.x) {
+        const int c = (int)(i % C4) * 4;
+        const long row = i / C4;
+        const int lp = (int)(row % p.Lp_y), b = (int)(row / p.Lp_y);
+        const int l = lp - p.pad_y;
+        float v[4] = {0.f, 0.f, 0.f, 0.f};
+        if (l >= 0 && l < p.L) {
+            float xv[4], m[4], is[4], ga[4], be[4], s[4], rs[4] = {0.f, 0.f, 0.f, 0.f};
+            bn_ld4<VEC>(p.x + ((long)b * p.Lp_x + l) * p.C + c, xv);
+            bn_ld4<VEC>(p.mean + c, m); bn_ld4<VEC>(p.invstd + c, is); bn_ld4<VEC>(p.gamma + c, ga); bn_ld4<VEC>(p.beta + c, be);
+            if (p.res) bn_ld4<VEC>(p.res + ((long)b * p.Lp_res + p.pad_res + l) * p.C + c, rs);
+            bn_scale4(p, b, l, c, s);
+            const bool cut = p.len && l >= p.len[b];
+#pragma unroll
+            for (int j = 0; j < 4; ++j) {
+                float t = (xv[j] - m[j]) * is[j] * ga[j] + be[j];
+                if (p.act == 1) t = fmaxf(t, 0.f);
+                else if (p.act == 2) t = t2_tanh(t);
+                t = bn_mul_rn(t, s[j]);
+                if (p.res) t = bn_add_rn(t, rs[j]);
+                if (cut) t = p.fill;
+                v[j] = t;
+            }
+        }
+        bn_st4<VEC>(p.y + i * 4, v);
+    }
+}
+
+template <bool VEC> __device__ __forceinline__ void bn_dz4(const BnK& p, int b, int l, int c, const float m[4], const float is[4],
+                                                           const float ga[4], const float be[4], float xhat[4], float dz[4]) {
+    float xv[4], g[4], s[4];
+    bn_ld4<VEC>(p.x + ((long)b * p.Lp_x + l) * p.C + c, xv);
+    bn_ld4<VEC>(p.dy + ((long)b * p.Lp_dy + p.pad_dy + l) * p.C + c, g);
+    bn_scale4(p, b, l, c, s);
+#pragma unroll
+    for (int j = 0; j < 4; ++j) {
+        xhat[j] = (xv[j] - m[j]) * is[j];
+        float gj = bn_mul_rn(g[j], s[j]);
+        const float pre = xhat[j] * ga[j] + be[j];
+        if (p.act == 1) gj = pre > 0.f ? gj : 0.f;
+        else if (p.act == 2) { const float t = t2_tanh(pre); gj *= (1.f - t * t); }
+        dz[j] = gj;
+    }
+}
+
+template <bool VEC> __global__ __launch_bounds__(256) void bn_bwd_reduce4_kernel(BnK p) {
+    __shared__ f32x4 s1[4][4][16], s2[4][4][16];
+    const int cq = threadIdx.x & 15, rl = (threadIdx.x >> 4) & 3, sub = threadIdx.x >> 6;
+    const int c = (blockIdx.x * 16 + cq) * 4;
+    const long R = (long)p.B * p.L;
+    const long r0 = ((long)blockIdx.y * 4 + sub) * 128;
+    long r1 = r0 + 128; if (r1 > R) r1 = R;
+    float a[4] = {0.f, 0.f, 0.f, 0.f}, q[4] = {0.f, 0.f, 0.f, 0.f};
+    if (blockIdx.x == 0 && blockIdx.y == 0 && threadIdx.x == 0) atomicAdd(&p.sums[2 * p.C], (double)R);
+    if (c < p.C && r0 < R) {
+        float m[4], is[4], ga[4], be[4];
+        bn_ld4<VEC>(p.mean + c, m); bn_ld4<VEC>(p.invstd + c, is); bn_ld4<VEC>(p.gamma + c, ga); bn_ld4<VEC>(p.beta + c, be);
+        int b = (int)((r0 + rl) / p.L), l = (int)((r0 + rl) % p.L);
+#pragma unroll 4
+        for (long r = r0 + rl; r < r1; r += 4, l += 4) {
+            while (l >= p.L) { l -= p.L; ++b; }
+            float xh[4], dz[4];
+            bn_dz4<VEC>(p, b, l, c, m, is, ga, be, xh, dz);
+#pragma unroll
+            for (int j = 0; j < 4; ++j) { a[j] += dz[j]; q[j] = fmaf(dz[j], xh[j], q[j]); }
+        }
+    }
+    f32x4 ta, tq;
+    ta.x = a[0]; ta.y = a[1]; ta.z = a[2]; ta.w = a[3]; tq.x = q[0]; tq.y = q[1]; tq.z = q[2]; tq.w = q[3];
+    s1[sub][rl][cq] = ta; s2[sub][rl][cq] = tq;
+    __syncthreads();
+    if (rl == 0 && c < p.C && r0 < R) {
+        const f32x4 u0 = s1[sub][0][cq], u1 = s1[sub][1][cq], u2 = s1[sub][2][cq], u3 = s1[sub][3][cq];
+        const f32x4 w0 = s2[sub][0][cq], w1 = s2[sub][1][cq], w2 = s2[sub][2][cq], w3 = s2[sub][3][cq];
+        atomicAdd(&p.sums[c + 0], (double)u0.x + u1.x + u2.x + u3.x);
+        atomicAdd(&p.sums[c + 1], (double)u0.y + u1.y + u2.y + u3.y);
+        atomicAdd(&p.sums[c + 2], (double)u0.z + u1.z + u2.z + u3.z);
+        atomicAdd(&p.sums[c + 3], (double)u0.w + u1.w + u2.w + u3.w);
+        atomicAdd(&p.sums[p.C + c + 0], (double)w0.x + w1.x + w2.x + w3.x);
+        atomicAdd(&p.sums[p.C + c + 1], (double)w0.y + w1.y + w2.y + w3.y);
+        atomicAdd(&p.sums[p.C + c + 2], (double)w0.z + w1.z + w2.z + w3.z);
+        atomicAdd(&p.sums[p.C + c + 3], (double)w0.w + w1.w + w2.w + w3.w);
+    }
+}
+
+template <bool VEC> __global__ __launch_bounds__(256) void bn_bwd_apply4_kernel(BnK p) {
+    const int C4 = p.C >> 2;
+    const long n = (long)p.B * p.Lp_dx * C4;
+    const float invn = (float)(1.0 / p.sums[2 * p.C]);
+    for (long i = (long)blockIdx.x * blockDim.x + threadIdx.x; i < n; i += (long)gridDim.x * blockDim.x) {
+        const int c = (int)(i % C4) * 4;
+        const long row = i / C4;
+        const int lp = (int)(row % p.Lp_dx), b = (int)(row / p.Lp_dx);
+        const int l = lp - p.pad_dx;
+        float v[4] = {0.f, 0.f, 0.f, 0.f};
+        if (l >= 0 && l < p.L) {
+            float m[4], is[4], ga[4], be[4], xh[4], dz[4];
+            bn_ld4<VEC>(p.mean + c, m); bn_ld4<VEC>(p.invstd + c, is); bn_ld4<VEC>(p.gamma + c, ga); bn_ld4<VEC>(p.beta + c, be);
+            bn_dz4<VEC>(p, b, l, c, m, is, ga, be, xh, dz);
+#pragma unroll
+            for (int j = 0; j < 4; ++j) {
+                const float gi = ga[j] * is[j];
+                if (p.training) v[j] = gi * (dz[j] - (float)p.sums[c + j] * invn - xh[j] * (float)p.sums[p.C + c + j] * invn);
+                else v[j] = gi * dz[j];
+            }
+        }
+        bn_st4<VEC>(p.dx + i * 4, v);
+        if (lp == 0 && b == 0) {
+#pragma unroll
+            for (int j = 0; j < 4; ++j) {
+                p.dbeta[c + j] += (float)(p.sums[c + j] * p.grad_share);
+                p.dgamma[c + j] += (float)(p.sums[p.C + c + j] * p.grad_share);
+            }
+        }
+    }
+}
+
 void to_bnk(const T2Bn* s, BnK& k) {
     k.B = s->B; k.L = s->L; k.C = s->C; k.x = s->x; k.Lp_x = s->Lp_x; k.gamma = s->gamma; k.beta = s->beta;
     k.rmean = s->running_mean; k.rvar = s->running_var; k.training = s->training; k.momentum = s->momentum; k.eps = s->eps;
@@ -263,6 +409,14 @@
     k.y = s->y; k.Lp_y = s->Lp_y; k.pad_y = s->pad_y; k.dy = s->dy; k.Lp_dy = s->Lp_dy; k.pad_dy = s->pad_dy;
     k.dx = s->dx; k.Lp_dx = s->Lp_dx; k.pad_dx = s->pad_dx; k.dgamma = s->dgamma; k.dbeta = s->dbeta;
     k.shift = s->shift; k.grad_share = s->grad_share > 0.f ? (double)s->grad_share : 1.0;
+    k.drop_seed = s->drop_seed; k.drop_stream = s->drop_stream; k.drop_rate = s->drop_rate;
+}
+
+inline bool bn_lazy(const T2Bn* s) { return !s->drop && s->drop_rate > 0.f; }
+inline bool bn_vec4(const T2Bn* s, bool backward) {
+    bool ok = t2_aligned16(s->x) && t2_aligned16(s->gamma) && t2_aligned16(s->beta) && t2_aligned16(s->mean) && t2_aligned16(s->invstd);
+    if (backward) return ok && t2_aligned16(s->dy) && t2_aligned16(s->dx);
+    return ok && t2_aligned16(s->y) && (!s->res || t2_aligned16(s->res));
 }
 
 inline int ew_grid(long n) { long g = (n + 255) / 256; return (int)(g > 4096 ? 4096 : (g < 1 ? 1 : g)); }
@@ -594,19 +748,15 @@
 }
 
 __global__ void philox_mask_kernel(float* out, long n, float p, uint64_t seed, uint64_t stream_id) {
-    const float keep_scale = 1.f / (1.f - p);
+    const float keep_scale = t2_keep_scale(p);
     const long n4 = (n + 3) / 4;
     for (long i = (long)blockIdx.x * blockDim.x + threadIdx.x; i < n4; i += (long)gridDim.x * blockDim.x) {
         uint32_t r[4];
-        t2_philox4((uint32_t)i, (uint32_t)(i >> 32), (uint32_t)stream_id, (uint32_t)(stream_id >> 32), (uint32_t)seed,
-                   (uint32_t)(seed >> 32), r);
+        t2_mask_words(i, seed, stream_id, r);
 #pragma unroll
         for (int j = 0; j < 4; ++j) {
             const long e = 4 * i + j;
-            if (e < n) {
-                const float u = (float)(r[j] >> 8) * (1.0f / 16777216.0f);
-                out[e] = u < p ? 0.f : keep_scale;
-            }
+            if (e < n) out[e] = t2_mask_value(r[j], p, keep_scale);
         }
     }
 }
@@ -615,13 +765,57 @@
     const long n4 = (n + 3) / 4;
     for (long i = (long)blockIdx.x * blockDim.x + threadIdx.x; i < n4; i += (long)gridDim.x * blockDim.x) {
         uint32_t r[4];
-        t2_philox4((uint32_t)i, (uint32_t)(i >> 32), (uint32_t)stream_id, (uint32_t)(stream_id >> 32), (uint32_t)seed,
-                   (uint32_t)(seed >> 32), r);
+        t2_mask_words(i, seed, stream_id, r);
 #pragma unroll
         for (int j = 0; j < 4; ++j) {
             const long e = 4 * i + j;
-            if (e < n) out[e] = (float)(r[j] >> 8) * (1.0f / 16777216.0f) < p ? 1.f : 0.f;
-        }
+            if (e < n) out[e] = t2_mask_value(r[j], p, 0.f, true);
+        }
+    }
+}
+
+struct MasksK { T2PhiloxMasks m; };
+__global__ __launch_bounds__(256) void philox_masks_kernel(MasksK k) {
+    const int y = blockIdx.y;
+    float* out = k.m.out[y];
+    const long n = k.m.n[y];
+    const float p = k.m.rate[y];
+    const uint64_t sid = k.m.stream_id[y];
+    const bool bern = k.m.kind[y] != 0;
+    const float keep_scale = t2_keep_scale(p);
+    const bool vec = (((uintptr_t)out) & 15) == 0;
+    const long n4 = (n + 3) / 4;
+    for (long i = (long)blockIdx.x * blockDim.x + threadIdx.x; i < n4; i += (long)gridDim.x * blockDim.x) {
+        uint32_t r[4];
+        t2_mask_words(i, k.m.seed, sid, r);
+        if (vec && 4 * i + 3 < n) {
+            f32x4 v;
+            v.x = t2_mask_value(r[0], p, keep_scale, bern); v.y = t2_mask_value(r[1], p, keep_scale, bern);
+            v.z = t2_mask_value(r[2], p, keep_scale, bern); v.w = t2_mask_value(r[3], p, keep_scale, bern);
+            *(f32x4*)(out + 4 * i) = v;
+        } else {
+#pragma unroll
+            for (int j = 0; j < 4; ++j) {
+                const long e = 4 * i + j;
+                if (e < n) out[e] = t2_mask_value(r[j], p, keep_scale, bern);
+            }
+        }
+    }
+}
+
+struct PacksK { T2ConvPacks c; };
+__global__ __launch_bounds__(256) void pack_conv_ws_kernel(PacksK k) {
+    const int y = blockIdx.y;
+    const float* w = k.c.w[y];
+    float* wp = k.c.wp[y];
+    const int Co = k.c.Co[y], Ci = k.c.Ci[y], K = k.c.K[y], flip = k.c.flip[y];
+    const long n = (long)Co * Ci * K;
+    for (long i = (long)blockIdx.x * blockDim.x + threadIdx.x; i < n; i += (long)gridDim.x * blockDim.x) {
+        const int kk = (int)(i % K);
+        const int ci = (int)((i / K) % Ci);
+        const int co = (int)(i / ((long)K * Ci));
+        if (!flip) wp[(long)co * K * Ci + (long)kk * Ci + ci] = w[i];
+        else wp[(long)ci * K * Co + (long)(K - 1 - kk) * Co + co] = w[i];
     }
 }
 
@@ -757,6 +951,22 @@
     hipLaunchKernelGGL(pack_conv_w_kernel, dim3(ew_grid((long)Co * Ci * K)), dim3(256), 0, ST, w, wp, Co, Ci, K, flip);
     T2_CHECK_LAUNCH(); return T2_OK;
 }
+extern "C" int t2_pack_conv_weights(const T2ConvPacks* p, void* stream) {
+    (void)hipGetLastError();
+    T2_REQUIRE(p && p->count >= 0 && p->count <= 16, "t2_pack_conv_weights: 0..16 entries");
+    if (p->count == 0) return T2_OK;
+    long most = 0;
+    for (int i = 0; i < p->count; ++i) {
+        T2_REQUIRE(p->w[i] && p->wp[i] && p->Co[i] > 0 && p->Ci[i] > 0 && p->K[i] > 0, "t2_pack_conv_weights: null or empty entry");
+        const long n = (long)p->Co[i] * p->Ci[i] * p->K[i];
+        if (n > most) most = n;
+    }
+    long gx = (most + 256 * 4 - 1) / (256 * 4);
+    gx = gx < 1 ? 1 : (gx > 1024 ? 1024 : gx);
+    PacksK k; k.c = *p;
+    hipLaunchKernelGGL(pack_conv_ws_kernel, dim3((unsigned)gx, p->count), dim3(256), 0, ST, k);
+    T2_CHECK_LAUNCH(); return T2_OK;
+}
 extern "C" int t2_unpack_conv_wgrad(const float* gp, float* g, int Co, int Ci, int K, void* stream) {
     (void)hipGetLastError();
     T2_REQUIRE(gp && g, "t2_unpack_conv_wgrad: null");
@@ -770,6 +980,7 @@
     T2_REQUIRE(s->training ? (s->sums != nullptr) : (s->running_mean && s->running_var), "t2_bn_fwd: stats operands");
     T2_REQUIRE(s->phase >= 0 && s->phase <= 2 && (s->phase == 0 || (s->training && s->shift)),
                "t2_bn_fwd: phases 1/2 (sync-BN) need training statistics and a rank-independent shift");
+    T2_REQUIRE(!bn_lazy(s) || (s->C % 4 == 0 && s->drop_rate < 1.f), "t2_bn_fwd: a generated mask needs C % 4 == 0 and a rate below 1");
     BnK k; to_bnk(s, k);
     if (s->training && s->phase != 2) {
         if (s->tile_stats) {
@@ -784,7 +995,12 @@
     }
     if (s->phase != 1) {
         hipLaunchKernelGGL(bn_finalize_kernel, dim3(t2_cdiv(s->C, 256)), dim3(256), 0, ST, k);
-        hipLaunchKernelGGL(bn_apply_kernel, dim3(ew_grid((long)s->B * s->Lp_y * s->C)), dim3(256), 0, ST, k);
+        if (!bn_lazy(s)) hipLaunchKernelGGL(bn_apply_kernel, dim3(ew_grid((long)s->B * s->Lp_y * s->C)), dim3(256), 0, ST, k);
+        else {
+            const dim3 g4(ew_grid((long)s->B * s->Lp_y * (s->C / 4)));
+            if (bn_vec4(s, false)) hipLaunchKernelGGL(bn_apply4_kernel<true>, g4, dim3(256), 0, ST, k);
+            else hipLaunchKernelGGL(bn_apply4_kernel<false>, g4, dim3(256), 0, ST, k);
+        }
     }
     T2_CHECK_LAUNCH(); return T2_OK;
 }
@@ -794,14 +1010,29 @@
     T2_REQUIRE(s && s->x && s->gamma && s->beta && s->mean && s->invstd && s->dy && s->dx && s->sums && s->dgamma && s->dbeta,
                "t2_bn_bwd: null operand");
     T2_REQUIRE(s->phase >= 0 && s->phase <= 2, "t2_bn_bwd: bad phase");
+    T2_REQUIRE(!bn_lazy(s) || (s->C % 4 == 0 && s->drop_rate < 1.f), "t2_bn_bwd: a generated mask needs C % 4 == 0 and a rate below 1");
     BnK k; to_bnk(s, k);
+    const bool lazy = bn_lazy(s), vec = lazy && bn_vec4(s, true);
     if (s->phase != 2) {
         if (!s->sums_prezeroed) (void)hipMemsetAsync(s->sums, 0, sizeof(double) * (2 * s->C + 2), ST);
         const long R = (long)s->B * s->L;
-        const int rpb = 128;
-        hipLaunchKernelGGL(bn_bwd_reduce_kernel, dim3(t2_cdiv(s->C, 64), t2_cdiv(R, rpb)), dim3(256), 0, ST, k, rpb);
-    }
-    if (s->phase != 1) hipLaunchKernelGGL(bn_bwd_apply_kernel, dim3(ew_grid((long)s->B * s->Lp_dx * s->C)), dim3(256), 0, ST, k);
+        if (!lazy) {
+            const int rpb = 128;
+            hipLaunchKernelGGL(bn_bwd_reduce_kernel, dim3(t2_cdiv(s->C, 64), t2_cdiv(R, rpb)), dim3(256), 0, ST, k, rpb);
+        } else {
+            const dim3 g4(t2_cdiv(s->C, 64), t2_cdiv(t2_cdiv(R, 128), 4));
+            if (vec) hipLaunchKernelGGL(bn_bwd_reduce4_kernel<true>, g4, dim3(256), 0, ST, k);
+            else hipLaunchKernelGGL(bn_bwd_reduce4_kernel<false>, g4, dim3(256), 0, ST, k);
+        }
+    }
+    if (s->phase != 1) {
+        if (!lazy) hipLaunchKernelGGL(bn_bwd_apply_kernel, dim3(ew_grid((long)s->B * s->Lp_dx * s->C)), dim3(256), 0, ST, k);
+        else {
+            const dim3 g4(ew_grid((long)s->B * s->Lp_dx * (s->C / 4)));
+            if (vec) hipLaunchKernelGGL(bn_bwd_apply4_kernel<true>, g4, dim3(256), 0, ST, k);
+            else hipLaunchKernelGGL(bn_bwd_apply4_kernel<false>, g4, dim3(256), 0, ST, k);
+        }
+    }
     T2_CHECK_LAUNCH(); return T2_OK;
 }
 
@@ -1067,6 +1298,23 @@
     hipLaunchKernelGGL(philox_bernoulli_kernel, dim3(ew_grid((n + 3) / 4)), dim3(256), 0, ST, out, (long)n, p, seed, stream_id);
     T2_CHECK_LAUNCH(); return T2_OK;
 }
+extern "C" int t2_philox_masks(const T2PhiloxMasks* m, void* stream) {
+    (void)hipGetLastError();
+    T2_REQUIRE(m && m->count >= 0 && m->count <= 8, "t2_philox_masks: 0..8 regions");
+    long most = 0;
+    for (int i = 0; i < m->count; ++i) {
+        T2_REQUIRE(m->n[i] >= 0 && (m->out[i] || m->n[i] == 0) && ((uintptr_t)m->out[i] & 3) == 0 && m->rate[i] >= 0.f &&
+                   (m->kind[i] == 0 ? m->rate[i] < 1.f : (m->kind[i] == 1 && m->rate[i] <= 1.f)),
+                   "t2_philox_masks: a region is (4-byte aligned pointer, n >= 0, rate in [0, 1) for kind 0 / [0, 1] for kind 1)");
+        if (m->n[i] > most) most = m->n[i];
+    }
+    if (most == 0) return T2_OK;
+    long gx = ((most + 3) / 4 + 256 * 4 - 1) / (256 * 4);
+    gx = gx < 1 ? 1 : (gx > 2048 ? 2048 : gx);
+    MasksK k; k.m = *m;
+    hipLaunchKernelGGL(philox_masks_kernel, dim3((unsigned)gx, m->count), dim3(256), 0, ST, k);
+    T2_CHECK_LAUNCH(); return T2_OK;
+}
 extern "C" int t2_sumsq(const float* g, int64_t n, double* out, void* stream) {
     (void)hipGetLastError();
     T2_REQUIRE(g && out, "t2_sumsq: null");
diff --git a/tacotron2_amd/csrc/t2_error.cpp b/tacotron2_amd/csrc/t2_error.cpp
--- a/tacotron2_amd/csrc/t2_error.cpp
+++ b/tacotron2_amd/csrc/t2_error.cpp
@@ -13,7 +13,7 @@
     T2_SZ(T2Gemm); T2_SZ(T2Seg); T2_SZ(T2LstmStep); T2_SZ(T2LstmStride); T2_SZ(T2LstmBwdStep); T2_SZ(T2LstmBwdStride);
     T2_SZ(T2AttnStep); T2_SZ(T2AttnSeq); T2_SZ(T2AttnSeqBwd); T2_SZ(T2Bn); T2_SZ(T2Infer); T2_SZ(T2StopScan); T2_SZ(T2ZeroRegions);
     T2_SZ(T2AlignDur); T2_SZ(T2AttnZone); T2_SZ(T2LossOpts); T2_SZ(T2MelCeps); T2_SZ(T2Dtw);
-    T2_SZ(T2Yin); T2_SZ(T2ProsodyStats);
+    T2_SZ(T2Yin); T2_SZ(T2ProsodyStats); T2_SZ(T2ConvPacks); T2_SZ(T2PhiloxMasks);
 #undef T2_SZ
     return -1;
 }
diff --git a/tacotron2_amd/engine.py b/tacotron2_amd/engine.py
--- a/tacotron2_amd/engine.py
+++ b/tacotron2_amd/engine.py
@@ -368,6 +368,49 @@
     return BackwardSchedule(tuple(chunks), tuple(tail))
 
 
+class LazyMask:
+    __slots__ = ("seed", "stream", "rate", "shape")
+
+    def __init__(self, seed: int, stream: int, rate: float, shape: tuple):
+        self.seed, self.stream, self.rate, self.shape = int(seed), int(stream), float(rate), tuple(shape)
+
+    def materialise(self, dev) -> torch.Tensor:
+        n = 1
+        for s in self.shape:
+            n *= s
+        m = torch.empty(n, dtype=torch.float32, device=dev)
+        call("t2_philox_mask", m, n, self.rate, self.seed, self.stream, _stream())
+        return m.view(*self.shape)
+
+
+def mask_plan(d: dict, r: int, cell_dropout: float, zoneout: float, B: int, L: int, T: int, training: bool, step: int) -> list:
+    p = float(d["dropout"])
+    E, Pd, A, D, M, Pn = d["encoded_dim"], d["prenet_dim"], d["att_rnn_dim"], d["rnn_hidden_dim"], d["num_mels"], d["postnet_dim"]
+    Tf, T = T, (T + r - 1) // r
+    plan, sid = [], [step * 64]
+
+    def add(key, i, name, shape, rate, conv=False):
+        plan.append((key, i, name, shape, rate, sid[0], 0, conv))
+        sid[0] += 1
+
+    if p > 0.0:
+        for i in range(2):
+            add("prenet_drop", i, f"pre{i}", (T + 1, B, Pd), p)
+    if training:
+        if p > 0.0:
+            for i in range(3):
+                add("enc_drop", i, f"enc{i}", (B, L, E), p, True)
+            for i, c in enumerate([Pn, Pn, Pn, Pn, M]):
+                add("post_drop", i, f"post{i}", (B, Tf, c), p, True)
+        if cell_dropout > 0.0:
+            add("att_drop", None, "att", (T, B, A), cell_dropout)
+            add("dec_drop", None, "dec", (T, B, D), cell_dropout)
+        if zoneout > 0.0:
+            for i, (key, H) in enumerate((("att_zone_h", A), ("att_zone_c", A), ("dec_zone_h", D), ("dec_zone_c", D))):
+                plan.append((key, None, key, (T, B, H), zoneout, step * 64 + 48 + i, 1, False))
+    return plan
+
+
 class Engine:
 
     def __init__(self, ps: ParamStore):
@@ -381,6 +424,7 @@
         self._ceps_bases: Dict[tuple, torch.Tensor] = {}
         self._cleared: Dict[tuple, tuple] = {}
         self._bn_clean: set = set()
+        self._packs: Dict[bool, tuple] = {}
         self._persist_next = 0
         self._side = None
         self.chunk = 64
@@ -504,40 +548,41 @@
             ev.record(torch.cuda.current_stream())
             self.spans.append((name, e0, ev))
 
-    def make_masks(self, B: int, L: int, T: int, training: bool, seed: int, step: int) -> dict:
+    def make_masks(self, B: int, L: int, T: int, training: bool, seed: int, step: int, lazy: bool = False) -> dict:
         d = self.d
-        p = float(d["dropout"])
-        E, Pd, A, D, M, Pn = d["encoded_dim"], d["prenet_dim"], d["att_rnn_dim"], d["rnn_hidden_dim"], d["num_mels"], d["postnet_dim"]
+        A, D = d["att_rnn_dim"], d["rnn_hidden_dim"]
         st = _stream()
-        sid = [step * 64]
-        Tf, T = T, (T + self.r - 1) // self.r
-
-        def gen(name, n, rate):
-            m = self.buf("mask." + name, n)
-            call("t2_philox_mask", m, n, rate, seed, sid[0], st)
-            sid[0] += 1
-            return m
-
-        masks = {}
-        if p > 0.0:
-            masks["prenet_drop"] = [gen(f"pre{i}", (T + 1) * B * Pd, p).view(T + 1, B, Pd) for i in range(2)]
-        if training:
-            if p > 0.0:
-                masks["enc_drop"] = [gen(f"enc{i}", B * L * E, p).view(B, L, E) for i in range(3)]
-                chans = [Pn, Pn, Pn, Pn, M]
-                masks["post_drop"] = [gen(f"post{i}", B * Tf * c, p).view(B, Tf, c) for i, c in enumerate(chans)]
-            if self.cell_dropout > 0.0:
-                masks["att_drop"] = gen("att", T * B * A, self.cell_dropout).view(T, B, A)
-                masks["dec_drop"] = gen("dec", T * B * D, self.cell_dropout).view(T, B, D)
-        if self.zoneout > 0.0 and training:
-            for i, (key, H) in enumerate((("att_zone_h", A), ("att_zone_c", A), ("dec_zone_h", D), ("dec_zone_c", D))):
-                masks[key] = self.buf("mask." + key, T, B, H)
-                call("t2_philox_bernoulli", masks[key], T * B * H, self.zoneout, seed, step * 64 + 48 + i, st)
-        elif self.zoneout > 0.0:
+        masks, regions = {}, []
+        for key, i, name, shape, rate, sid, kind, conv in mask_plan(d, self.r, self.cell_dropout, self.zoneout, B, L, T, training, step):
+            n = shape[0] * shape[1] * shape[2]
+            if lazy and conv and shape[2] % 4 == 0:
+                m = LazyMask(seed, sid, rate, shape)
+            else:
+                m = self.buf("mask." + name, n)
+                if lazy:
+                    regions.append((m, n, rate, sid, kind))
+                else:
+                    call("t2_philox_bernoulli" if kind else "t2_philox_mask", m, n, rate, seed, sid, st)
+                m = m.view(*shape)
+            if i is None:
+                masks[key] = m
+            else:
+                masks.setdefault(key, []).append(m)
+        if self.zoneout > 0.0 and not training:
             for cell, H in (("att", A), ("dec", D)):
                 block = self.buf(f"mask.{cell}_zone_p", 1, B, H).fill_(self.zoneout)
                 masks[cell + "_zone_h"] = masks[cell + "_zone_c"] = block
+        if lazy:
+            masks["_generate"] = (seed, regions)
         return masks
+
+    def generate_masks(self, masks: dict) -> None:
+        seed, regions = masks.get("_generate") or (0, [])
+        for i0 in range(0, len(regions), 8):
+            part = regions[i0:i0 + 8]
+            pm = make("T2PhiloxMasks", out=[m for m, *_ in part], n=[n for _, n, *_ in part], rate=[x[2] for x in part],
+                      stream_id=[x[3] for x in part], kind=[x[4] for x in part], seed=seed, count=len(part))
+            call("t2_philox_masks", pm, _stream())
 
     def buf(self, name: str, *shape, dtype=torch.float32, zero: bool = False) -> torch.Tensor:
         n = 1
@@ -668,12 +713,51 @@
         call("t2_lstm_pack_bwd", W, ldw, N4, W2, ldw2, N2, ncols, out, _stream())
         return out
 
+    @staticmethod
+    def bn_drop(drop, B, L, C) -> dict:
+        if not isinstance(drop, LazyMask):
+            return dict(drop=drop)
+        assert drop.shape == (B, L, C), f"LazyMask of shape {drop.shape} at a ({B}, {L}, {C}) layer"
+        return dict(drop=None, drop_seed=drop.seed, drop_stream=drop.stream, drop_rate=drop.rate)
+
+    def conv_layers(self) -> list:
+        E, M, Pn = self.d["encoded_dim"], self.d["num_mels"], self.d["postnet_dim"]
+        chans = [M, Pn, Pn, Pn, Pn, M]
+        return [(f"enc.conv{li}", f"encoder.convolutions.{i}.weight", E, E) for li, i in enumerate((0, 4, 8))] + \
+               [(f"post.conv{li}", f"postnet.postnet.{4 * li}.weight", chans[li + 1], chans[li]) for li in range(5)]
+
+    def pack_conv_weights(self, ctx, backward: bool) -> None:
+        P = self.ps.P
+        cached = self._packs.get(backward)
+        if cached is not None and cached[0] == self.ps.flat.data_ptr() and all(self._ws.get(n) is t for n, t in cached[1]):
+            blocks, images = cached[2], cached[3]
+        else:
+            entries, images = [], {}
+            for tag, key, Co, Ci in self.conv_layers():
+                images[(tag, 0)] = self.buf(f"{tag}.wp", Co, 5 * Ci)
+                entries.append((P[key], images[(tag, 0)], Co, Ci, 0))
+                if backward:
+                    images[(tag, 1)] = self.buf(f"{tag}.wf", Ci, 5 * Co)
+                    entries.append((P[key], images[(tag, 1)], Co, Ci, 1))
+            blocks = []
+            for i0 in range(0, len(entries), 16):
+                part = entries[i0:i0 + 16]
+                blocks.append(make("T2ConvPacks", w=[e[0] for e in part], wp=[e[1] for e in part], Co=[e[2] for e in part],
+                                   Ci=[e[3] for e in part], K=[5] * len(part), flip=[e[4] for e in part], count=len(part)))
+            names = [f"{tag}.{'wf' if flip else 'wp'}" for tag, flip in images]
+            self._packs[backward] = (self.ps.flat.data_ptr(), [(n, self._ws[n]) for n in names], blocks, images)
+        for cp in blocks:
+            call("t2_pack_conv_weights", cp, _stream())
+        ctx["packed"] = dict(images)
+
     def conv_bn_fwd(self, tag, x_pad, w, bias, bn_prefix, B, L, Ci, Co, act, drop, training, ctx,
                     y=None, Lp_y=None, pad_y=2, res=None, Lp_res=0, pad_res=0, length=None, fill=0.0):
         P, Bf = self.ps.P, self.ps.Bf
         Lp = L + 4
-        wp = self.buf(f"{tag}.wp", Co, 5 * Ci)
-        call("t2_pack_conv_weight", w, wp, Co, Ci, 5, 0, _stream())
+        wp = ctx.get("packed", {}).get((tag, 0))
+        if wp is None:
+            wp = self.buf(f"{tag}.wp", Co, 5 * Ci)
+            call("t2_pack_conv_weight", w, wp, Co, Ci, 5, 0, _stream())
         raw = self.buf(f"{tag}.raw", B * Lp, Co)
         Mg = B * Lp - 4
         tstats = None
@@ -692,8 +776,8 @@
         bn = make("T2Bn", B=B, L=L, C=Co, x=raw, Lp_x=Lp, gamma=P[bn_prefix + ".weight"], beta=P[bn_prefix + ".bias"],
                   running_mean=Bf[bn_prefix + ".running_mean"], running_var=Bf[bn_prefix + ".running_var"],
                   training=1 if training else 0, momentum=0.1, eps=1e-5, sums=sums, mean=mean, invstd=invstd, act=act,
-                  drop=drop, res=res, Lp_res=Lp_res, pad_res=pad_res, len=length, fill=fill, y=y, Lp_y=Lp_y, pad_y=pad_y,
-                  sums_prezeroed=1, tile_stats=tstats, tile_M=Mg if tstats is not None else 0)
+                  res=res, Lp_res=Lp_res, pad_res=pad_res, len=length, fill=fill, y=y, Lp_y=Lp_y, pad_y=pad_y,
+                  sums_prezeroed=1, tile_stats=tstats, tile_M=Mg if tstats is not None else 0, **self.bn_drop(drop, B, L, Co))
         if sync:
             shift = self.buf(f"{tag}.shift", Co)
             shift.copy_(Bf[bn_prefix + ".running_mean"])
@@ -850,8 +934,10 @@
         self.begin_phase(backward=False)
         self.mark("start")
         main0, side0 = torch.cuda.current_stream(), self.side_stream()
+        self.pack_conv_weights(ctx, backward=save_for_backward)
         self._wait(side0, main0)
         with torch.cuda.stream(side0):
+            self.generate_masks(masks)
             mel_tm = self.buf("mel_tm", T + 1, B, M)
             call("t2_mel_to_tm_r", mel, mel_tm, B, Tf, M, r, _stream())
             pd = masks.get("prenet_drop")
@@ -1011,8 +1097,8 @@
         sums = self.bn_sums(tag, backward=True)
         bn = make("T2Bn", B=B, L=L, C=Co, x=c["raw"], Lp_x=Lp, gamma=P[bn_prefix + ".weight"], beta=P[bn_prefix + ".bias"],
                   training=1 if training else 0, momentum=0.1, eps=1e-5, sums=sums, sums_prezeroed=1, mean=c["mean"], invstd=c["invstd"],
-                  act=act, drop=c["drop"], dy=dy, Lp_dy=Lp_dy, pad_dy=pad_dy, dx=draw, Lp_dx=Lp, pad_dx=2,
-                  dgamma=G[bn_prefix + ".weight"], dbeta=G[bn_prefix + ".bias"])
+                  act=act, dy=dy, Lp_dy=Lp_dy, pad_dy=pad_dy, dx=draw, Lp_dx=Lp, pad_dx=2,
+                  dgamma=G[bn_prefix + ".weight"], dbeta=G[bn_prefix + ".bias"], **self.bn_drop(c["drop"], B, L, Co))
         if training and self.sync_bn_group is not None:
             import torch.distributed as dist
             bn.phase = 1
@@ -1036,8 +1122,10 @@
                 wgrad()
         if not need_dx:
             return None
-        wf = self.buf(f"{tag}.wf", Ci, 5 * Co)
-        call("t2_pack_conv_weight", w, wf, Co, Ci, 5, 1, st)
+        wf = ctx.get("packed", {}).get((tag, 1))
+        if wf is None:
+            wf = self.buf(f"{tag}.wf", Ci, 5 * Co)
+            call("t2_pack_conv_weight", w, wf, Co, Ci, 5, 1, st)
         dx = self.buf(f"{tag}.dx", B * Lp, Ci)
         self.gemm_fill(draw, wf, dx, R, Ci, 5 * Co, Co, 5 * Co, Ci)
         return dx
diff --git a/tacotron2_amd/trainer.py b/tacotron2_amd/trainer.py
--- a/tacotron2_amd/trainer.py
+++ b/tacotron2_amd/trainer.py
@@ -134,7 +134,7 @@
         T = mel.shape[1]
         eng.marks = []; eng.spans = []
         if masks is None:
-            masks = eng.make_masks(B, L, T, True, self.seed + 7919 * self.rank, self.global_step)
+            masks = eng.make_masks(B, L, T, True, self.seed + 7919 * self.rank, self.global_step, lazy=True)
         eng.mark("masks")
         outs, ctx = eng.forward_tf(ci, batch["chars_idx_len"], mel, batch["mel_spectrogram_len"],
                                    speaker_id=batch.get("speaker_id"),
```

After: 296,400, median of 6. About the same (+0.1%).
